# misterk72/MiniVideo

Hardware: NVIDIA B200
Metric: 1080p_idr_frames_per_s_recon_rgb (higher is better)
Workload: dtype int32

## Files before the change

minivideo_b200/csrc/mvg_api.cu:

```cuda
#include "mvgpu.h"

#include <cuda_runtime.h>
#include <nvtx3/nvToolsExt.h>

#include <algorithm>
#include <cstdarg>
#include <cstdio>
#include <cstdlib>
#include <cstring>
#include <new>
#include <thread>
#include <vector>

#include "mvg_internal.h"
#include "mvg_kernels.cuh"
#include "mvg_fused.cuh"


static char g_create_error[512] = "";

struct MvgRange {
    explicit MvgRange(const char *name) { nvtxRangePushA(name); }
    ~MvgRange() { nvtxRangePop(); }
};

#define MVG_PIPE_DEPTH 3
#define MVG_MAX_TICKETS 8

struct MvgTicket {
    cudaEvent_t done = nullptr;
    bool busy = false;
    uint64_t *h_picbase = nullptr;
    int cap = 0;
};
#define MVG_WORK_RING  64
#define MVG_K2_GROUP   1024

struct mvg_ctx {
    int device = -1, sm_count = 0;
    int k1_ctas_per_sm = 1, k2_ctas_per_sm = 1, kf_ctas_per_sm = 1;
    int mode = MVG_PIPELINE_FUSED;
    int stagger_override = -1;
    int max_w = 0, max_h = 0, max_pics = 0;
    int w_mbs = 0, h_mbs = 0;
    bool have_sps = false;
    char err[512] = "";

    cudaStream_t stream = nullptr, s_h2d = nullptr, s_d2h = nullptr;
    cudaEvent_t ev[4] = {nullptr, nullptr, nullptr, nullptr};
    cudaEvent_t ev_mark[2] = {nullptr, nullptr};
    cudaEvent_t ev_h2d[MVG_PIPE_DEPTH] = {}, ev_comp[MVG_PIPE_DEPTH] = {}, ev_d2h[MVG_PIPE_DEPTH] = {};
    bool ran_k3 = false, ran_fused = false;
    bool tiles_valid = false;
    int launches = 0, last_scale = 0;

    uint8_t *d_kind = nullptr, *d_i16 = nullptr, *d_cm = nullptr, *d_cbp = nullptr, *d_modes = nullptr;
    int8_t *d_qp = nullptr;
    int16_t *d_coeff = nullptr;
    uint32_t *d_nzb = nullptr, *d_woff = nullptr;
    uint16_t *d_words = nullptr;
    uint64_t *d_picbase = nullptr;
    MvgTicket tickets[MVG_MAX_TICKETS];
    long long pipe_idx = 0;
    bool region_used[MVG_PIPE_DEPTH] = {};
    int16_t *d_resid = nullptr;
    MvgMbCtl *d_ctl = nullptr;
    uint8_t *d_tiles = nullptr;
    uint8_t *d_yuv = nullptr, *d_rgb = nullptr;
    uint2 *d_halo = nullptr;
    int *d_work = nullptr;
    unsigned long long *d_stats = nullptr;
    int work_next = 0;
    unsigned epoch = 0;
    int pipe_chunk = 0;
    MvgTables *d_tab = nullptr;
    MvgLuts *d_luts = nullptr;
    struct Alloc { void *base; size_t bytes; const char *name; };
    std::vector<Alloc> allocs;
    bool guard = false;

    size_t n_mb_max() const { return (size_t)max_w * max_h; }
    size_t n_mb() const { return (size_t)w_mbs * h_mbs; }
};

static int fail(mvg_ctx *ctx, const char *fmt, ...)
{
    char *dst = ctx ? ctx->err : g_create_error;
    va_list ap;
    va_start(ap, fmt);
    vsnprintf(dst, 512, fmt, ap);
    va_end(ap);
    return MVG_FAILURE;
}

#define CK(ctx, call)                                                                      \
    do {                                                                                   \
        cudaError_t e__ = (call);                                                          \
        if (e__ != cudaSuccess)                                                            \
            return fail(ctx, "%s failed: %s (%s:%d)", #call, cudaGetErrorString(e__), __FILE__, __LINE__); \
    } while (0)


static void zigzag(int n, uint8_t *zz)
{
    int r = 0, c = 0;
    bool up = true;
    for (int k = 0; k < n * n; k++) {
        zz[k] = (uint8_t)(r * n + c);
        if (up) {
            if (c == n - 1) { r++; up = false; }
            else if (r == 0) { c++; up = false; }
            else { r--; c++; }
        } else {
            if (r == n - 1) { c++; up = true; }
            else if (c == 0) { r++; up = true; }
            else { r++; c--; }
        }
    }
}

extern "C" int mvg_build_level_scale(const uint8_t *lists4x4, const uint8_t *list8x8,
                                     int32_t ls4[3 * 6 * 16], int32_t ls8[6 * 64])
{
    static const int v4[6][3] = {{10,16,13},{11,18,14},{13,20,16},{14,23,18},{16,25,20},{18,29,23}};
    static const int v8[6][6] = {{20,18,32,19,25,24},{22,19,35,21,28,26},{26,23,42,24,33,31},
                                 {28,25,45,26,35,33},{32,28,51,30,40,38},{36,32,58,34,46,43}};
    if (!ls4 || !ls8) return MVG_FAILURE;
    uint8_t zz4[16], zz8[64];
    zigzag(4, zz4); zigzag(8, zz8);
    for (int c = 0; c < 3; c++) {
        int m[16];
        for (int k = 0; k < 16; k++) m[zz4[k]] = lists4x4 ? lists4x4[c * 16 + k] : 16;
        for (int q = 0; q < 6; q++)
            for (int i = 0; i < 4; i++)
                for (int j = 0; j < 4; j++) {
                    const int cls = (i % 2 == 0 && j % 2 == 0) ? 0 : (i % 2 == 1 && j % 2 == 1) ? 1 : 2;
                    ls4[(c * 6 + q) * 16 + i * 4 + j] = m[i * 4 + j] * v4[q][cls];
                }
    }
    int m8[64];
    for (int k = 0; k < 64; k++) m8[zz8[k]] = list8x8 ? list8x8[k] : 16;
    for (int q = 0; q < 6; q++)
        for (int i = 0; i < 8; i++)
            for (int j = 0; j < 8; j++) {
                int cls;
                if (i % 4 == 0 && j % 4 == 0) cls = 0;
                else if (i % 2 == 1 && j % 2 == 1) cls = 1;
                else if (i % 4 == 2 && j % 4 == 2) cls = 2;
                else if ((i % 4 == 0 && j % 2 == 1) || (i % 2 == 1 && j % 4 == 0)) cls = 3;
                else if ((i % 4 == 0 && j % 4 == 2) || (i % 4 == 2 && j % 4 == 0)) cls = 4;
                else cls = 5;
                ls8[q * 64 + i * 8 + j] = m8[i * 8 + j] * v8[q][cls];
            }
    return MVG_SUCCESS;
}

struct Ref { bool left; int i; };
static Ref T(int i) { return {false, i}; }
static Ref L(int i) { return i < 0 ? Ref{false, -1} : Ref{true, i}; }

struct Taps { Ref r[4]; int form; };
static Taps tap3(Ref p, Ref q, Ref r) { return {{p, q, q, r}, 3}; }
static Taps tap2(Ref p, Ref q) { return {{p, p, q, q}, 2}; }
static Taps tap1(Ref p) { return {{p, p, p, p}, 1}; }
static Taps tapend(Ref p, Ref q) { return {{p, q, q, q}, 4}; }

static Taps nxn_taps(int n, int mode, int x, int y)
{
    switch (mode) {
    case 0: return tap1(T(x));
    case 1: return tap1(L(y));
    case 3: return (x == n - 1 && y == n - 1) ? tapend(T(2 * n - 2), T(2 * n - 1))
                                              : tap3(T(x + y), T(x + y + 1), T(x + y + 2));
    case 4:
        if (x > y) return tap3(T(x - y - 2), T(x - y - 1), T(x - y));
        if (x < y) return tap3(L(y - x - 2), L(y - x - 1), L(y - x));
        return tap3(T(0), T(-1), L(0));
    case 5: {
        const int z = 2 * x - y, i = x - (y >> 1);
        if (z >= 0 && !(z & 1)) return tap2(T(i - 1), T(i));
        if (z >= 0) return tap3(T(i - 2), T(i - 1), T(i));
        if (z == -1) return tap3(L(0), T(-1), T(0));
        return tap3(L(y - 2 * x - 1), L(y - 2 * x - 2), L(y - 2 * x - 3));
    }
    case 6: {
        const int z = 2 * y - x, i = y - (x >> 1);
        if (z >= 0 && !(z & 1)) return tap2(L(i - 1), L(i));
        if (z >= 0) return tap3(L(i - 2), L(i - 1), L(i));
        if (z == -1) return tap3(L(0), T(-1), T(0));
        return tap3(T(x - 2 * y - 1), T(x - 2 * y - 2), T(x - 2 * y - 3));
    }
    case 7: {
        const int i = x + (y >> 1);
        return (y & 1) ? tap3(T(i), T(i + 1), T(i + 2)) : tap2(T(i), T(i + 1));
    }
    case 8: {
        const int z = x + 2 * y, i = y + (x >> 1), zmax = 2 * n - 3;
        if (z > zmax) return tap1(L(n - 1));
        if (z == zmax) return tapend(L(n - 2), L(n - 1));
        return (z & 1) ? tap3(L(i), L(i + 1), L(i + 2)) : tap2(L(i), L(i + 1));
    }
    default: return tap1(T(0));
    }
}

extern "C" void mvg_build_luts(MvgLuts *out)
{
    memset(out, 0, sizeof *out);
    for (int row = 0; row < 16; row++) {
        const int mode = row == 11 ? 3 : row == 15 ? 7 : row;
        const bool dc = row == 2 || row == 9 || row == 10;
        if ((mode > 8 && !dc)) continue;
        const bool tr = row < 9;
        for (int y = 0; y < 4; y++)
            for (int x = 0; x < 4; x++) {
                Taps t = nxn_taps(4, mode, x, y);
                if (dc) {
                    const bool above = row == 9 || (row == 2 && !(x & 1));
                    for (int k = 0; k < 4; k++) t.r[k] = above ? T(k) : L(k);
                }
                uint32_t word = 0;
                for (int k = 0; k < 4; k++) {
                    int off;
                    if (t.r[k].left) off = t.r[k].i * MVG_LT_STRIDE - 1;
                    else {
                        int i = t.r[k].i;
                        if (!tr && i > 3) i = 3;
                        off = -MVG_LT_STRIDE + i;
                    }
                    word |= (uint32_t)(off + MVG_LUT4_BIAS) << (8 * k);
                }
                out->lut4[row][y * 4 + x] = out->lut4[row][16 + y * 4 + x] = word;
            }
    }
    auto line8 = [](Ref r) { return r.left ? MVG_N8_LEFT(r.i) : MVG_N8_TOP(r.i); };
    for (int mode = 0; mode < 9; mode++)
        for (int lane = 0; lane < 32; lane++) {
            uint32_t word = 0;
            for (int s = 0; s < 2; s++) {
                const int x = ((lane >> 3) & 1) * 4 + (lane & 1) * 2 + s, y = (lane >> 4) * 4 + ((lane >> 1) & 3);
                int idx = MVG_N8_DC, variant = 0;
                if (mode != 2) {
                    const Taps t = nxn_taps(8, mode, x, y);
                    if (t.form == 1) { idx = line8(t.r[0]); variant = 0; }
                    else if (t.form == 2) {
                        const int a = line8(t.r[0]), b = line8(t.r[3]);
                        idx = a < b ? a : b; variant = 1;
                    } else { idx = line8(t.r[1]); variant = 2; }
                }
                word |= (uint32_t)(mode == 2 ? MVG_N8_DC : MVG_N8_IDX(idx, variant)) << (16 * s);
            }
            out->lut8[mode][lane] = word;
        }
}


extern "C" const char *mvg_last_error(const mvg_ctx *ctx) { return ctx ? ctx->err : g_create_error; }

#define MVG_GUARD_BYTES ((size_t)64 << 10)
#define MVG_GUARD_BYTE  0xA5
#define MVG_POISON_BYTE 0x5A

static cudaError_t galloc(mvg_ctx *ctx, void **p, size_t bytes, const char *name)
{
    const size_t g = ctx->guard ? MVG_GUARD_BYTES : 0;
    void *base = nullptr;
    cudaError_t e = cudaMalloc(&base, bytes + 2 * g);
    if (e != cudaSuccess) return e;
    try { ctx->allocs.push_back({base, bytes, name}); } catch (...) { cudaFree(base); return cudaErrorMemoryAllocation; }
    if (ctx->guard) {
        e = cudaMemset(base, MVG_GUARD_BYTE, bytes + 2 * g);
        if (e == cudaSuccess) e = cudaMemset((uint8_t *)base + g, MVG_POISON_BYTE, bytes);
        if (e != cudaSuccess) return e;
    }
    *p = (uint8_t *)base + g;
    return cudaSuccess;
}
template <typename T>
static cudaError_t dalloc(mvg_ctx *ctx, T **p, size_t count, const char *name) { return galloc(ctx, (void **)p, count * sizeof(T), name); }

extern "C" int mvg_create(mvg_ctx **out, int device, int max_w_mbs, int max_h_mbs, int max_pics)
{
    if (!out) return fail(nullptr, "mvg_create: out is NULL");
    *out = nullptr;
    if (max_w_mbs < 1 || max_h_mbs < 1 || max_pics < 1) return fail(nullptr, "mvg_create: bad geometry");
    int n_dev = 0;
    cudaError_t e = cudaGetDeviceCount(&n_dev);
    if (e != cudaSuccess || n_dev == 0)
        return fail(nullptr, "mvg_create: no CUDA device (%s); this library has no CPU fallback",
                    e == cudaSuccess ? "device count 0" : cudaGetErrorString(e));
    if (device < 0 || device >= n_dev) return fail(nullptr, "mvg_create: device %d out of range (0..%d)", device, n_dev - 1);

    mvg_ctx *ctx = new (std::nothrow) mvg_ctx;
    if (!ctx) return fail(nullptr, "mvg_create: out of host memory");
    ctx->device = device; ctx->max_w = max_w_mbs; ctx->max_h = max_h_mbs; ctx->max_pics = max_pics;
    if (const char *gd = getenv("MVG_DEBUG_GUARD")) ctx->guard = gd[0] == '1';

    auto bail = [&](const char *what, cudaError_t err) {
        fail(nullptr, "mvg_create: %s: %s", what, cudaGetErrorString(err));
        mvg_destroy(ctx);
        return MVG_FAILURE;
    };
#define TRY(what, call) do { cudaError_t e2 = (call); if (e2 != cudaSuccess) return bail(what, e2); } while (0)
    TRY("cudaSetDevice", cudaSetDevice(device));
    cudaDeviceProp prop;
    TRY("cudaGetDeviceProperties", cudaGetDeviceProperties(&prop, device));
    ctx->sm_count = prop.multiProcessorCount;
    TRY("k1 shared memory", cudaFuncSetAttribute(k1_dequant_idct, cudaFuncAttributeMaxDynamicSharedMemorySize, (int)(sizeof(K1WarpSmem) * K1_WARPS)));
    TRY("occupancy k1", cudaOccupancyMaxActiveBlocksPerMultiprocessor(&ctx->k1_ctas_per_sm, k1_dequant_idct, K1_WARPS * 32, sizeof(K1WarpSmem) * K1_WARPS));
    TRY("k2 shared memory", cudaFuncSetAttribute(k2_wavefront, cudaFuncAttributeMaxDynamicSharedMemorySize, (int)K2_SMEM_BYTES));
    TRY("occupancy k2", cudaOccupancyMaxActiveBlocksPerMultiprocessor(&ctx->k2_ctas_per_sm, k2_wavefront, K2_WARPS * 32, K2_SMEM_BYTES));
    TRY("kf shared memory", cudaFuncSetAttribute(kf_recon<KF_OUT_TILES>, cudaFuncAttributeMaxDynamicSharedMemorySize, (int)KF_SMEM_BYTES(KF_OUT_TILES)));
    TRY("kf shared memory", cudaFuncSetAttribute(kf_recon<KF_OUT_RGB>, cudaFuncAttributeMaxDynamicSharedMemorySize, (int)KF_SMEM_BYTES(KF_OUT_RGB)));
    TRY("kf shared memory", cudaFuncSetAttribute(kf_recon<KF_OUT_RGBS, 1>, cudaFuncAttributeMaxDynamicSharedMemorySize, (int)KF_SMEM_BYTES(KF_OUT_RGBS)));
    TRY("kf shared memory", cudaFuncSetAttribute(kf_recon<KF_OUT_RGBS, 2>, cudaFuncAttributeMaxDynamicSharedMemorySize, (int)KF_SMEM_BYTES(KF_OUT_RGBS)));
    TRY("kf shared memory", cudaFuncSetAttribute(kf_recon<KF_OUT_RGBS, 3>, cudaFuncAttributeMaxDynamicSharedMemorySize, (int)KF_SMEM_BYTES(KF_OUT_RGBS)));
    TRY("kf shared memory", cudaFuncSetAttribute(kf_recon<KF_OUT_RGBS, 4>, cudaFuncAttributeMaxDynamicSharedMemorySize, (int)KF_SMEM_BYTES(KF_OUT_RGBS)));
    {
        int a = 0, b = 0;
        TRY("occupancy kf", cudaOccupancyMaxActiveBlocksPerMultiprocessor(&a, kf_recon<KF_OUT_RGB>, KF_WARPS_OF(KF_OUT_RGB) * 32, KF_SMEM_BYTES(KF_OUT_RGB)));
        TRY("occupancy kf", cudaOccupancyMaxActiveBlocksPerMultiprocessor(&b, kf_recon<KF_OUT_TILES>, KF_WARPS_OF(KF_OUT_TILES) * 32, KF_SMEM_BYTES(KF_OUT_TILES)));
        ctx->kf_ctas_per_sm = std::min(a, b);
    }
    if (ctx->k1_ctas_per_sm < 1 || ctx->k2_ctas_per_sm < 1 || ctx->kf_ctas_per_sm < 1)
        return bail("kernel does not fit on an SM", cudaErrorLaunchOutOfResources);
    if (const char *m = getenv("MVG_PIPELINE")) ctx->mode = strcmp(m, "split") == 0 ? MVG_PIPELINE_SPLIT : MVG_PIPELINE_FUSED;
    if (const char *e = getenv("MVG_KF_STAGGER")) ctx->stagger_override = std::min(std::max(atoi(e), 0), 64);
    TRY("stream", cudaStreamCreateWithFlags(&ctx->stream, cudaStreamNonBlocking));
    TRY("stream", cudaStreamCreateWithFlags(&ctx->s_h2d, cudaStreamNonBlocking));
    TRY("stream", cudaStreamCreateWithFlags(&ctx->s_d2h, cudaStreamNonBlocking));
    for (auto &ev : ctx->ev) TRY("event", cudaEventCreate(&ev));
    for (auto &ev : ctx->ev_mark) TRY("event", cudaEventCreate(&ev));
    for (int i = 0; i < MVG_PIPE_DEPTH; i++) {
        TRY("event", cudaEventCreateWithFlags(&ctx->ev_h2d[i], cudaEventDisableTiming));
        TRY("event", cudaEventCreateWithFlags(&ctx->ev_comp[i], cudaEventDisableTiming));
        TRY("event", cudaEventCreateWithFlags(&ctx->ev_d2h[i], cudaEventDisableTiming));
    }
    const size_t n = ctx->n_mb_max() * (size_t)max_pics;
    TRY("alloc mb_kind", dalloc(ctx, &ctx->d_kind, n, "mb_kind"));
    TRY("alloc i16_mode", dalloc(ctx, &ctx->d_i16, n, "i16_mode"));
    TRY("alloc chroma_mode", dalloc(ctx, &ctx->d_cm, n, "chroma_mode"));
    TRY("alloc qp", dalloc(ctx, &ctx->d_qp, n, "qp"));
    TRY("alloc cbp", dalloc(ctx, &ctx->d_cbp, n, "cbp"));
    TRY("alloc luma_modes", dalloc(ctx, &ctx->d_modes, n * 16, "luma_modes"));
    TRY("alloc coeff", dalloc(ctx, &ctx->d_coeff, n * 384, "coeff"));
    TRY("alloc tiles", dalloc(ctx, &ctx->d_tiles, n * 384, "tiles"));
    TRY("alloc rgb", dalloc(ctx, &ctx->d_rgb, n * 768, "rgb"));
    TRY("alloc halo", dalloc(ctx, &ctx->d_halo, n * 8, "halo"));
    if (!ctx->guard) TRY("clear halo", cudaMemset(ctx->d_halo, 0, n * 8 * sizeof(uint2)));
    TRY("alloc work", dalloc(ctx, &ctx->d_work, MVG_WORK_RING, "work"));
    TRY("alloc stats", dalloc(ctx, &ctx->d_stats, 16, "stats"));
    TRY("clear stats", cudaMemset(ctx->d_stats, 0, 16 * sizeof(unsigned long long)));
    TRY("alloc tables", dalloc(ctx, &ctx->d_tab, 1, "tables"));
    TRY("alloc luts", dalloc(ctx, &ctx->d_luts, 1, "luts"));
    MvgLuts luts;
    mvg_build_luts(&luts);
    TRY("upload luts", cudaMemcpy(ctx->d_luts, &luts, sizeof luts, cudaMemcpyHostToDevice));
#undef TRY
    *out = ctx;
    return MVG_SUCCESS;
}

extern "C" int mvg_destroy(mvg_ctx *ctx)
{
    if (!ctx) return MVG_FAILURE;
    cudaSetDevice(ctx->device);
    cudaDeviceSynchronize();
    for (auto &a : ctx->allocs) cudaFree(a.base);
    for (auto &t : ctx->tickets) { if (t.h_picbase) cudaFreeHost(t.h_picbase); if (t.done) cudaEventDestroy(t.done); }
    for (auto ev : ctx->ev) if (ev) cudaEventDestroy(ev);
    for (auto ev : ctx->ev_mark) if (ev) cudaEventDestroy(ev);
    for (int i = 0; i < MVG_PIPE_DEPTH; i++) {
        if (ctx->ev_h2d[i]) cudaEventDestroy(ctx->ev_h2d[i]);
        if (ctx->ev_comp[i]) cudaEventDestroy(ctx->ev_comp[i]);
        if (ctx->ev_d2h[i]) cudaEventDestroy(ctx->ev_d2h[i]);
    }
    if (ctx->stream) cudaStreamDestroy(ctx->stream);
    if (ctx->s_h2d) cudaStreamDestroy(ctx->s_h2d);
    if (ctx->s_d2h) cudaStreamDestroy(ctx->s_d2h);
    delete ctx;
    return MVG_SUCCESS;
}

extern "C" int mvg_set_sps(mvg_ctx *ctx, int width_mbs, int height_mbs,
                           const int32_t level_scale4x4[3 * 6 * 16], const int32_t level_scale8x8[6 * 64],
                           int cb_qp_offset, int cr_qp_offset)
{
    MvgRange nvtx_range("mvg_set_sps");
    if (!ctx) return MVG_FAILURE;
    if (!level_scale4x4 || !level_scale8x8) return fail(ctx, "mvg_set_sps: NULL table");
    if (width_mbs < 1 || height_mbs < 1 || width_mbs > ctx->max_w || height_mbs > ctx->max_h)
        return fail(ctx, "mvg_set_sps: %dx%d MBs exceeds the context capacity %dx%d",
                    width_mbs, height_mbs, ctx->max_w, ctx->max_h);
    CK(ctx, cudaSetDevice(ctx->device));
    MvgTables t;
    memset(&t, 0, sizeof t);
    memcpy(t.ls4, level_scale4x4, sizeof t.ls4);
    memcpy(t.ls8, level_scale8x8, sizeof t.ls8);
    for (int c = 0; c < 3; c++)
        for (int qp = 0; qp < 52; qp++)
            for (int k = 0; k < 16; k++) {
                const int32_t v = t.ls4[c][qp % 6][k];
                t.ls4q[c][qp][k] = qp > 23 ? (int32_t)((uint32_t)v << (qp / 6 - 4)) : v;
            }
    uint8_t zz8[64];
    zigzag(8, zz8);
    for (int k = 0; k < 64; k++) t.zz8inv[zz8[k]] = (uint8_t)k;
    t.cb_qp_offset = cb_qp_offset; t.cr_qp_offset = cr_qp_offset;
    CK(ctx, cudaStreamSynchronize(ctx->s_h2d));
    CK(ctx, cudaStreamSynchronize(ctx->stream));
    CK(ctx, cudaStreamSynchronize(ctx->s_d2h));
    CK(ctx, cudaMemcpy(ctx->d_tab, &t, sizeof t, cudaMemcpyHostToDevice));
    ctx->w_mbs = width_mbs; ctx->h_mbs = height_mbs; ctx->have_sps = true;
    return MVG_SUCCESS;
}

extern "C" int mvg_set_pipeline(mvg_ctx *ctx, int chunk_pics)
{
    if (!ctx || chunk_pics < 0) return MVG_FAILURE;
    ctx->pipe_chunk = chunk_pics;
    return MVG_SUCCESS;
}

extern "C" int mvg_dev_k2_stats(mvg_ctx *ctx, unsigned long long out[16])
{
    if (!ctx || !out) return MVG_FAILURE;
    CK(ctx, cudaSetDevice(ctx->device));
    CK(ctx, cudaStreamSynchronize(ctx->stream));
    CK(ctx, cudaMemcpy(out, ctx->d_stats, 16 * sizeof(unsigned long long), cudaMemcpyDeviceToHost));
    CK(ctx, cudaMemset(ctx->d_stats, 0, 16 * sizeof(unsigned long long)));
    return MVG_SUCCESS;
}

extern "C" long long mvg_debug_check(mvg_ctx *ctx, char *report, size_t report_cap)
{
    if (!ctx) return -1;
    if (report && report_cap) report[0] = 0;
    if (!ctx->guard) return 0;
    if (cudaSetDevice(ctx->device) != cudaSuccess || cudaDeviceSynchronize() != cudaSuccess) return -1;
    std::vector<uint8_t> h(MVG_GUARD_BYTES);
    long long bad = 0;
    for (auto &a : ctx->allocs)
        for (int side = 0; side < 2; side++) {
            const uint8_t *src = (const uint8_t *)a.base + (side ? MVG_GUARD_BYTES + a.bytes : 0);
            if (cudaMemcpy(h.data(), src, MVG_GUARD_BYTES, cudaMemcpyDeviceToHost) != cudaSuccess) return -1;
            long long here = 0;
            for (uint8_t b : h) here += b != MVG_GUARD_BYTE;
            if (here && report && report_cap) {
                const size_t o = strlen(report);
                snprintf(report + o, report_cap - o, "%s%s(%s): %lld bytes", o ? ", " : "", a.name, side ? "after" : "before", here);
            }
            bad += here;
        }
    return bad;
}

extern "C" int mvg_debug_check_kernels(mvg_ctx *ctx, unsigned long long out[8])
{
    if (!ctx || !out) return MVG_FAILURE;
    memset(out, 0, 8 * sizeof(unsigned long long));
#ifdef MVG_CHECKED
    CK(ctx, cudaSetDevice(ctx->device));
    CK(ctx, cudaDeviceSynchronize());
    CK(ctx, cudaMemcpyFromSymbol(out, mvg_check_fail, 8 * sizeof(unsigned long long)));
    return MVG_SUCCESS;
#else
    return MVG_UNSUPPORTED;
#endif
}

extern "C" int mvg_device_count(void)
{
    int n = 0;
    return cudaGetDeviceCount(&n) == cudaSuccess ? n : 0;
}

extern "C" int mvg_width(const mvg_ctx *ctx) { return ctx ? 16 * ctx->w_mbs : 0; }
extern "C" int mvg_height(const mvg_ctx *ctx) { return ctx ? 16 * ctx->h_mbs : 0; }
extern "C" int mvg_max_pics(const mvg_ctx *ctx) { return ctx ? ctx->max_pics : 0; }
extern "C" int mvg_sm_count(const mvg_ctx *ctx) { return ctx ? ctx->sm_count : 0; }

extern "C" void *mvg_host_alloc(size_t bytes)
{
    void *p = nullptr;
    if (cudaHostAlloc(&p, bytes, cudaHostAllocDefault) != cudaSuccess) return nullptr;
    return p;
}
extern "C" void mvg_host_free(void *p) { if (p) cudaFreeHost(p); }


static int check_ready(mvg_ctx *ctx, int first_slot, int n_pics, const char *who)
{
    if (!ctx) return MVG_FAILURE;
    if (!ctx->have_sps) return fail(ctx, "%s: mvg_set_sps() has not been called", who);
    if (n_pics < 1 || first_slot < 0 || first_slot + n_pics > ctx->max_pics)
        return fail(ctx, "%s: slots [%d,%d) outside [0,%d)", who, first_slot, first_slot + n_pics, ctx->max_pics);
    return MVG_SUCCESS;
}

static int upload_async(mvg_ctx *ctx, const mvg_batch *b, int src_pic, int first_slot, int n_pics, cudaStream_t st)
{
    const size_t n = ctx->n_mb(), o = (size_t)first_slot * n, s = (size_t)src_pic * n, cnt = (size_t)n_pics * n;
    CK(ctx, cudaMemcpyAsync(ctx->d_kind + o, b->mb_kind + s, cnt, cudaMemcpyHostToDevice, st));
    CK(ctx, cudaMemcpyAsync(ctx->d_i16 + o, b->i16_mode + s, cnt, cudaMemcpyHostToDevice, st));
    CK(ctx, cudaMemcpyAsync(ctx->d_cm + o, b->chroma_mode + s, cnt, cudaMemcpyHostToDevice, st));
    CK(ctx, cudaMemcpyAsync(ctx->d_qp + o, b->qp_y + s, cnt, cudaMemcpyHostToDevice, st));
    if (b->cbp) CK(ctx, cudaMemcpyAsync(ctx->d_cbp + o, b->cbp + s, cnt, cudaMemcpyHostToDevice, st));
    CK(ctx, cudaMemcpyAsync(ctx->d_modes + o * 16, b->luma_modes + s * 16, cnt * 16, cudaMemcpyHostToDevice, st));
    CK(ctx, cudaMemcpyAsync(ctx->d_coeff + o * 384, b->coeff + s * 384, cnt * 768, cudaMemcpyHostToDevice, st));
    return MVG_SUCCESS;
}

static int check_batch(mvg_ctx *ctx, const mvg_batch *b, const char *who)
{
    if (!b) return fail(ctx, "%s: batch is NULL", who);
    if (!b->mb_kind || !b->i16_mode || !b->chroma_mode || !b->qp_y || !b->luma_modes || !b->coeff)
        return fail(ctx, "%s: a required SoA pointer is NULL", who);
    return MVG_SUCCESS;
}

extern "C" int mvg_upload(mvg_ctx *ctx, const mvg_batch *b, int first_slot)
{
    MvgRange nvtx_range("mvg_upload");
    if (!ctx) return MVG_FAILURE;
    if (check_batch(ctx, b, "mvg_upload") != MVG_SUCCESS) return MVG_FAILURE;
    if (check_ready(ctx, first_slot, b->n_pics, "mvg_upload") != MVG_SUCCESS) return MVG_FAILURE;
    CK(ctx, cudaSetDevice(ctx->device));
    if (upload_async(ctx, b, 0, first_slot, b->n_pics, ctx->stream) != MVG_SUCCESS) return MVG_FAILURE;
    CK(ctx, cudaStreamSynchronize(ctx->stream));
    return MVG_SUCCESS;
}

extern "C" int mvg_clone_slot(mvg_ctx *ctx, int src_slot, int dst_slot)
{
    MvgRange nvtx_range("mvg_clone_slot");
    if (check_ready(ctx, src_slot, 1, "mvg_clone_slot") != MVG_SUCCESS) return MVG_FAILURE;
    if (check_ready(ctx, dst_slot, 1, "mvg_clone_slot") != MVG_SUCCESS) return MVG_FAILURE;
    CK(ctx, cudaSetDevice(ctx->device));
    const size_t n = ctx->n_mb(), s = (size_t)src_slot * n, d = (size_t)dst_slot * n;
    cudaStream_t st = ctx->stream;
    CK(ctx, cudaMemcpyAsync(ctx->d_kind + d, ctx->d_kind + s, n, cudaMemcpyDeviceToDevice, st));
    CK(ctx, cudaMemcpyAsync(ctx->d_i16 + d, ctx->d_i16 + s, n, cudaMemcpyDeviceToDevice, st));
    CK(ctx, cudaMemcpyAsync(ctx->d_cm + d, ctx->d_cm + s, n, cudaMemcpyDeviceToDevice, st));
    CK(ctx, cudaMemcpyAsync(ctx->d_qp + d, ctx->d_qp + s, n, cudaMemcpyDeviceToDevice, st));
    CK(ctx, cudaMemcpyAsync(ctx->d_cbp + d, ctx->d_cbp + s, n, cudaMemcpyDeviceToDevice, st));
    CK(ctx, cudaMemcpyAsync(ctx->d_modes + d * 16, ctx->d_modes + s * 16, n * 16, cudaMemcpyDeviceToDevice, st));
    CK(ctx, cudaMemcpyAsync(ctx->d_coeff + d * 384, ctx->d_coeff + s * 384, n * 768, cudaMemcpyDeviceToDevice, st));
    return MVG_SUCCESS;
}


static int ensure_yuv(mvg_ctx *ctx)
{
    if (!ctx->d_yuv) CK(ctx, dalloc(ctx, &ctx->d_yuv, ctx->n_mb_max() * (size_t)ctx->max_pics * 384, "yuv"));
    return MVG_SUCCESS;
}
static int ensure_split(mvg_ctx *ctx)
{
    const size_t n = ctx->n_mb_max() * (size_t)ctx->max_pics;
    if (!ctx->d_resid) CK(ctx, dalloc(ctx, &ctx->d_resid, n * 384, "residual"));
    if (!ctx->d_ctl) CK(ctx, dalloc(ctx, &ctx->d_ctl, n, "ctl"));
    return MVG_SUCCESS;
}

static int launch_planar(mvg_ctx *ctx, int first_slot, int n_pics, cudaStream_t st)
{
    if (ensure_yuv(ctx) != MVG_SUCCESS) return MVG_FAILURE;
    K3Params p;
    p.tiles = ctx->d_tiles; p.yuv = ctx->d_yuv; p.rgb = nullptr; p.width = 16 * ctx->w_mbs; p.height = 16 * ctx->h_mbs;
    p.scale = 1; p.first_slot = first_slot; p.n_pics = n_pics;
    const long long threads = (long long)ctx->n_mb() * 12 * n_pics;
    const int grid = (int)std::min<long long>((threads + 255) / 256, (long long)ctx->sm_count * 32);
    k4_yuv_planar<<<grid, 256, 0, st>>>(p);
    CK(ctx, cudaGetLastError());
    return MVG_SUCCESS;
}

static int launch_k1(mvg_ctx *ctx, int first_slot, int n_pics, cudaStream_t st)
{
    if (ensure_split(ctx) != MVG_SUCCESS) return MVG_FAILURE;
    const size_t n = ctx->n_mb();
    K1Params p;
    const size_t o = (size_t)first_slot * n;
    p.mb_kind = ctx->d_kind + o; p.i16_mode = ctx->d_i16 + o; p.chroma_mode = ctx->d_cm + o;
    p.luma_modes = ctx->d_modes + o * 16; p.qp_y = ctx->d_qp + o; p.coeff = ctx->d_coeff + o * 384;
    p.resid = ctx->d_resid + o * 384; p.ctl = ctx->d_ctl + o; p.tab = ctx->d_tab;
    p.n_mbs = (long long)n * n_pics;
    const long long groups = (p.n_mbs + K1_GROUP - 1) / K1_GROUP;
    const long long want = (groups + K1_WARPS - 1) / K1_WARPS;
    const int grid = (int)std::min<long long>(want, (long long)ctx->sm_count * ctx->k1_ctas_per_sm);
    k1_dequant_idct<<<grid, K1_WARPS * 32, sizeof(K1WarpSmem) * K1_WARPS, st>>>(p);
    CK(ctx, cudaGetLastError());
    return MVG_SUCCESS;
}

static int launch_k3(mvg_ctx *ctx, int first_slot, int n_pics, int rgb_scale, cudaStream_t st)
{
    const size_t n = ctx->n_mb();
    const int width = 16 * ctx->w_mbs, height = 16 * ctx->h_mbs;
    K3Params p;
    p.tiles = ctx->d_tiles; p.yuv = nullptr; p.rgb = ctx->d_rgb; p.width = width; p.height = height; p.scale = rgb_scale;
    p.first_slot = first_slot; p.n_pics = n_pics;
    const long long threads = rgb_scale == 1 ? (long long)n * 8 * n_pics
                                             : (long long)(width / rgb_scale) * (height / rgb_scale) * n_pics;
    const int grid = (int)std::min<long long>((threads + 255) / 256, (long long)ctx->sm_count * 32);
    const bool pow2 = rgb_scale == 2 || rgb_scale == 4 || rgb_scale == 8 || rgb_scale == 16;
    if (rgb_scale == 1) k3_rgb_full<<<grid, 256, 0, st>>>(p);
    else if (pow2) k3_rgb_scaled<<<(int)std::min<long long>(((long long)n * n_pics + 31) / 32, (long long)ctx->sm_count * 16), 256, 0, st>>>(p);
    else k3_rgb_scaled_generic<<<grid, 256, 0, st>>>(p);
    CK(ctx, cudaGetLastError());
    return MVG_SUCCESS;
}

static int launch_stages(mvg_ctx *ctx, int first_slot, int n_pics, int rgb_scale, bool want_tiles, cudaStream_t st, bool timed)
{
    const int W = ctx->w_mbs, H = ctx->h_mbs;
    const size_t n = ctx->n_mb();
    const int width = 16 * W, height = 16 * H;
    if (rgb_scale < 0 || (rgb_scale > 0 && (width % rgb_scale || height % rgb_scale)))
        return fail(ctx, "rgb_scale %d does not divide %dx%d", rgb_scale, width, height);

    int *work = ctx->d_work + ctx->work_next;
    ctx->work_next = (ctx->work_next + 1) % MVG_WORK_RING;
    CK(ctx, cudaMemsetAsync(work, 0, sizeof(int), st));
    if (++ctx->epoch == 0) ctx->epoch = 1;

    const bool fused = ctx->mode == MVG_PIPELINE_FUSED;
    const bool thumbs = rgb_scale == 2 || rgb_scale == 4 || rgb_scale == 8 || rgb_scale == 16;
    const bool rgb_direct = fused && !want_tiles && (rgb_scale == 1 || thumbs);
    int launches = 0;
    if (timed) CK(ctx, cudaEventRecord(ctx->ev[0], st));
    if (!fused) {
        if (launch_k1(ctx, first_slot, n_pics, st) != MVG_SUCCESS) return MVG_FAILURE;
        launches++;
    }
    if (timed) CK(ctx, cudaEventRecord(ctx->ev[1], st));
    const long long items = (long long)n_pics * H;
    if (fused) {
        KFParams p;
        p.mb_kind = ctx->d_kind; p.i16_mode = ctx->d_i16; p.chroma_mode = ctx->d_cm; p.luma_modes = ctx->d_modes;
        p.qp_y = ctx->d_qp; p.coeff = ctx->d_coeff; p.tiles = ctx->d_tiles; p.rgb = ctx->d_rgb; p.halo = ctx->d_halo;
        p.work = work; p.tab = ctx->d_tab; p.luts = ctx->d_luts; p.epoch = ctx->epoch;
        p.w_mbs = W; p.h_mbs = H; p.first_slot = first_slot; p.n_pics = n_pics; p.group = MVG_K2_GROUP;
        p.sel[0] = 1u; p.sel[1] = 1u << 8; p.sel[2] = 1u << 16; p.sel[3] = 1u << 24;
        p.stats = ctx->d_stats;
        p.stagger = items < 2LL * ctx->sm_count * KF_WARPS ? KF_GROUP + 1 : KF_STAGGER;
        if (ctx->stagger_override >= 0) p.stagger = ctx->stagger_override;
        const int grid = (int)std::min<long long>(items, (long long)ctx->sm_count * ctx->kf_ctas_per_sm);
        if (rgb_direct && thumbs) {
            const unsigned bt = KF_WARPS_OF(KF_OUT_RGBS) * 32;
            const size_t sm = KF_SMEM_BYTES(KF_OUT_RGBS);
            if (rgb_scale == 2)      kf_recon<KF_OUT_RGBS, 1><<<grid, bt, sm, st>>>(p);
            else if (rgb_scale == 4) kf_recon<KF_OUT_RGBS, 2><<<grid, bt, sm, st>>>(p);
            else if (rgb_scale == 8) kf_recon<KF_OUT_RGBS, 3><<<grid, bt, sm, st>>>(p);
            else                     kf_recon<KF_OUT_RGBS, 4><<<grid, bt, sm, st>>>(p);
        } else if (rgb_direct) kf_recon<KF_OUT_RGB><<<grid, KF_WARPS_OF(KF_OUT_RGB) * 32, KF_SMEM_BYTES(KF_OUT_RGB), st>>>(p);
        else kf_recon<KF_OUT_TILES><<<grid, KF_WARPS_OF(KF_OUT_TILES) * 32, KF_SMEM_BYTES(KF_OUT_TILES), st>>>(p);
        launches++;
    } else {
        K2Params p;
        p.resid = ctx->d_resid; p.ctl = ctx->d_ctl; p.tiles = ctx->d_tiles; p.halo = ctx->d_halo;
        p.epoch = ctx->epoch; p.group = MVG_K2_GROUP; p.stats = ctx->d_stats;
        p.sel[0] = 1u; p.sel[1] = 1u << 8; p.sel[2] = 1u << 16; p.sel[3] = 1u << 24;
        p.work = work; p.luts = ctx->d_luts; p.w_mbs = W; p.h_mbs = H; p.first_slot = first_slot; p.n_pics = n_pics;
        const int grid = (int)std::min<long long>((items + K2_WARPS - 1) / K2_WARPS, (long long)ctx->sm_count * ctx->k2_ctas_per_sm);
        k2_wavefront<<<grid, K2_WARPS * 32, K2_SMEM_BYTES, st>>>(p);
        launches++;
    }
    CK(ctx, cudaGetLastError());
    if (timed) CK(ctx, cudaEventRecord(ctx->ev[2], st));
    const bool run_k3 = rgb_scale >= 1 && !rgb_direct;
    if (run_k3) {
        if (launch_k3(ctx, first_slot, n_pics, rgb_scale, st) != MVG_SUCCESS) return MVG_FAILURE;
        launches++;
    }
    if (timed) {
        CK(ctx, cudaEventRecord(ctx->ev[3], st));
        ctx->ran_k3 = run_k3;
        ctx->ran_fused = fused;
        ctx->launches = launches;
    }
    ctx->last_scale = rgb_scale;
    ctx->tiles_valid = !rgb_direct;
    return MVG_SUCCESS;
}

extern "C" int mvg_run(mvg_ctx *ctx, int first_slot, int n_pics, int rgb_scale)
{
    MvgRange nvtx_range("mvg_run");
    if (check_ready(ctx, first_slot, n_pics, "mvg_run") != MVG_SUCCESS) return MVG_FAILURE;
    CK(ctx, cudaSetDevice(ctx->device));
    return launch_stages(ctx, first_slot, n_pics, rgb_scale, true, ctx->stream, true);
}

extern "C" int mvg_run_thumbs(mvg_ctx *ctx, int first_slot, int n_pics, int rgb_scale)
{
    MvgRange nvtx_range("mvg_run_thumbs");
    if (check_ready(ctx, first_slot, n_pics, "mvg_run_thumbs") != MVG_SUCCESS) return MVG_FAILURE;
    if (rgb_scale < 1) return fail(ctx, "mvg_run_thumbs: rgb_scale %d", rgb_scale);
    CK(ctx, cudaSetDevice(ctx->device));
    return launch_stages(ctx, first_slot, n_pics, rgb_scale, false, ctx->stream, true);
}

extern "C" int mvg_run_rgb(mvg_ctx *ctx, int first_slot, int n_pics)
{
    MvgRange nvtx_range("mvg_run_rgb");
    if (check_ready(ctx, first_slot, n_pics, "mvg_run_rgb") != MVG_SUCCESS) return MVG_FAILURE;
    CK(ctx, cudaSetDevice(ctx->device));
    return launch_stages(ctx, first_slot, n_pics, 1, false, ctx->stream, true);
}

extern "C" int mvg_set_pipeline_mode(mvg_ctx *ctx, int mode)
{
    if (!ctx || (mode != MVG_PIPELINE_FUSED && mode != MVG_PIPELINE_SPLIT)) return MVG_FAILURE;
    ctx->mode = mode;
    return MVG_SUCCESS;
}

extern "C" int mvg_sync(mvg_ctx *ctx)
{
    if (!ctx) return MVG_FAILURE;
    CK(ctx, cudaSetDevice(ctx->device));
    CK(ctx, cudaStreamSynchronize(ctx->stream));
    CK(ctx, cudaStreamSynchronize(ctx->s_h2d));
    CK(ctx, cudaStreamSynchronize(ctx->s_d2h));
    return MVG_SUCCESS;
}

extern "C" int mvg_get_timing(mvg_ctx *ctx, mvg_timing *out)
{
    if (!ctx || !out) return MVG_FAILURE;
    CK(ctx, cudaSetDevice(ctx->device));
    CK(ctx, cudaEventSynchronize(ctx->ev[3]));
    out->k1_dequant_idct_ms = out->k2_wavefront_ms = out->fused_ms = 0.f;
    if (ctx->ran_fused) CK(ctx, cudaEventElapsedTime(&out->fused_ms, ctx->ev[1], ctx->ev[2]));
    else {
        CK(ctx, cudaEventElapsedTime(&out->k1_dequant_idct_ms, ctx->ev[0], ctx->ev[1]));
        CK(ctx, cudaEventElapsedTime(&out->k2_wavefront_ms, ctx->ev[1], ctx->ev[2]));
    }
    out->k3_rgb_ms = 0.f;
    if (ctx->ran_k3) CK(ctx, cudaEventElapsedTime(&out->k3_rgb_ms, ctx->ev[2], ctx->ev[3]));
    CK(ctx, cudaEventElapsedTime(&out->total_ms, ctx->ev[0], ctx->ev[3]));
    out->launches = ctx->launches;
    return MVG_SUCCESS;
}

extern "C" int mvg_mark(mvg_ctx *ctx, int which)
{
    if (!ctx || which < 0 || which > 1) return MVG_FAILURE;
    CK(ctx, cudaSetDevice(ctx->device));
    CK(ctx, cudaEventRecord(ctx->ev_mark[which], ctx->stream));
    return MVG_SUCCESS;
}

extern "C" int mvg_mark_elapsed(mvg_ctx *ctx, float *ms)
{
    if (!ctx || !ms) return MVG_FAILURE;
    CK(ctx, cudaSetDevice(ctx->device));
    CK(ctx, cudaEventSynchronize(ctx->ev_mark[1]));
    CK(ctx, cudaEventElapsedTime(ms, ctx->ev_mark[0], ctx->ev_mark[1]));
    return MVG_SUCCESS;
}


static size_t rgb_bytes(const mvg_ctx *ctx, int scale)
{
    return (size_t)(16 * ctx->w_mbs / scale) * (16 * ctx->h_mbs / scale) * 3;
}

extern "C" int mvg_download_yuv420(mvg_ctx *ctx, int slot, uint8_t *y, uint8_t *cb, uint8_t *cr)
{
    MvgRange nvtx_range("mvg_download_yuv420");
    if (check_ready(ctx, slot, 1, "mvg_download_yuv420") != MVG_SUCCESS) return MVG_FAILURE;
    if (!ctx->tiles_valid) return fail(ctx, "mvg_download_yuv420: the last run produced RGB24 only (mvg_run_rgb, mvg_run_thumbs); use mvg_run()");
    CK(ctx, cudaSetDevice(ctx->device));
    const size_t n = ctx->n_mb();
    if (launch_planar(ctx, slot, 1, ctx->stream) != MVG_SUCCESS) return MVG_FAILURE;
    const uint8_t *src = ctx->d_yuv + (size_t)slot * n * 384;
    CK(ctx, cudaStreamSynchronize(ctx->stream));
    if (y) CK(ctx, cudaMemcpy(y, src, n * 256, cudaMemcpyDeviceToHost));
    if (cb) CK(ctx, cudaMemcpy(cb, src + n * 256, n * 64, cudaMemcpyDeviceToHost));
    if (cr) CK(ctx, cudaMemcpy(cr, src + n * 320, n * 64, cudaMemcpyDeviceToHost));
    return MVG_SUCCESS;
}

extern "C" int mvg_download_rgb(mvg_ctx *ctx, int slot, uint8_t *rgb)
{
    MvgRange nvtx_range("mvg_download_rgb");
    if (check_ready(ctx, slot, 1, "mvg_download_rgb") != MVG_SUCCESS) return MVG_FAILURE;
    if (!rgb || ctx->last_scale < 1) return fail(ctx, "mvg_download_rgb: no RGB output (last run had rgb_scale 0)");
    CK(ctx, cudaSetDevice(ctx->device));
    const size_t sz = rgb_bytes(ctx, ctx->last_scale);
    CK(ctx, cudaStreamSynchronize(ctx->stream));
    CK(ctx, cudaMemcpy(rgb, ctx->d_rgb + (size_t)slot * sz, sz, cudaMemcpyDeviceToHost));
    return MVG_SUCCESS;
}

extern "C" int mvg_download_residual(mvg_ctx *ctx, int slot, int16_t *residual)
{
    MvgRange nvtx_range("mvg_download_residual");
    if (check_ready(ctx, slot, 1, "mvg_download_residual") != MVG_SUCCESS) return MVG_FAILURE;
    if (!residual) return fail(ctx, "mvg_download_residual: NULL");
    CK(ctx, cudaSetDevice(ctx->device));
    const size_t n = ctx->n_mb();
    if (launch_k1(ctx, slot, 1, ctx->stream) != MVG_SUCCESS) return MVG_FAILURE;
    CK(ctx, cudaStreamSynchronize(ctx->stream));
    int16_t *tmp = new (std::nothrow) int16_t[n * 384];
    if (!tmp) return fail(ctx, "mvg_download_residual: out of host memory");
    cudaError_t e = cudaMemcpy(tmp, ctx->d_resid + (size_t)slot * n * 384, n * 768, cudaMemcpyDeviceToHost);
    if (e != cudaSuccess) { delete[] tmp; return fail(ctx, "cudaMemcpy failed: %s", cudaGetErrorString(e)); }
    for (size_t mb = 0; mb < n; mb++) {
        const int16_t *src = tmp + mb * 384;
        int16_t *dst = residual + mb * 384;
        for (int b = 0; b < 16; b++) {
            const int bx = (b & 1) | (((b >> 2) & 1) << 1), by = ((b >> 1) & 1) | ((b >> 3) << 1);
            for (int i = 0; i < 4; i++)
                for (int j = 0; j < 4; j++) dst[(by * 4 + i) * 16 + bx * 4 + j] = src[b * 16 + i * 4 + j];
        }
        for (int p = 0; p < 2; p++)
            for (int b = 0; b < 4; b++)
                for (int i = 0; i < 4; i++)
                    for (int j = 0; j < 4; j++)
                        dst[256 + p * 64 + ((b >> 1) * 4 + i) * 8 + (b & 1) * 4 + j] = src[256 + p * 64 + b * 16 + i * 4 + j];
    }
    delete[] tmp;
    return MVG_SUCCESS;
}


static int take_ticket(mvg_ctx *ctx, mvg_ticket *out)
{
    for (int i = 0; i < MVG_MAX_TICKETS; i++)
        if (!ctx->tickets[i].busy) {
            if (!ctx->tickets[i].done) CK(ctx, cudaEventCreateWithFlags(&ctx->tickets[i].done, cudaEventDisableTiming | cudaEventBlockingSync));
            *out = i;
            return MVG_SUCCESS;
        }
    return fail(ctx, "too many submissions in flight (%d): mvg_wait() for one first", MVG_MAX_TICKETS);
}

template <typename Upload, typename Expand>
static int decode_pipeline(mvg_ctx *ctx, int n_pics, uint8_t *yuv_out, uint8_t *rgb_out, int rgb_scale, cudaEvent_t done_ev,
                           Upload upload, Expand expand)
{
    const int scale = rgb_out ? rgb_scale : 0;
    const size_t n = ctx->n_mb();
    const size_t yuv_sz = n * 384, rgb_sz = scale ? rgb_bytes(ctx, scale) : 0;
    if (yuv_out && ensure_yuv(ctx) != MVG_SUCCESS) return MVG_FAILURE;
    int depth = MVG_PIPE_DEPTH;
    if (ctx->max_pics < depth) depth = 1;
    const int region = std::max(1, ctx->max_pics / depth);
    int chunk = std::min(region, std::max(1, (n_pics + 7) / 8));
    if (scale > 1 && !yuv_out) chunk = std::min(region, std::max(chunk, std::min(n_pics, 128)));
    if (ctx->pipe_chunk > 0) chunk = std::min(ctx->pipe_chunk, region);
    for (int done = 0; done < n_pics; done += chunk, ctx->pipe_idx++) {
        const int cnt = std::min(chunk, n_pics - done);
        const int r = (int)(ctx->pipe_idx % depth), slot0 = r * region;
        const bool used = ctx->region_used[r];
        ctx->region_used[r] = true;
        if (used) CK(ctx, cudaStreamWaitEvent(ctx->s_h2d, ctx->ev_comp[r], 0));
        if (upload(done, slot0, cnt) != MVG_SUCCESS) return MVG_FAILURE;
        CK(ctx, cudaEventRecord(ctx->ev_h2d[r], ctx->s_h2d));
        CK(ctx, cudaStreamWaitEvent(ctx->stream, ctx->ev_h2d[r], 0));
        if (used) CK(ctx, cudaStreamWaitEvent(ctx->stream, ctx->ev_d2h[r], 0));
        if (expand(slot0, cnt) != MVG_SUCCESS) return MVG_FAILURE;
        if (launch_stages(ctx, slot0, cnt, scale, yuv_out != nullptr, ctx->stream, false) != MVG_SUCCESS) return MVG_FAILURE;
        if (yuv_out && launch_planar(ctx, slot0, cnt, ctx->stream) != MVG_SUCCESS) return MVG_FAILURE;
        CK(ctx, cudaEventRecord(ctx->ev_comp[r], ctx->stream));
        CK(ctx, cudaStreamWaitEvent(ctx->s_d2h, ctx->ev_comp[r], 0));
        if (yuv_out)
            CK(ctx, cudaMemcpyAsync(yuv_out + (size_t)done * yuv_sz, ctx->d_yuv + (size_t)slot0 * yuv_sz,
                                    (size_t)cnt * yuv_sz, cudaMemcpyDeviceToHost, ctx->s_d2h));
        if (rgb_out)
            CK(ctx, cudaMemcpyAsync(rgb_out + (size_t)done * rgb_sz, ctx->d_rgb + (size_t)slot0 * rgb_sz,
                                    (size_t)cnt * rgb_sz, cudaMemcpyDeviceToHost, ctx->s_d2h));
        CK(ctx, cudaEventRecord(ctx->ev_d2h[r], ctx->s_d2h));
    }
    CK(ctx, cudaEventRecord(done_ev, ctx->s_d2h));
    return MVG_SUCCESS;
}

extern "C" int mvg_wait(mvg_ctx *ctx, mvg_ticket ticket)
{
    MvgRange nvtx_range("mvg_wait");
    if (!ctx) return MVG_FAILURE;
    if (ticket < 0 || ticket >= MVG_MAX_TICKETS || !ctx->tickets[ticket].busy) return fail(ctx, "mvg_wait: ticket %d is not in flight", (int)ticket);
    CK(ctx, cudaSetDevice(ctx->device));
    ctx->tickets[ticket].busy = false;
    CK(ctx, cudaEventSynchronize(ctx->tickets[ticket].done));
    return MVG_SUCCESS;
}

extern "C" int mvg_poll(mvg_ctx *ctx, mvg_ticket ticket, int *done)
{
    if (!ctx || !done) return MVG_FAILURE;
    if (ticket < 0 || ticket >= MVG_MAX_TICKETS || !ctx->tickets[ticket].busy) return fail(ctx, "mvg_poll: ticket %d is not in flight", (int)ticket);
    const cudaError_t e = cudaEventQuery(ctx->tickets[ticket].done);
    if (e != cudaSuccess && e != cudaErrorNotReady) return fail(ctx, "mvg_poll: %s", cudaGetErrorString(e));
    *done = e == cudaSuccess;
    return MVG_SUCCESS;
}

extern "C" int mvg_submit(mvg_ctx *ctx, const mvg_batch *b, uint8_t *yuv_out, uint8_t *rgb_out, int rgb_scale, mvg_ticket *ticket)
{
    MvgRange nvtx_range("mvg_submit");
    if (!ctx) return MVG_FAILURE;
    if (!ticket) return fail(ctx, "mvg_submit: ticket is NULL");
    if (check_batch(ctx, b, "mvg_submit") != MVG_SUCCESS) return MVG_FAILURE;
    if (!ctx->have_sps) return fail(ctx, "mvg_submit: mvg_set_sps() has not been called");
    if (b->n_pics < 1) return fail(ctx, "mvg_submit: empty batch");
    if (rgb_out && rgb_scale < 1) return fail(ctx, "mvg_submit: rgb_out given but rgb_scale < 1");
    CK(ctx, cudaSetDevice(ctx->device));
    if (take_ticket(ctx, ticket) != MVG_SUCCESS) return MVG_FAILURE;
    MvgTicket &t = ctx->tickets[*ticket];
    const mvg_batch batch = *b;
    if (decode_pipeline(ctx, batch.n_pics, yuv_out, rgb_out, rgb_scale, t.done,
                        [&](int done, int slot0, int cnt) { return upload_async(ctx, &batch, done, slot0, cnt, ctx->s_h2d); },
                        [&](int, int) { return (int)MVG_SUCCESS; }) != MVG_SUCCESS) return MVG_FAILURE;
    t.busy = true;
    return MVG_SUCCESS;
}

extern "C" int mvg_decode_host(mvg_ctx *ctx, const mvg_batch *b, uint8_t *yuv_out, uint8_t *rgb_out, int rgb_scale)
{
    mvg_ticket t;
    if (mvg_submit(ctx, b, yuv_out, rgb_out, rgb_scale, &t) != MVG_SUCCESS) return MVG_FAILURE;
    return mvg_wait(ctx, t);
}


extern "C" int mvg_pack_batch(const int16_t *coeff, int n_pics, int n_mbs, uint32_t *nz_blocks, uint32_t *word_off,
                              uint64_t *pic_off, uint16_t *words, size_t words_capacity, int n_threads)
{
    MvgRange nvtx_range("mvg_pack_batch");
    if (!coeff || !nz_blocks || !word_off || !pic_off || !words || n_pics < 1 || n_mbs < 1) return MVG_FAILURE;
    try {
    std::vector<uint64_t> pic_words((size_t)n_pics);
    auto pass1 = [&](int p) {
        uint64_t off = 0;
        for (int m = 0; m < n_mbs; m++) {
            const size_t mb = (size_t)p * n_mbs + m;
            const int16_t *c = coeff + mb * 384;
            uint32_t nzb = 0;
            unsigned words_here = 0;
            for (int b = 0; b < 24; b++) {
                unsigned cnt = 0;
                for (int k = 0; k < 16; k++) cnt += c[b * 16 + k] != 0;
                if (cnt) { nzb |= 1u << b; words_here += 1 + cnt; }
            }
            nz_blocks[mb] = nzb;
            word_off[mb] = (uint32_t)off;
            off += words_here;
        }
        pic_words[(size_t)p] = off;
    };
    auto pass2 = [&](int p) {
        for (int m = 0; m < n_mbs; m++) {
            const size_t mb = (size_t)p * n_mbs + m;
            const int16_t *c = coeff + mb * 384;
            const uint32_t nzb = nz_blocks[mb];
            uint16_t *w = words + pic_off[p] + word_off[mb];
            uint16_t *lv = w + __builtin_popcount(nzb);
            for (int b = 0; b < 24; b++) {
                if (!((nzb >> b) & 1u)) continue;
                unsigned mask = 0;
                for (int k = 0; k < 16; k++)
                    if (c[b * 16 + k]) { mask |= 1u << k; *lv++ = (uint16_t)c[b * 16 + k]; }
                *w++ = (uint16_t)mask;
            }
        }
    };
    int nt = n_threads > 0 ? n_threads : (int)std::thread::hardware_concurrency();
    nt = std::max(1, std::min(nt, n_pics));
    auto run = [&](auto &fn) {
        std::vector<std::thread> th;
        for (int t = 0; t < nt; t++)
            th.emplace_back([&, t] { for (int p = t; p < n_pics; p += nt) fn(p); });
        for (auto &x : th) x.join();
    };
    run(pass1);
    pic_off[0] = 0;
    for (int p = 0; p < n_pics; p++) pic_off[p + 1] = pic_off[p] + pic_words[(size_t)p];
    if (pic_off[n_pics] > words_capacity) return MVG_FAILURE;
    run(pass2);
    } catch (...) {
        return MVG_FAILURE;
    }
    return MVG_SUCCESS;
}

extern "C" int mvg_submit_packed(mvg_ctx *ctx, const mvg_packed_batch *b, uint8_t *yuv_out, uint8_t *rgb_out, int rgb_scale, mvg_ticket *ticket)
{
    MvgRange nvtx_range("mvg_submit_packed");
    if (!ctx) return MVG_FAILURE;
    if (!ticket) return fail(ctx, "mvg_submit_packed: ticket is NULL");
    if (!b) return fail(ctx, "mvg_decode_host_packed: batch is NULL");
    if (!b->mb_kind || !b->i16_mode || !b->chroma_mode || !b->qp_y || !b->luma_modes || !b->nz_blocks || !b->word_off ||
        !b->pic_off || !b->words)
        return fail(ctx, "mvg_decode_host_packed: a required pointer is NULL");
    if (!ctx->have_sps) return fail(ctx, "mvg_decode_host_packed: mvg_set_sps() has not been called");
    if (b->n_pics < 1) return fail(ctx, "mvg_decode_host_packed: empty batch");
    if (rgb_out && rgb_scale < 1) return fail(ctx, "mvg_decode_host_packed: rgb_out given but rgb_scale < 1");
    CK(ctx, cudaSetDevice(ctx->device));
    const size_t n = ctx->n_mb();
    if (!ctx->d_words) {
        const size_t cap = ctx->n_mb_max() * (size_t)ctx->max_pics;
        CK(ctx, dalloc(ctx, &ctx->d_nzb, cap, "nz_blocks"));
        CK(ctx, dalloc(ctx, &ctx->d_woff, cap, "word_off"));
        CK(ctx, dalloc(ctx, &ctx->d_words, cap * MVG_PACKED_WORDS_PER_MB, "words"));
        CK(ctx, dalloc(ctx, &ctx->d_picbase, (size_t)ctx->max_pics * 2 + 2, "pic_base"));
    }
    if (take_ticket(ctx, ticket) != MVG_SUCCESS) return MVG_FAILURE;
    MvgTicket &tk = ctx->tickets[*ticket];
    if (b->n_pics > tk.cap) {
        if (tk.h_picbase) cudaFreeHost(tk.h_picbase);
        tk.h_picbase = nullptr; tk.cap = 0;
        CK(ctx, cudaHostAlloc((void **)&tk.h_picbase, ((size_t)b->n_pics * 2 + 2) * sizeof(uint64_t), cudaHostAllocDefault));
        tk.cap = b->n_pics;
    }
    for (int p = 0; p < b->n_pics; p++)
        if (b->pic_off[p + 1] < b->pic_off[p] || b->pic_off[p + 1] - b->pic_off[p] > (uint64_t)n * MVG_PACKED_WORDS_PER_MB)
            return fail(ctx, "mvg_decode_host_packed: picture %d has an impossible word count", p);
    auto upload = [&](int done, int slot0, int cnt) -> int {
        const size_t o = (size_t)slot0 * n, s = (size_t)done * n, c = (size_t)cnt * n;
        cudaStream_t st = ctx->s_h2d;
        CK(ctx, cudaMemcpyAsync(ctx->d_kind + o, b->mb_kind + s, c, cudaMemcpyHostToDevice, st));
        CK(ctx, cudaMemcpyAsync(ctx->d_i16 + o, b->i16_mode + s, c, cudaMemcpyHostToDevice, st));
        CK(ctx, cudaMemcpyAsync(ctx->d_cm + o, b->chroma_mode + s, c, cudaMemcpyHostToDevice, st));
        CK(ctx, cudaMemcpyAsync(ctx->d_qp + o, b->qp_y + s, c, cudaMemcpyHostToDevice, st));
        CK(ctx, cudaMemcpyAsync(ctx->d_modes + o * 16, b->luma_modes + s * 16, c * 16, cudaMemcpyHostToDevice, st));
        CK(ctx, cudaMemcpyAsync(ctx->d_nzb + o, b->nz_blocks + s, c * sizeof(uint32_t), cudaMemcpyHostToDevice, st));
        CK(ctx, cudaMemcpyAsync(ctx->d_woff + o, b->word_off + s, c * sizeof(uint32_t), cudaMemcpyHostToDevice, st));
        const uint64_t w0 = b->pic_off[done], w1 = b->pic_off[done + cnt], base = (uint64_t)o * MVG_PACKED_WORDS_PER_MB;
        if (w1 > w0)
            CK(ctx, cudaMemcpyAsync(ctx->d_words + base, b->words + w0, (size_t)(w1 - w0) * sizeof(uint16_t), cudaMemcpyHostToDevice, st));
        uint64_t *hb = tk.h_picbase + 2 * (size_t)done;
        for (int i = 0; i <= cnt; i++) hb[i] = base + (b->pic_off[done + i] - w0);
        CK(ctx, cudaMemcpyAsync(ctx->d_picbase + 2 * (size_t)slot0, hb, (size_t)(cnt + 1) * sizeof(uint64_t), cudaMemcpyHostToDevice, st));
        return MVG_SUCCESS;
    };
    auto expand = [&](int slot0, int cnt) -> int {
        K0Params p;
        const size_t o = (size_t)slot0 * n;
        p.nz_blocks = ctx->d_nzb + o; p.word_off = ctx->d_woff + o; p.pic_base = ctx->d_picbase + 2 * (size_t)slot0;
        p.words = ctx->d_words; p.coeff = ctx->d_coeff + o * 384; p.n_mbs = (long long)cnt * (long long)n; p.mbs_per_pic = (int)n;
        const long long warps = p.n_mbs;
        const int grid = (int)std::min<long long>((warps + 7) / 8, (long long)ctx->sm_count * 16);
        k0_expand_levels<<<grid, 256, 0, ctx->stream>>>(p);
        CK(ctx, cudaGetLastError());
        return MVG_SUCCESS;
    };
    if (decode_pipeline(ctx, b->n_pics, yuv_out, rgb_out, rgb_scale, tk.done, upload, expand) != MVG_SUCCESS) return MVG_FAILURE;
    tk.busy = true;
    return MVG_SUCCESS;
}

extern "C" int mvg_decode_host_packed(mvg_ctx *ctx, const mvg_packed_batch *b, uint8_t *yuv_out, uint8_t *rgb_out, int rgb_scale)
{
    mvg_ticket t;
    if (mvg_submit_packed(ctx, b, yuv_out, rgb_out, rgb_scale, &t) != MVG_SUCCESS) return MVG_FAILURE;
    return mvg_wait(ctx, t);
}
```

minivideo_b200/csrc/mvg_fused.cuh:

```cuda
#pragma once

#include <cstddef>

#include "mvg_kernels.cuh"

#ifndef KF_GROUP
#define KF_GROUP 4
#endif
#ifndef KF_WARPS
#define KF_WARPS 25
#endif
#ifndef KF_WARPS_TILES
#define KF_WARPS_TILES 28
#endif
#ifndef KF_WARPS_RGBS
#define KF_WARPS_RGBS 28
#endif
#define KF_WARPS_OF(out) ((out) == 1 ? KF_WARPS : (out) == 2 ? KF_WARPS_RGBS : KF_WARPS_TILES)
#ifndef KF_COMPACT8
#define KF_COMPACT8 false
#endif
#ifndef KF_POLL_NS
#define KF_POLL_NS 1000
#endif
#ifndef KF_STAGGER
#define KF_STAGGER 12
#endif
#ifndef KF_MBS
#define KF_MBS 392
#endif
#define KF_OUT_TILES 0
#define KF_OUT_RGB   1
#define KF_OUT_RGBS  2
#define KF_RGBS_PITCH 96
#define KF_RGB_STRIDE 112
#ifndef KF_WO_GROUP
#define KF_WO_GROUP (KF_GROUP == 4)
#endif
#define KF_RGB_GSTRIDE 208
#ifndef KF_HALO_GROUP
#define KF_HALO_GROUP (KF_GROUP == 4)
#endif

struct KFParams {
    const uint8_t *mb_kind, *i16_mode, *chroma_mode, *luma_modes;
    const int8_t  *qp_y;
    const int16_t *coeff;
    uint8_t       *tiles;
    uint8_t       *rgb;
    uint2         *halo;
    int           *work;
    const MvgTables *tab;
    const MvgLuts   *luts;
    unsigned        epoch;
    int w_mbs, h_mbs, first_slot, n_pics, group;
    int stagger;
    unsigned        sel[4];
    unsigned long long *stats;
};

#ifdef KF_STATS
#define KF_STAT(...) __VA_ARGS__
#else
#define KF_STAT(...)
#endif

template <int OUT>
struct KFWarpSmemT {
    union {
        MvgXfScratch<KF_GROUP> x;
        uint8_t rgb[OUT == 0 ? 16 : OUT == 2 ? 8 * KF_RGBS_PITCH : KF_WO_GROUP ? 16 * KF_RGB_GSTRIDE : 16 * KF_RGB_STRIDE];
    } u;
    MVG_CANARY(c0)
    __align__(128) int16_t tile[KF_GROUP * KF_MBS];
    __align__(8) uint64_t mbar;
    __align__(16) uint32_t hrow[36];
    MVG_CANARY(c1)
    __align__(16) uint8_t lt[MVG_LT_ROWS * MVG_LT_STRIDE];
    uint8_t ct_pad[4];
    alignas(OUT == 0 ? 16 : 4) uint8_t ct[2][MVG_CT_PLANE];
    MVG_CANARY(c2)
    __align__(16) uint8_t n8[MVG_N8_BYTES];
    MVG_CANARY(c3)
#ifdef KF_REC_PAD
    uint8_t pad[KF_REC_PAD];
#endif
};

#define KF_LUT_BYTES  ((sizeof(MvgLuts) + 127) / 128 * 128)
#define KF_TAB_BYTES  ((sizeof(MvgXfTables) + 127) / 128 * 128)
#define KF_SMEM_BYTES(out) (sizeof(KFWarpSmemT<out>) * KF_WARPS_OF(out) + 2048 + KF_LUT_BYTES + KF_TAB_BYTES)

#ifdef KF_MAXREG
#define KF_BOUNDS __maxnreg__(KF_MAXREG)
#else
#define KF_BOUNDS __launch_bounds__(KF_WARPS_OF(OUT) * 32, 1)
#endif
template <int OUT, int SL = 2>
__global__ void KF_BOUNDS
kf_recon(KFParams p)
{
    extern __shared__ __align__(128) uint8_t kf_smem[];
    typedef KFWarpSmemT<OUT> KFWarpSmem;
    const int lane = mvg_lane();
    const unsigned wid = __shfl_sync(MVG_FULL, threadIdx.x >> 5, 0);
    const unsigned base = mvg_smem_u32(kf_smem);
    const unsigned lut_addr = __shfl_sync(MVG_FULL, mvg_keep((base + 2047u) & ~2047u), 0);
    const unsigned n_before = (lut_addr - base) / (unsigned)sizeof(KFWarpSmem);
    MvgLuts *luts = reinterpret_cast<MvgLuts *>(__cvta_shared_to_generic(lut_addr));
    MvgXfTables &T = *reinterpret_cast<MvgXfTables *>(__cvta_shared_to_generic(lut_addr + (unsigned)KF_LUT_BYTES));
    unsigned rec_addr = base + (wid < n_before ? wid * (unsigned)sizeof(KFWarpSmem)
                                               : (lut_addr - base) + (unsigned)(KF_LUT_BYTES + KF_TAB_BYTES) + (wid - n_before) * (unsigned)sizeof(KFWarpSmem));
    rec_addr = __shfl_sync(MVG_FULL, mvg_keep(rec_addr), 0);
    KFWarpSmem &s = *reinterpret_cast<KFWarpSmem *>(__cvta_shared_to_generic(rec_addr));
    for (int i = threadIdx.x; i < (int)(KF_LUT_BYTES / 16); i += blockDim.x)
        reinterpret_cast<uint4 *>(luts)[i] = __ldg(reinterpret_cast<const uint4 *>(p.luts) + i);
    mvg_xf_load_tables(T, p.tab);
    if (lane == 0) mvg_mbar_init(&s.mbar, 1);
    asm volatile("fence.mbarrier_init.release.cluster;" ::: "memory");
    asm volatile("fence.proxy.async.shared::cta;" ::: "memory");
    __syncthreads();

    const int W = p.w_mbs, H = p.h_mbs, n_mb = W * H;
    const int total = p.n_pics * H;
    const unsigned epoch = p.epoch;
    const int n_groups = (W + KF_GROUP - 1) / KF_GROUP;

    K2Ctx c;
#ifdef MVG_CHECKED
    c.rec_lo = reinterpret_cast<const uint8_t *>(&s); c.rec_hi = c.rec_lo + sizeof(KFWarpSmem);
    if (lane < 4) s.c0[lane] = s.c1[lane] = s.c2[lane] = s.c3[lane] = MVG_CANARY_WORD;
    __syncwarp();
#endif
    c.lt = s.lt; c.ct = &s.ct[0][0]; c.n8 = s.n8; c.lut8 = reinterpret_cast<const uint8_t *>(&luts->lut8[0][lane]);
    c.lane = lane;
    c.sel = p.sel;
    c.resid = reinterpret_cast<const uint8_t *>(s.tile);
    {
        const int half = lane >> 4, pix = lane & 15, px = pix & 3, py = pix >> 2;
        c.lut4 = lut_addr + (unsigned)lane * 4u;
        c.h4 = half ? 0u : (unsigned)(4 * MVG_LT_STRIDE - 8);
        c.s4 = py * MVG_LT_STRIDE + px + (int)c.h4;
        c.r4odd = pix * 2 + (half ? 64 : 0);
        c.r4even = pix * 2 + (half ? -64 : 0);
        c.m4c = half ? 0x10100010u : 0x10001000u;
        c.m4b = half ? 0x00000100u : 0x00000011u;
        c.m4cc = half ? 0x00001000u : 0u;
        const int n = lane < 25 ? lane : 24;
        if (n < 8)       c.n8tr = (7 - n) * MVG_LT_STRIDE - 1;
        else if (n == 8) c.n8tr = -MVG_LT_STRIDE - 1;
        else             c.n8tr = -MVG_LT_STRIDE + (n - 9);
        c.n8notr = n > 16 ? -MVG_LT_STRIDE + 7 : c.n8tr;
        const int x8 = ((lane >> 3) & 1) * 4 + (lane & 1) * 2, y8 = (lane >> 4) * 4 + ((lane >> 1) & 3);
        c.s8 = y8 * MVG_LT_STRIDE + x8;
        c.fixA = lane == 7 ? 0x10u : lane == 8 ? 0x22u : lane == 9 ? 0x20u : 0u;
        c.fixB = lane == 7 ? 0x04u : lane == 8 ? 0x05u : lane == 9 ? 0x08u : 0u;
        c.fixD = lane == 7 ? 0x01u : lane == 9 ? 0x02u : 0u;
        c.lut4 = mvg_keep(c.lut4); c.h4 = mvg_keep(c.h4); c.s4 = mvg_keep(c.s4); c.r4odd = mvg_keep(c.r4odd); c.r4even = mvg_keep(c.r4even);
    }
    uint8_t *const halo_top = lane < 4 ? s.lt + K2_TO(lane * 4, -1)
                            : lane < 8 ? s.ct[(lane >> 1) & 1] + K2_CO((lane & 1) * 4, -1)
                                       : s.lt + K2_TO(16 + (lane & 1) * 4, -1);
    const uint8_t *const halo_bot = lane < 4 ? halo_top + 16 * MVG_LT_STRIDE : halo_top + 8 * MVG_CT_STRIDE;
    const uint8_t *const cn_src = (lane == 3 || lane == 5 || lane == 7) ? halo_top + 3 : s.lt;
    uint8_t *const cn_dst = lane == 3 ? s.lt + K2_TO(-1, -1) : lane == 5 ? s.ct[0] + K2_CO(-1, -1)
                          : lane == 7 ? s.ct[1] + K2_CO(-1, -1) : s.lt;
    const uint8_t *wo_src, *wo_csrc = nullptr;
    uint8_t *lc_dst, *lc_cdst = nullptr, *rgb_dst = nullptr;
    const uint8_t *lc_src = nullptr;
    int wo_off = 0;
    if (OUT == KF_OUT_TILES) {
        wo_src = lane < 16 ? s.lt + K2_TO(0, lane) : s.ct[(lane >> 3) & 1] + K2_CO(0, lane & 7);
        wo_off = lane < 16 ? lane * 16 : 256 + (lane - 16) * 8;
        lc_dst = lane < 16 ? s.lt + K2_TO(-1, lane) : s.ct[(lane >> 3) & 1] + K2_CO(-1, lane & 7);
    } else {
        const int q = lane >> 2, h = lane & 3;
        wo_src = s.lt + K2_TO(4 * h, 2 * q);
        wo_csrc = s.ct[0] + K2_CO(2 * h, q);
        lc_dst = s.lt + K2_TO(-1, 2 * q);
        lc_cdst = s.ct[0] + K2_CO(-1, q);
        lc_dst = lane < 16 ? s.lt + K2_TO(-1, lane) : s.ct[(lane >> 3) & 1] + K2_CO(-1, lane & 7);
        lc_src = lc_dst + (lane < 16 ? 16 : 8);
        rgb_dst = KF_WO_GROUP ? s.u.rgb + q * KF_RGB_GSTRIDE + 12 * h : s.u.rgb + 2 * q * KF_RGB_STRIDE + 12 * h;
    }
    const unsigned lc_sel = lane < 16 ? 7u : 3u;
    const int pitch = 48 * W;

    MvgSideInfo side;
    side.init(lane, p.mb_kind, p.i16_mode, p.chroma_mode, p.luma_modes, p.qp_y);
    unsigned parity = 0;
    KF_STAT(unsigned long long st[8] = {0, 0, 0, 0, 0, 0, 0, 0};)

    for (;;) {
        int item = 0;
        if (lane == 0) item = atomicAdd(p.work, 1);
        item = __shfl_sync(MVG_FULL, item, 0);
        if (item >= total) break;
        const int g0 = item / (p.group * H);
        const int gsize = min(p.group, p.n_pics - g0 * p.group);
        const int within = item - g0 * p.group * H;
        const int row = within / gsize;
        const int slot = p.first_slot + g0 * p.group + (within - row * gsize);
        const size_t mb0 = (size_t)slot * n_mb + (size_t)row * W;
        const int16_t *lv_row = p.coeff + mb0 * 384;

        if (lane == 0) {
            const int n0 = min(KF_GROUP, W);
            asm volatile("fence.proxy.async.shared::cta;" ::: "memory");
            mvg_mbar_expect_tx(&s.mbar, (unsigned)n0 * 768u);
            if (KF_MBS == 384) mvg_bulk_load(s.tile, lv_row, (unsigned)n0 * 768u, &s.mbar);
            else for (int j = 0; j < n0; j++) mvg_bulk_load(s.tile + j * KF_MBS, lv_row + j * 384, 768u, &s.mbar);
        }
        unsigned nmeta = side.load(lane, (long long)mb0, min(KF_GROUP, W));

        constexpr int sl = SL, per = 16 >> sl;
        const int opitch = W * per * 3;
        uint8_t *wo_run = OUT == KF_OUT_TILES ? p.tiles + mb0 * 384 + wo_off
                        : OUT == KF_OUT_RGB   ? p.rgb + (size_t)slot * ((size_t)n_mb * 768) + (size_t)row * 16 * pitch
                                              : p.rgb + ((size_t)slot * H + row) * ((size_t)per * opitch);
        uint2 *hm_run = p.halo + mb0 * 8 + lane;
        const bool availB = row > 0, publish = row < H - 1;
        const int hwords = W * 8;
#if KF_HALO_GROUP
        const uint4 *ha_run = reinterpret_cast<const uint4 *>(p.halo + (mb0 - W) * 8) + lane;
        uint4 hq = make_uint4(0, epoch, 0, epoch);
#else
        const uint2 *ha_run = p.halo + (mb0 - W) * 8 + lane;
        uint2 qa = make_uint2(0, epoch), qb = make_uint2(0, epoch);
#endif
        if (availB) {
            if (p.stagger > 0) {
                const uint2 *probe = p.halo + (mb0 - W + min(p.stagger, W - 1)) * 8 + 7;
                KF_STAT(const long long ts = clock64();)
                while (mvg_ld_relaxed_u64(probe).y != epoch) { __nanosleep(2000); KF_STAT(st[0]++;) }
                KF_STAT(st[1] += clock64() - ts;)
            }
#if KF_HALO_GROUP
            if (lane < 17 && 2 * lane < hwords) hq = mvg_ld_relaxed_2u64(ha_run);
#else
            if (lane < hwords) qb = mvg_ld_relaxed_u64(ha_run);
#endif
        }
#if !KF_HALO_GROUP
        unsigned okA = 0;
#endif

        KF_STAT(st[5]++; const long long trow = clock64();)
        for (int g = 0; g < n_groups; g++) {
            const unsigned meta = nmeta;
            const int nmb = min(KF_GROUP, W - g * KF_GROUP);
            const int n_next = min(KF_GROUP, W - (g + 1) * KF_GROUP);
            if (n_next > 0) nmeta = side.load(lane, (long long)mb0 + (g + 1) * KF_GROUP, n_next);
            int16_t *tile = s.tile;
            mvg_mbar_wait(&s.mbar, parity);
            parity ^= 1u;
            if (n_next > 0 && lane == 0) mvg_mbar_expect_tx(&s.mbar, (unsigned)n_next * 768u);

            mvg_xf_group<KF_GROUP, KF_MBS>(tile, s.u.x, T, meta, nmb, lane);
            const uint4 rec = mvg_ctl_from_meta(meta);

#if KF_HALO_GROUP
            if (availB) {
                for (;;) {
                    if (__all_sync(MVG_FULL, hq.y == epoch && hq.w == epoch)) break;
                    const uint2 *probe = p.halo + (mb0 - W + min(g * KF_GROUP + max(p.stagger, KF_GROUP + 1), W - 1)) * 8 + 7;
                    KF_STAT(const long long ts = clock64(); st[2]++;)
                    while (mvg_ld_relaxed_u64(probe).y != epoch) { __nanosleep(KF_POLL_NS); KF_STAT(st[3]++;) }
                    KF_STAT(st[4] += clock64() - ts;)
                    if (lane < 17 && g * 32 + 2 * lane < hwords) hq = mvg_ld_relaxed_2u64(ha_run);
                }
                if (lane < 17) *reinterpret_cast<uint2 *>(s.hrow + 2 * lane) = make_uint2(hq.x, hq.z);
                ha_run += 16;
                hq = make_uint4(0, epoch, 0, epoch);
                if (n_next > 0 && lane < 17 && (g + 1) * 32 + 2 * lane < hwords) hq = mvg_ld_relaxed_2u64(ha_run);
                __syncwarp();
            }
#endif

            for (int j = 0; j < nmb; j++) {
                const int mx = g * KF_GROUP + j;
#if !KF_HALO_GROUP
                const int hj = mx & 3;
#endif
                const bool availA = mx > 0, availC = availB && mx < W - 1, availD = availA && availB;

#if KF_HALO_GROUP
                if (availB && lane < 10) *reinterpret_cast<unsigned *>(halo_top) = s.hrow[8 * j + lane];
                __syncwarp();
#else
                if (availB) {
                    if (hj == 0) {
                        qa = qb;
                        okA = __ballot_sync(MVG_FULL, qa.y == epoch);
                    }
                    bool all_ok = okA == MVG_FULL;
                    if (hj == 3 && availC) all_ok = all_ok && (__ballot_sync(MVG_FULL, qb.y == epoch) & 3u) == 3u;
                    if (!all_ok) {
                      const unsigned need = availC ? 0x3FFu : 0xFFu;
                      unsigned have = __funnelshift_r(okA, hj == 3 ? __ballot_sync(MVG_FULL, qb.y == epoch) : 0u, 8 * hj);
                      if ((have & need) != need) {
                        const uint2 *probe = p.halo + (mb0 - W + min(mx + max(p.stagger, 2), W - 1)) * 8 + 7;
                        KF_STAT(const long long ts = clock64(); st[2]++;)
                        while (mvg_ld_relaxed_u64(probe).y != epoch) { __nanosleep(KF_POLL_NS); KF_STAT(st[3]++;) }
                        KF_STAT(st[4] += clock64() - ts;)
                        do {
                            if ((mx & ~3) * 8 + lane < hwords) qa = mvg_ld_relaxed_u64(ha_run);
                            if ((mx & ~3) * 8 + 32 + lane < hwords) qb = mvg_ld_relaxed_u64(ha_run + 32);
                            okA = __ballot_sync(MVG_FULL, qa.y == epoch);
                            have = __funnelshift_r(okA, __ballot_sync(MVG_FULL, qb.y == epoch), 8 * hj);
                        } while ((have & need) != need);
                      }
                    }
                    const unsigned src = (hj == 3 && lane < 2) ? qb.x : qa.x;
                    const unsigned v = __shfl_sync(MVG_FULL, src, (8 * hj + lane) & 31);
                    if (lane < 10) *reinterpret_cast<unsigned *>(halo_top) = v;
                    if (hj == 3) ha_run += 32;
                }
                __syncwarp();
                if (availB && hj == 0) {
                    qb = make_uint2(0, epoch);
                    if (mx * 8 + 32 + lane < hwords) qb = mvg_ld_relaxed_u64(ha_run + 32);
                }
#endif
                c.resid = reinterpret_cast<const uint8_t *>(tile + j * KF_MBS);
                const unsigned cx = __shfl_sync(MVG_FULL, rec.x, 8 * j), cy = __shfl_sync(MVG_FULL, rec.y, 8 * j);
                const unsigned cz = __shfl_sync(MVG_FULL, rec.z, 8 * j);

                const int kind = cx & 255, i16 = (cx >> 8) & 255, cmode = (cx >> 16) & 255;
                if (kind == MVG_MB_I16x16)    k2_luma16(c, i16, availA, availB);
                else if (kind == MVG_MB_I4x4) k2_luma4(c, cy, cz, availA, availB, availC);
                else                          k2_luma8<KF_COMPACT8>(c, cy, availA, availB, availC, availD);
                k2_chroma(c, cmode, availA, availB);
                __syncwarp();

                if (publish && lane < 8)
                    mvg_st_relaxed_u64(hm_run, *reinterpret_cast<const unsigned *>(halo_bot), epoch);
                hm_run += 8;
                if (OUT == KF_OUT_TILES) {
                    const uint2 wa = *reinterpret_cast<const uint2 *>(wo_src);
                    uint2 wb = make_uint2(0u, 0u);
                    if (lane < 16) {
                        wb = *reinterpret_cast<const uint2 *>(wo_src + 8);
                        *reinterpret_cast<uint4 *>(wo_run) = make_uint4(wa.x, wa.y, wb.x, wb.y);
                    } else *reinterpret_cast<uint2 *>(wo_run) = wa;
                    wo_run += 384;
                    *lc_dst = (uint8_t)__byte_perm(wa.y, wb.y, lc_sel);
                } else {
                    const unsigned y0 = *reinterpret_cast<const unsigned *>(wo_src);
                    const unsigned y1 = *reinterpret_cast<const unsigned *>(wo_src + MVG_LT_STRIDE);
                    const unsigned cb2 = mvg_pair_lo(*reinterpret_cast<const uint16_t *>(wo_csrc));
                    const unsigned cr2 = mvg_pair_lo(*reinterpret_cast<const uint16_t *>(wo_csrc + MVG_CT_PLANE));
                    *lc_dst = *lc_src;
                    const unsigned rC = __vsub2(((cr2 * 204u) >> 7) & 0x01ff01ffu, 0x00de00deu);
                    const unsigned bC = __vsub2(((cb2 * 129u) >> 6) & 0x03ff03ffu, 0x01140114u);
                    const unsigned gC = __vsub2(__vsub2(0x00870087u, ((cb2 * 25u) >> 6) & 0x00ff00ffu),
                                                ((cr2 * 13u) >> 4) & 0x00ff00ffu);
                    if (OUT == KF_OUT_RGBS) {
                        unsigned aR = 0, aG = 0, aB = 0;
#pragma unroll
                        for (int r = 0; r < 2; r++) {
                            const unsigned w = r ? y1 : y0;
                            const unsigned te = ((mvg_pair_even(w) * 149u) >> 7) & 0x01ff01ffu;
                            const unsigned to = ((mvg_pair_odd(w) * 149u) >> 7) & 0x01ff01ffu;
                            aR += mvg_add_clip8x2(te, rC) + mvg_add_clip8x2(to, rC);
                            aG += mvg_add_clip8x2(te, gC) + mvg_add_clip8x2(to, gC);
                            aB += mvg_add_clip8x2(te, bC) + mvg_add_clip8x2(to, bC);
                        }
                        const int q = lane >> 2, h = lane & 3;
                        if constexpr (sl == 1) {
                            uint16_t *d = reinterpret_cast<uint16_t *>(s.u.rgb + q * KF_RGBS_PITCH + j * 24 + h * 6);
                            const unsigned R0 = ((aR & 0xffffu) + 2) >> 2, R1 = ((aR >> 16) + 2) >> 2;
                            const unsigned G0 = ((aG & 0xffffu) + 2) >> 2, G1 = ((aG >> 16) + 2) >> 2;
                            const unsigned B0 = ((aB & 0xffffu) + 2) >> 2, B1 = ((aB >> 16) + 2) >> 2;
                            d[0] = (uint16_t)(R0 | (G0 << 8)); d[1] = (uint16_t)(B0 | (R1 << 8)); d[2] = (uint16_t)(G1 | (B1 << 8));
                        } else {
                            unsigned R = (aR & 0xffffu) + (aR >> 16), G = (aG & 0xffffu) + (aG >> 16), B = (aB & 0xffffu) + (aB >> 16);
                            R += __shfl_xor_sync(MVG_FULL, R, 4); G += __shfl_xor_sync(MVG_FULL, G, 4); B += __shfl_xor_sync(MVG_FULL, B, 4);
                            if constexpr (sl >= 3) {
                                R += __shfl_xor_sync(MVG_FULL, R, 8); G += __shfl_xor_sync(MVG_FULL, G, 8); B += __shfl_xor_sync(MVG_FULL, B, 8);
                                R += __shfl_xor_sync(MVG_FULL, R, 1); G += __shfl_xor_sync(MVG_FULL, G, 1); B += __shfl_xor_sync(MVG_FULL, B, 1);
                            }
                            if constexpr (sl == 4) {
                                R += __shfl_xor_sync(MVG_FULL, R, 16); G += __shfl_xor_sync(MVG_FULL, G, 16); B += __shfl_xor_sync(MVG_FULL, B, 16);
                                R += __shfl_xor_sync(MVG_FULL, R, 2); G += __shfl_xor_sync(MVG_FULL, G, 2); B += __shfl_xor_sync(MVG_FULL, B, 2);
                            }
                            const bool writer = sl == 2 ? !(q & 1) : sl == 3 ? !(q & 3) && !(h & 1) : lane == 0;
                            if (writer) {
                                constexpr unsigned rnd = 1u << (2 * sl - 1);
                                constexpr int qs = sl > 1 ? sl - 1 : 0, hs = sl > 2 ? sl - 2 : 0;
                                uint8_t *d = s.u.rgb + (q >> qs) * KF_RGBS_PITCH + (j * per + (h >> hs)) * 3;
                                d[0] = (uint8_t)((R + rnd) >> (2 * sl)); d[1] = (uint8_t)((G + rnd) >> (2 * sl)); d[2] = (uint8_t)((B + rnd) >> (2 * sl));
                            }
                        }
                    } else
#pragma unroll
                    for (int r = 0; r < 2; r++) {
                        const unsigned w = r ? y1 : y0;
                        const unsigned te = ((mvg_pair_even(w) * 149u) >> 7) & 0x01ff01ffu;
                        const unsigned to = ((mvg_pair_odd(w) * 149u) >> 7) & 0x01ff01ffu;
                        const unsigned Re = mvg_add_clip8x2(te, rC), Ro = mvg_add_clip8x2(to, rC);
                        const unsigned Ge = mvg_add_clip8x2(te, gC), Go = mvg_add_clip8x2(to, gC);
                        const unsigned Be = mvg_add_clip8x2(te, bC), Bo = mvg_add_clip8x2(to, bC);
                        const unsigned X = __byte_perm(Re, Ge, 0x6240);
                        const unsigned Y = __byte_perm(Be, Ro, 0x6240);
                        const unsigned Z = __byte_perm(Go, Bo, 0x6240);
                        unsigned *d = KF_WO_GROUP ? reinterpret_cast<unsigned *>(rgb_dst + r * 8 * KF_RGB_GSTRIDE + 48 * j)
                                                  : reinterpret_cast<unsigned *>(rgb_dst + r * KF_RGB_STRIDE + 48 * (j & 1));
                        d[0] = __byte_perm(X, Y, 0x5410);
                        d[1] = __byte_perm(Z, X, 0x7610);
                        d[2] = __byte_perm(Y, Z, 0x7632);
                    }
                }
                *cn_dst = *cn_src;
                __syncwarp();
                if (j < n_next && lane == 0) {
                    asm volatile("fence.proxy.async.shared::cta;" ::: "memory");
                    mvg_bulk_load(tile + j * KF_MBS, lv_row + (size_t)(mx + KF_GROUP) * 384, 768u, &s.mbar);
                }
                if (OUT == KF_OUT_RGBS && j == nmb - 1) {
                    constexpr int unit = sl <= 2 ? 4 : 1, ppr = KF_GROUP * per * 3 / unit, total = per * ppr;
#pragma unroll 1
                    for (int idx = lane; idx < total; idx += 32) {
                        const int r = idx / ppr, c = idx - r * ppr;
                        if (c * unit < nmb * per * 3) {
                            if (unit == 4) *reinterpret_cast<unsigned *>(wo_run + (size_t)r * opitch + 4 * c) = *reinterpret_cast<const unsigned *>(s.u.rgb + r * KF_RGBS_PITCH + 4 * c);
                            else wo_run[(size_t)r * opitch + c] = s.u.rgb[r * KF_RGBS_PITCH + c];
                        }
                    }
                    wo_run += KF_GROUP * per * 3;
                    __syncwarp();
                }
#if KF_WO_GROUP
                if (OUT == KF_OUT_RGB && j == nmb - 1) {
                    const int wc = lane & 3, ws = (lane >> 3) + 4 * ((lane >> 2) & 1);
                    const uint8_t *rd = s.u.rgb + ws * KF_RGB_GSTRIDE + wc * 16;
                    uint8_t *gd = wo_run + (size_t)(2 * ws) * pitch + wc * 16;
#pragma unroll
                    for (int hb = 0; hb < 2; hb++)
#pragma unroll
                        for (int m = 0; m < 3; m++)
                            if (4 * m + wc < 3 * nmb)
                                *reinterpret_cast<uint4 *>(gd + (size_t)hb * pitch + 64 * m) =
                                    *reinterpret_cast<const uint4 *>(rd + hb * 8 * KF_RGB_GSTRIDE + 64 * m);
                    wo_run += 192;
                    __syncwarp();
                }
#else
                if (OUT == KF_OUT_RGB && ((j & 1) || j == nmb - 1)) {
                    const int n_here = (j & 1) + 1;
#pragma unroll
                    for (int k = 0; k < 3; k++) {
                        const int ch = lane + 32 * k, r = ch / 6, col = ch - r * 6;
                        if (col < 3 * n_here) {
                            const uint4 v = *reinterpret_cast<const uint4 *>(s.u.rgb + r * KF_RGB_STRIDE + col * 16);
#ifdef KF_RGB_LINEAR
                            *reinterpret_cast<uint4 *>(p.rgb + (size_t)slot * ((size_t)n_mb * 768) + ((size_t)row * W + mx - (j & 1)) * 768 + ch * 16) = v;
#else
                            *reinterpret_cast<uint4 *>(wo_run + (size_t)r * pitch + col * 16) = v;
#endif
                        }
                    }
                    wo_run += 96;
                    __syncwarp();
                }
#endif
            }
        }
        KF_STAT(st[6] += clock64() - trow;)
    }
    KF_STAT(if (lane == 0 && p.stats) for (int i = 0; i < 8; i++) atomicAdd(p.stats + i, st[i]);)
#ifdef MVG_CHECKED
    __syncwarp();
    if (lane < 4) MVG_ASSERT(s.c0[lane] == MVG_CANARY_WORD && s.c1[lane] == MVG_CANARY_WORD && s.c2[lane] == MVG_CANARY_WORD && s.c3[lane] == MVG_CANARY_WORD, 2);
#endif
}
```

minivideo_b200/csrc/mvg_kernels.cuh:

```cuda
#pragma once

#include <cuda_runtime.h>
#include <stddef.h>
#include <stdint.h>

#include "mvg_internal.h"

#define MVG_FULL 0xffffffffu

#ifdef MVG_CHECKED
__device__ unsigned long long mvg_check_fail[8];
#define MVG_ASSERT(cond, slot) do { if (!(cond)) atomicAdd(&mvg_check_fail[slot], 1ull); } while (0)
#define MVG_CANARY(name) uint32_t name[4];
#define MVG_CANARY_WORD 0xC0DEC0DEu
#else
#define MVG_ASSERT(cond, slot) do { } while (0)
#define MVG_CANARY(name)
#endif


struct MvgTables {
    int32_t ls4[3][6][16];
    int32_t ls4q[3][52][16];
    int32_t ls8[6][64];
    uint8_t zz8inv[64];
    int32_t cb_qp_offset, cr_qp_offset;
};

__device__ __forceinline__ int mvg_clip8(int v) { return min(max(v, 0), 255); }

__device__ __forceinline__ int mvg_lane()
{
    int l;
    asm volatile("mov.u32 %0, %%laneid;" : "=r"(l));
    return l;
}

__device__ __forceinline__ int mvg_keep(int v) { asm volatile("" : "+r"(v)); return v; }
__device__ __forceinline__ unsigned mvg_keep(unsigned v) { asm volatile("" : "+r"(v)); return v; }

__constant__ unsigned char mvg_qpc_tab[22] = {29,30,31,32,32,33,34,34,35,35,36,36,37,37,37,38,38,38,39,39,39,39};

__device__ __forceinline__ int mvg_chroma_qp(int qp_y, int offset)
{
    const int qpi = min(max(qp_y + offset, 0), 51);
    return qpi < 30 ? qpi : (int)mvg_qpc_tab[qpi - 30];
}


struct K0Params {
    const uint32_t *nz_blocks, *word_off;
    const uint64_t *pic_base;
    const uint16_t *words;
    int16_t        *coeff;
    long long       n_mbs;
    int             mbs_per_pic;
};

__global__ void __launch_bounds__(256)
k0_expand_levels(K0Params p)
{
    const int lane = threadIdx.x & 31;
    const long long warp0 = ((long long)blockIdx.x * blockDim.x + threadIdx.x) >> 5;
    const long long n_warps = ((long long)gridDim.x * blockDim.x) >> 5;
    for (long long mb = warp0; mb < p.n_mbs; mb += n_warps) {
        const unsigned nzb = __ldg(p.nz_blocks + mb) & 0x00FFFFFFu;
        const long long pic = mb / p.mbs_per_pic;
        const uint16_t *w = p.words + __ldg(p.pic_base + pic) + __ldg(p.word_off + mb);
        const uint16_t *end = p.words + __ldg(p.pic_base + pic + 1);
        const bool coded = (nzb >> lane) & 1u;
        const uint16_t *mp = w + __popc(nzb & ((1u << lane) - 1u));
        const unsigned mask = (coded && mp < end) ? (unsigned)__ldg(mp) : 0u;
        int pre = __popc(mask);
#pragma unroll
        for (int o = 1; o < 32; o <<= 1) {
            const int t = __shfl_up_sync(MVG_FULL, pre, o);
            if (lane >= o) pre += t;
        }
        const uint16_t *lv = w + __popc(nzb) + pre - __popc(mask);
        unsigned out[8] = {0, 0, 0, 0, 0, 0, 0, 0};
        unsigned m = mask;
        while (m) {
            const int k = __ffs(m) - 1;
            m &= m - 1;
            const unsigned v = lv < end ? (unsigned)__ldg(lv) : 0u;
            lv++;
#pragma unroll
            for (int q = 0; q < 8; q++)
                if ((k >> 1) == q) out[q] |= v << (16 * (k & 1));
        }
        if (lane < 24) {
            uint4 *dst = reinterpret_cast<uint4 *>(p.coeff + mb * 384 + lane * 16);
            dst[0] = make_uint4(out[0], out[1], out[2], out[3]);
            dst[1] = make_uint4(out[4], out[5], out[6], out[7]);
        }
    }
}


struct K1Params {
    const uint8_t *mb_kind, *i16_mode, *chroma_mode, *luma_modes;
    const int8_t  *qp_y;
    const int16_t *coeff;
    int16_t       *resid;
    MvgMbCtl      *ctl;
    const MvgTables *tab;
    long long      n_mbs;
};

__device__ __forceinline__ void mvg_bfly4(int a, int b, int c, int d, int &o0, int &o1, int &o2, int &o3)
{
    int e0 = a + c, e1 = a - c, e2 = (b >> 1) - d, e3 = b + (d >> 1);
    o0 = e0 + e3; o1 = e1 + e2; o2 = e1 - e2; o3 = e0 - e3;
}

__device__ __forceinline__ void mvg_idct8_1d(int (&v)[8])
{
    int a0 = v[0] + v[4];
    int a1 = -v[3] + v[5] - v[7] - (v[7] >> 1);
    int a2 = v[0] - v[4];
    int a3 = v[1] + v[7] - v[3] - (v[3] >> 1);
    int a4 = (v[2] >> 1) - v[6];
    int a5 = -v[1] + v[7] + v[5] + (v[5] >> 1);
    int a6 = v[2] + (v[6] >> 1);
    int a7 = v[3] + v[5] + v[1] + (v[1] >> 1);
    int b0 = a0 + a6, b1 = a1 + (a7 >> 2), b2 = a2 + a4, b3 = a3 + (a5 >> 2);
    int b4 = a2 - a4, b5 = (a3 >> 2) - a5, b6 = a0 - a6, b7 = a7 - (a1 >> 2);
    v[0] = b0 + b7; v[1] = b2 + b5; v[2] = b4 + b3; v[3] = b6 + b1;
    v[4] = b6 - b1; v[5] = b4 - b3; v[6] = b2 - b5; v[7] = b0 - b7;
}

__device__ __forceinline__ unsigned mvg_pack_sat16(int hi, int lo)
{
    unsigned d;
    asm("cvt.pack.sat.s16.s32 %0, %1, %2;" : "=r"(d) : "r"(hi), "r"(lo));
    return d;
}
__device__ __forceinline__ unsigned mvg_pack_shr6(int hi, int lo)
{
    const unsigned t = ((mvg_pack_sat16(hi, lo) >> 6) & 0x03ff03ffu) ^ 0x02000200u;
    return __vsub2(t, 0x02000200u);
}

#define K1_WARPS 12
#define K1_GROUP 4
#define K1_TILE  (K1_GROUP * 384)

__device__ __forceinline__ uint32_t mvg_smem_u32(const void *p) { return (uint32_t)__cvta_generic_to_shared(p); }
__device__ __forceinline__ void mvg_mbar_init(uint64_t *bar, unsigned count)
{
    asm volatile("mbarrier.init.shared::cta.b64 [%0], %1;" :: "r"(mvg_smem_u32(bar)), "r"(count) : "memory");
}
__device__ __forceinline__ void mvg_mbar_expect_tx(uint64_t *bar, unsigned bytes)
{
    asm volatile("mbarrier.arrive.expect_tx.shared::cta.b64 _, [%0], %1;" :: "r"(mvg_smem_u32(bar)), "r"(bytes) : "memory");
}
__device__ __forceinline__ void mvg_mbar_wait(uint64_t *bar, unsigned parity)
{
    unsigned ok;
    do {
        asm volatile("{\n .reg .pred p;\n mbarrier.try_wait.parity.shared::cta.b64 p, [%1], %2;\n selp.u32 %0, 1, 0, p;\n}"
                     : "=r"(ok) : "r"(mvg_smem_u32(bar)), "r"(parity) : "memory");
    } while (!ok);
}
__device__ __forceinline__ void mvg_bulk_load(void *dst_smem, const void *src, unsigned bytes, uint64_t *bar)
{
    asm volatile("cp.async.bulk.shared::cluster.global.mbarrier::complete_tx::bytes [%0], [%1], %2, [%3];"
                 :: "r"(mvg_smem_u32(dst_smem)), "l"(src), "r"(bytes), "r"(mvg_smem_u32(bar)) : "memory");
}
__device__ __forceinline__ void mvg_bulk_store(void *dst, const void *src_smem, unsigned bytes)
{
    asm volatile("fence.proxy.async.shared::cta;" ::: "memory");
    asm volatile("cp.async.bulk.global.shared::cta.bulk_group [%0], [%1], %2;"
                 :: "l"(dst), "r"(mvg_smem_u32(src_smem)), "r"(bytes) : "memory");
    asm volatile("cp.async.bulk.commit_group;" ::: "memory");
}
__device__ __forceinline__ void mvg_bulk_wait_read() { asm volatile("cp.async.bulk.wait_group.read 0;" ::: "memory"); }

template <int G>
struct MvgXfScratch {
    int32_t  dc[G][24];
    int32_t  f1[G][16];
    int32_t  tr[4][8][9];
    uint32_t meta[G];
    int32_t  ls0[G];
    uint8_t  list4[G * 24 + 8];
    uint8_t  list8[G * 4 + 4];
};

struct MvgXfTables {
    int32_t  ls4[3 * 6 * 16];
    int32_t  ls4q[3 * 52 * 16];
    int32_t  ls8[6 * 64];
    __align__(8) uint8_t zz8inv[64];
    uint8_t  dcsh[52];
    uint16_t qpc[2][52];
};

struct K1WarpSmem {
    __align__(128) int16_t tile[2][K1_TILE];
    MvgXfScratch<K1_GROUP> x;
    __align__(8) uint64_t mbar[2];
};

__device__ __forceinline__ int mvg_blk_of(int bx, int by) { return (bx & 1) | ((by & 1) << 1) | ((bx >> 1) << 2) | ((by >> 1) << 3); }

__device__ __forceinline__ void mvg_xf_load_tables(MvgXfTables &t, const MvgTables *tab)
{
    const int tid = threadIdx.x, nt = blockDim.x;
    for (int i = tid; i < 3 * 6 * 16; i += nt) t.ls4[i] = (&tab->ls4[0][0][0])[i];
    for (int i = tid; i < 3 * 52 * 16; i += nt) t.ls4q[i] = (&tab->ls4q[0][0][0])[i];
    for (int i = tid; i < 6 * 64; i += nt) t.ls8[i] = (&tab->ls8[0][0])[i];
    for (int i = tid; i < 64; i += nt) t.zz8inv[i] = tab->zz8inv[i];
    for (int i = tid; i < 52; i += nt) t.dcsh[i] = (uint8_t)(i > 23 ? 0 : 4 - i / 6);
    for (int i = tid; i < 104; i += nt) {
        const int pl = i >= 52, qpc = mvg_chroma_qp(i - 52 * pl, pl ? tab->cr_qp_offset : tab->cb_qp_offset);
        t.qpc[pl][i - 52 * pl] = (uint16_t)(qpc | ((qpc / 6) << 8));
    }
}

struct MvgSideInfo {
    const uint8_t *src;
    int stride;
    __device__ __forceinline__ void init(int lane, const uint8_t *mb_kind, const uint8_t *i16_mode, const uint8_t *chroma_mode,
                                         const uint8_t *luma_modes, const int8_t *qp_y)
    {
        const int mt = lane & 7;
        src = mt < 4 ? luma_modes + 4 * mt : mt == 4 ? mb_kind : mt == 5 ? reinterpret_cast<const uint8_t *>(qp_y)
                     : mt == 6 ? i16_mode : chroma_mode;
        stride = mt < 4 ? 16 : 1;
    }
    __device__ __forceinline__ unsigned load(int lane, long long first, int n) const
    {
        unsigned v = 0u;
        if ((lane >> 3) < n) {
            const uint8_t *q = src + (first + (lane >> 3)) * stride;
            if ((lane & 7) < 4) v = __ldg(reinterpret_cast<const unsigned *>(q));
            else v = (unsigned)__ldg(q);
        }
        return v;
    }
};

template <int G, int MBS = 384>
__device__ __forceinline__ void mvg_xf_group(int16_t *tile, MvgXfScratch<G> &s, const MvgXfTables &T, unsigned meta, int nmb, int lane)
{
    const int mj = lane >> 3, mt = lane & 7;
    const int kind_j = (int)__shfl_sync(MVG_FULL, meta, (lane & ~7) + 4);
    const int qp_j = min(max((int)(signed char)__shfl_sync(MVG_FULL, meta, (lane & ~7) + 5), 0), 51);
    if (mt == 0 && mj < G) {
        const unsigned sh = T.dcsh[qp_j];
        s.meta[mj] = (unsigned)kind_j | ((unsigned)(qp_j & 255) << 8) | (sh << 16) | (((1u << sh) >> 1) << 24);
        s.ls0[mj] = T.ls4q[qp_j * 16];
    }

    if (mj < nmb) {
        const int16_t *cf = tile + mj * MBS;
        if (kind_j == MVG_MB_I16x16 && mt < 4) {
            const int a = cf[mvg_blk_of(0, mt) * 16], b = cf[mvg_blk_of(1, mt) * 16];
            const int c = cf[mvg_blk_of(2, mt) * 16], d = cf[mvg_blk_of(3, mt) * 16];
            int32_t *f1 = s.f1[mj] + mt * 4;
            f1[0] = a + b + c + d; f1[1] = a + b - c - d; f1[2] = a - b - c + d; f1[3] = a - b + c - d;
        } else if (mt == 4 || mt == 5) {
            const int pl = mt - 4;
            const int16_t *cc = cf + 256 + pl * 64;
            const int c00 = cc[0], c01 = cc[16], c10 = cc[32], c11 = cc[48];
            const int qe = T.qpc[pl][qp_j], qpc = qe & 255, qd = qe >> 8;
            const int ls00 = T.ls4[((pl + 1) * 6 + (qpc - 6 * qd)) * 16];
            const int f[4] = {c00 + c01 + c10 + c11, c00 - c01 + c10 - c11, c00 + c01 - c10 - c11, c00 - c01 - c10 + c11};
#pragma unroll
            for (int k = 0; k < 4; k++) s.dc[mj][16 + pl * 4 + k] = (int)((unsigned)(f[k] * ls00) << qd) >> 5;
        }
    }
    __syncwarp();
    if (mj < nmb && kind_j == MVG_MB_I16x16 && mt < 4) {
        const int32_t *f1 = s.f1[mj];
        const int a = f1[mt], b = f1[4 + mt], c = f1[8 + mt], d = f1[12 + mt];
        const int f[4] = {a + b + c + d, a + b - c - d, a - b - c + d, a - b + c - d};
        const int qd = qp_j / 6, ls00 = T.ls4[(qp_j - 6 * qd) * 16];
#pragma unroll
        for (int i = 0; i < 4; i++) {
            const int t = f[i] * ls00;
            s.dc[mj][mvg_blk_of(mt, i)] = (qp_j >= 36) ? (int)((unsigned)t << (qd - 6)) : ((t + (1 << (5 - qd))) >> (6 - qd));
        }
    }
    __syncwarp();

    int n4 = 0, n8 = 0;
#pragma unroll 1
    for (int r = 0; r < (G * 24 + 31) / 32; r++) {
        const int u = lane + 32 * r, j0 = G <= 4 ? r + (lane >= 24 - 8 * r) : u / 24, b = u - 24 * j0;
        const bool live = j0 < nmb;
        const int j = live ? j0 : 0;
        const unsigned mw = s.meta[j];
        const int kind = mw & 255;
        const bool is8 = kind == MVG_MB_I8x8 && b < 16;
        uint4 *blk = reinterpret_cast<uint4 *>(tile + j * MBS + b * 16);
        const int o = (lane >> 2) & 1;
        const uint4 wa = blk[o], wb = blk[o ^ 1];
        const unsigned x0 = o ? wb.x : wa.x, x4 = o ? wa.x : wb.x;
        const unsigned rest = (x0 & 0xffff0000u) | x4 | wa.y | wa.z | wa.w | wb.y | wb.z | wb.w;
        const int dcraw = (short)(x0 & 0xffff);
        const bool nz8q = live && is8 && (rest | (x0 & 0xffffu)) != 0;
        const bool general = live && !is8 && rest != 0;
        {
            const bool has_dc = b >= 16 || kind == MVG_MB_I16x16;
            const int sh = (mw >> 16) & 255;
            const int plain = (dcraw * s.ls0[j] + (int)(mw >> 24)) >> sh;
            const int d = has_dc ? s.dc[j][b] : plain;
            const int rv = min(max((d + 32) >> 6, -512), 511);
            if (live && !is8 && rest == 0 && (rv != 0 || dcraw != 0)) {
                const unsigned pk = (unsigned)(rv & 0xffff) * 0x10001u;
                blk[o] = make_uint4(pk, pk, pk, pk); blk[o ^ 1] = make_uint4(pk, pk, pk, pk);
            }
        }
        const unsigned gb = __ballot_sync(MVG_FULL, general);
        if (general) s.list4[n4 + __popc(gb & ((1u << lane) - 1))] = (uint8_t)u;
        n4 += __popc(gb);
        const unsigned qb = __ballot_sync(MVG_FULL, nz8q);
        const bool any8 = live && is8 && ((qb >> (lane & ~3)) & 0xFu) != 0;
        const bool lead8 = any8 && (lane & 3) == 0;
        const unsigned lb = __ballot_sync(MVG_FULL, lead8);
        if (lead8) s.list8[n8 + __popc(lb & ((1u << lane) - 1))] = (uint8_t)(j * 4 + (b >> 2));
        n8 += __popc(lb);
    }
    __syncwarp();

    for (int base = 0; base < n4; base += 32) {
        if (base + lane < n4) {
            const int u = s.list4[base + lane], j = u / 24, b = u - 24 * j;
            MVG_ASSERT(base + lane < G * 24 + 8 && j < nmb, 1);
            const unsigned mw = s.meta[j];
            const int kind = mw & 255, qp = (signed char)(mw >> 8);
            const int comp = b < 16 ? 0 : (b < 20 ? 1 : 2);
            const int qpb = comp ? (T.qpc[comp - 1][qp] & 255) : qp;
            uint4 *blk = reinterpret_cast<uint4 *>(tile + j * MBS + b * 16);
            const uint4 a = blk[0], bb = blk[1];
            int c[16];
            c[0] = (short)(a.x & 0xffff); c[1] = (int)a.x >> 16; c[4] = (short)(a.y & 0xffff); c[8] = (int)a.y >> 16;
            c[5] = (short)(a.z & 0xffff); c[2] = (int)a.z >> 16; c[3] = (short)(a.w & 0xffff); c[6] = (int)a.w >> 16;
            c[9] = (short)(bb.x & 0xffff); c[12] = (int)bb.x >> 16; c[13] = (short)(bb.y & 0xffff); c[10] = (int)bb.y >> 16;
            c[7] = (short)(bb.z & 0xffff); c[11] = (int)bb.z >> 16; c[14] = (short)(bb.w & 0xffff); c[15] = (int)bb.w >> 16;
            const bool keep_dc = comp != 0 || kind == MVG_MB_I16x16;
            const int dc_in = keep_dc ? s.dc[j][b] : 0;
            const int4 *lq = reinterpret_cast<const int4 *>(T.ls4q + (comp * 52 + qpb) * 16);
            const int4 l0 = lq[0], l1 = lq[1], l2 = lq[2], l3 = lq[3];
            const int ls[16] = {l0.x, l0.y, l0.z, l0.w, l1.x, l1.y, l1.z, l1.w, l2.x, l2.y, l2.z, l2.w, l3.x, l3.y, l3.z, l3.w};
            {
                const int sh = T.dcsh[qpb], rnd = (1 << sh) >> 1;
#pragma unroll
                for (int k = 0; k < 16; k++) c[k] = (c[k] * ls[k] + rnd) >> sh;
            }
            if (keep_dc) c[0] = dc_in;
            c[0] += 32;
#pragma unroll
            for (int i = 0; i < 4; i++)
                mvg_bfly4(c[4 * i], c[4 * i + 1], c[4 * i + 2], c[4 * i + 3], c[4 * i], c[4 * i + 1], c[4 * i + 2], c[4 * i + 3]);
#pragma unroll
            for (int q = 0; q < 4; q++)
                mvg_bfly4(c[q], c[4 + q], c[8 + q], c[12 + q], c[q], c[4 + q], c[8 + q], c[12 + q]);
            uint4 o0, o1;
            o0.x = mvg_pack_shr6(c[1], c[0]);   o0.y = mvg_pack_shr6(c[3], c[2]);
            o0.z = mvg_pack_shr6(c[5], c[4]);   o0.w = mvg_pack_shr6(c[7], c[6]);
            o1.x = mvg_pack_shr6(c[9], c[8]);   o1.y = mvg_pack_shr6(c[11], c[10]);
            o1.z = mvg_pack_shr6(c[13], c[12]); o1.w = mvg_pack_shr6(c[15], c[14]);
            blk[0] = o0; blk[1] = o1;
        }
    }

    for (int base = 0; base < n8; base += 4) {
        const int slot = base + (lane >> 3), row = lane & 7;
        const bool act = slot < n8;
        int v[8];
        int16_t *o8 = tile;
        if (act) {
            const int id = s.list8[slot], j = id >> 2, b8 = id & 3;
            MVG_ASSERT(slot < G * 4 + 4 && j < nmb, 1);
            const int qp = (signed char)(s.meta[j] >> 8);
            const int qd8 = qp / 6;
            const int32_t *l8 = T.ls8 + (qp - 6 * qd8) * 64 + row * 8;
            const int16_t *in = tile + j * MBS + b8 * 64;
            const uint2 zz = *reinterpret_cast<const uint2 *>(T.zz8inv + row * 8);
#pragma unroll
            for (int q = 0; q < 8; q++) {
                const unsigned k = ((q < 4 ? zz.x : zz.y) >> (8 * (q & 3))) & 255u;
                v[q] = (int)in[k] * l8[q];
            }
            {
                const int up = max(qd8 - 6, 0), down = max(6 - qd8, 0), rnd = (1 << down) >> 1, mul = 1 << up;
#pragma unroll
                for (int q = 0; q < 8; q++) v[q] = (v[q] * mul + rnd) >> down;
            }
            if (row == 0) v[0] += 32;
            mvg_idct8_1d(v);
#pragma unroll
            for (int q = 0; q < 8; q++) s.tr[lane >> 3][row][q] = v[q];
            o8 = tile + j * MBS + (b8 * 4 + (row >> 2)) * 16 + (row & 3);
        }
        __syncwarp();
        if (act) {
#pragma unroll
            for (int i = 0; i < 8; i++) v[i] = s.tr[lane >> 3][i][row];
            mvg_idct8_1d(v);
#pragma unroll
            for (int i = 0; i < 8; i++) o8[(i >> 2) * 32 + (i & 3) * 4] = (int16_t)min(max(v[i] >> 6, -512), 511);
        }
        __syncwarp();
    }
    __syncwarp();
}

__device__ __forceinline__ uint4 mvg_ctl_from_meta(unsigned meta)
{
    const unsigned nib = (meta & 0xF) | ((meta >> 4) & 0xF0) | ((meta >> 8) & 0xF00) | ((meta >> 12) & 0xF000);
    const unsigned n1 = __shfl_down_sync(MVG_FULL, nib, 1), n2 = __shfl_down_sync(MVG_FULL, nib, 2);
    const unsigned n3 = __shfl_down_sync(MVG_FULL, nib, 3);
    const unsigned k4 = __shfl_down_sync(MVG_FULL, meta, 4), k6 = __shfl_down_sync(MVG_FULL, meta, 6);
    const unsigned k7 = __shfl_down_sync(MVG_FULL, meta, 7);
    return make_uint4((k4 & 255) | ((k6 & 255) << 8) | ((k7 & 255) << 16), nib | (n2 << 16),
                      __funnelshift_l(n1 | (n3 << 16), n1 | (n3 << 16), 8), 0u);
}

__global__ void __launch_bounds__(K1_WARPS * 32, 2)
k1_dequant_idct(K1Params p)
{
    __shared__ MvgXfTables s_tab;
    extern __shared__ __align__(128) uint8_t k1_smem[];
    K1WarpSmem *s_warp = reinterpret_cast<K1WarpSmem *>(k1_smem);
    mvg_xf_load_tables(s_tab, p.tab);

    const int lane = mvg_lane();
    K1WarpSmem &s = s_warp[threadIdx.x >> 5];
    if (lane == 0) { mvg_mbar_init(&s.mbar[0], 1); mvg_mbar_init(&s.mbar[1], 1); }
    asm volatile("fence.mbarrier_init.release.cluster;" ::: "memory");
    asm volatile("fence.proxy.async.shared::cta;" ::: "memory");
    __syncthreads();

    const long long n_groups = (p.n_mbs + K1_GROUP - 1) / K1_GROUP;
    const long long stride = (long long)gridDim.x * K1_WARPS;
    long long g = (long long)blockIdx.x * K1_WARPS + (threadIdx.x >> 5);

    MvgSideInfo side;
    side.init(lane, p.mb_kind, p.i16_mode, p.chroma_mode, p.luma_modes, p.qp_y);
    auto issue_load = [&](int buf, long long grp) {
        const long long mb0 = grp * K1_GROUP;
        const unsigned bytes = (unsigned)min((long long)K1_GROUP, p.n_mbs - mb0) * 768u;
        mvg_mbar_expect_tx(&s.mbar[buf], bytes);
        mvg_bulk_load(s.tile[buf], p.coeff + mb0 * 384, bytes, &s.mbar[buf]);
    };

    unsigned nmeta = 0;
    if (g < n_groups) {
        if (lane == 0) issue_load(0, g);
        nmeta = side.load(lane, g * K1_GROUP, (int)min((long long)K1_GROUP, p.n_mbs - g * K1_GROUP));
    }
    unsigned parity = 0;

    for (int it = 0; g < n_groups; g += stride, it++) {
        const int buf = it & 1;
        const unsigned meta = nmeta;
        {
            const long long gn = g + stride;
            if (gn < n_groups) {
                if (lane == 0) { mvg_bulk_wait_read(); issue_load(buf ^ 1, gn); }
                nmeta = side.load(lane, gn * K1_GROUP, (int)min((long long)K1_GROUP, p.n_mbs - gn * K1_GROUP));
            }
        }
        const long long mb0 = g * K1_GROUP;
        const int nmb = (int)min((long long)K1_GROUP, p.n_mbs - mb0);
        int16_t *tile = s.tile[buf];

        mvg_mbar_wait(&s.mbar[buf], (parity >> buf) & 1u);
        parity ^= 1u << buf;

        mvg_xf_group<K1_GROUP>(tile, s.x, s_tab, meta, nmb, lane);

        if (lane == 0) mvg_bulk_store(p.resid + mb0 * 384, tile, (unsigned)nmb * 768u);
        {
            const uint4 rec = mvg_ctl_from_meta(meta);
            if ((lane & 7) == 0 && (lane >> 3) < nmb) *reinterpret_cast<uint4 *>(p.ctl + mb0 + (lane >> 3)) = rec;
        }
        __syncwarp();
    }
    if (lane == 0) mvg_bulk_wait_read();
}


struct K2Params {
    const int16_t  *resid;
    const MvgMbCtl *ctl;
    uint8_t        *tiles;
    uint2          *halo;
    int            *work;
    const MvgLuts  *luts;
    unsigned        epoch;
    int w_mbs, h_mbs, first_slot, n_pics, group;
    unsigned long long *stats;
    unsigned        sel[4];
};

#ifdef MVG_K2_PROFILE
#define K2_PROF(...) __VA_ARGS__
#else
#define K2_PROF(...)
#endif
#ifndef K2_POLL_NS
#define K2_POLL_NS   100
#endif
#ifndef K2_WARPS
#define K2_WARPS     16
#endif
#define K2_CTL_CHUNK 32
#define K2_RING      4
#define K2_TO(x, y)  (((y) + 1) * MVG_LT_STRIDE + MVG_LT_XOFF + (x))
#define K2_CO(x, y)  (((y) + 1) * MVG_CT_STRIDE + MVG_CT_XOFF + (x))

struct K2WarpSmem {
    __align__(16) MvgMbCtl ctl[2 * K2_CTL_CHUNK];
    MVG_CANARY(c0)
    __align__(16) int16_t  resid[K2_RING][384];
    MVG_CANARY(c1)
    __align__(16) uint8_t  lt[MVG_LT_ROWS * MVG_LT_STRIDE];
    __align__(16) uint8_t  ct[2][MVG_CT_PLANE];
    MVG_CANARY(c2)
    __align__(16) uint8_t  n8[MVG_N8_BYTES];
    MVG_CANARY(c3)
};

#define K2_LUT_BYTES  ((sizeof(MvgLuts) + 127) / 128 * 128)
#define K2_SMEM_BYTES (sizeof(K2WarpSmem) * K2_WARPS + 2048 + K2_LUT_BYTES)

__device__ __forceinline__ void mvg_cp_async16(void *dst_smem, const void *src)
{
    asm volatile("cp.async.cg.shared.global [%0], [%1], 16;" :: "r"(mvg_smem_u32(dst_smem)), "l"(src) : "memory");
}
__device__ __forceinline__ void mvg_cp_async_commit() { asm volatile("cp.async.commit_group;" ::: "memory"); }
template <int N>
__device__ __forceinline__ void mvg_cp_async_wait() { asm volatile("cp.async.wait_group %0;" :: "n"(N) : "memory"); }

__device__ __forceinline__ uint2 mvg_ld_relaxed_u64(const uint2 *p)
{
    unsigned long long v;
    asm volatile("ld.relaxed.gpu.global.u64 %0, [%1];" : "=l"(v) : "l"(p) : "memory");
    return make_uint2((unsigned)v, (unsigned)(v >> 32));
}
__device__ __forceinline__ uint4 mvg_ld_relaxed_2u64(const uint4 *p)
{
    unsigned long long a, b;
    asm volatile("ld.relaxed.gpu.global.v2.u64 {%0, %1}, [%2];" : "=l"(a), "=l"(b) : "l"(p) : "memory");
    return make_uint4((unsigned)a, (unsigned)(a >> 32), (unsigned)b, (unsigned)(b >> 32));
}
__device__ __forceinline__ void mvg_st_relaxed_u64(uint2 *p, unsigned lo, unsigned hi)
{
    const unsigned long long v = (unsigned long long)lo | ((unsigned long long)hi << 32);
    asm volatile("st.relaxed.gpu.global.u64 [%0], %1;" :: "l"(p), "l"(v) : "memory");
}

__device__ __forceinline__ int mvg_sum4(unsigned w) { return (int)__dp4a(w, 0x01010101u, 0u); }
__device__ __forceinline__ int mvg_add_clip8(int pred, int r) { return __viaddmin_s32_relu(pred, r, 255); }
__device__ __forceinline__ unsigned mvg_add_clip8x2(unsigned pred2, unsigned r2) { return __viaddmin_s16x2_relu(pred2, r2, 0x00ff00ffu); }
__device__ __forceinline__ unsigned mvg_pair_lo(unsigned w) { return __byte_perm(w, 0, 0x4140); }
__device__ __forceinline__ unsigned mvg_pair_hi(unsigned w) { return __byte_perm(w, 0, 0x4342); }
__device__ __forceinline__ unsigned mvg_pairs_to_bytes(unsigned a, unsigned b) { return __byte_perm(a, b, 0x6420); }

struct K2Ctx {
#ifdef MVG_CHECKED
    const uint8_t *rec_lo, *rec_hi;
#endif
    uint8_t *lt, *ct;
    uint8_t *n8;
    const uint8_t *resid;
    const uint8_t *lut8;
    int lane;
    unsigned lut4;
    int s4;
    int r4odd, r4even;
    unsigned h4;
    unsigned m4c, m4b, m4cc;
    const unsigned *sel;
    int n8tr, n8notr;
    int s8;
    unsigned fixA, fixB, fixD;
};

__device__ __forceinline__ void k2_luma16(const K2Ctx &c, int mode, bool left, bool up)
{
    uint8_t *lt = c.lt;
    const int lane = c.lane, p = lane >> 2;
    const int x0 = (p & 2) * 4, y = ((p & 1) + (p >> 2) * 2) * 4 + (lane & 3);
    unsigned pp[4];
    if (mode == 0) {
        const uint2 t = *reinterpret_cast<const uint2 *>(lt + K2_TO(0, -1) + x0);
        pp[0] = mvg_pair_lo(t.x); pp[1] = mvg_pair_hi(t.x); pp[2] = mvg_pair_lo(t.y); pp[3] = mvg_pair_hi(t.y);
    } else if (mode == 1) {
        pp[0] = pp[1] = pp[2] = pp[3] = (unsigned)lt[K2_TO(-1, 0) + y * MVG_LT_STRIDE] * 0x10001u;
    } else if (mode == 2) {
        int v = 0;
        if (lane < 16) { if (left) v = lt[K2_TO(-1, 0) + lane * MVG_LT_STRIDE]; }
        else if (lane < 20) { if (up) v = mvg_sum4(*reinterpret_cast<const unsigned *>(lt + K2_TO(0, -1) + (lane - 16) * 4)); }
#pragma unroll
        for (int o = 16; o > 0; o >>= 1) v += __shfl_xor_sync(MVG_FULL, v, o);
        v = (left && up) ? (v + 16) >> 5 : (left || up) ? (v + 8) >> 4 : 128;
        pp[0] = pp[1] = pp[2] = pp[3] = (unsigned)v * 0x10001u;
    } else {
        int term = 0;
        const int i = lane & 7;
        if (lane < 8)       term = (i + 1) * ((int)lt[K2_TO(8 + i, -1)] - (int)lt[K2_TO(6 - i, -1)]);
        else if (lane < 16) term = (i + 1) * ((int)lt[K2_TO(-1, 8 + i)] - (int)lt[K2_TO(-1, 6 - i)]);
#pragma unroll
        for (int o = 4; o > 0; o >>= 1) term += __shfl_xor_sync(MVG_FULL, term, o);
        const int H = __shfl_sync(MVG_FULL, term, 0), V = __shfl_sync(MVG_FULL, term, 8);
        const int a = 16 * ((int)lt[K2_TO(-1, 15)] + (int)lt[K2_TO(15, -1)]);
        const int b = (5 * H + 32) >> 6, cc = (5 * V + 32) >> 6;
        const int v0 = a + cc * (y - 7) + 16 + b * (x0 - 7);
        unsigned pair = __vadd2((unsigned)(v0 & 0xffff) * 0x10001u, (unsigned)b << 16);
        const unsigned step = (unsigned)((2 * b) & 0xffff) * 0x10001u;
#pragma unroll
        for (int k = 0; k < 4; k++) {
            pp[k] = (__vimin_s16x2_relu(pair, 0x1fff1fffu) >> 5) & 0x00ff00ffu;
            pair = __vadd2(pair, step);
        }
    }
    const uint8_t *r = c.resid + (lane >> 2) * 64 + (lane & 3) * 8;
    const uint2 ra = *reinterpret_cast<const uint2 *>(r);
    const uint2 rb = *reinterpret_cast<const uint2 *>(r + 32);
    const unsigned lo = mvg_pairs_to_bytes(mvg_add_clip8x2(pp[0], ra.x), mvg_add_clip8x2(pp[1], ra.y));
    const unsigned hi = mvg_pairs_to_bytes(mvg_add_clip8x2(pp[2], rb.x), mvg_add_clip8x2(pp[3], rb.y));
    *reinterpret_cast<uint2 *>(lt + K2_TO(0, 0) + y * MVG_LT_STRIDE + x0) = make_uint2(lo, hi);
}

template <int T>
__device__ __forceinline__ void k2_luma4_step(const K2Ctx &c, unsigned seq, unsigned dcsteps)
{
    constexpr int bx0 = T & 1, by0 = T >> 1;
    constexpr bool v0 = T <= 7, v1 = T >= 2;
    constexpr int org1 = K2_TO(bx0 * 4 + 8, by0 * 4 - 4);
    constexpr int blk0 = (bx0 & 1) | ((by0 & 1) << 1) | ((bx0 >> 1) << 2) | ((by0 >> 1) << 3);
    constexpr int sh = 4 * (T & 7);
    const unsigned m = (sh >= 7 ? (seq >> (sh >= 7 ? sh - 7 : 0)) : (seq << (sh >= 7 ? 0 : 7 - sh))) & 0x780u;
    unsigned e;
    asm("ld.shared.u32 %0, [%1];" : "=r"(e) : "r"(m | c.lut4));
    const uint8_t *nb = c.lt + (org1 - MVG_LUT4_BIAS);
#ifdef MVG_CHECKED
#pragma unroll
    for (int k = 0; k < 4; k++) {
        const uint8_t *a = nb + __dp4a(e, c.sel[k], c.h4);
        MVG_ASSERT(a >= c.rec_lo && a < c.rec_hi, 0);
    }
#endif
    int sum = (int)nb[__dp4a(e, c.sel[0], c.h4)] + (int)nb[__dp4a(e, c.sel[1], c.h4)] +
              (int)nb[__dp4a(e, c.sel[2], c.h4)] + (int)nb[__dp4a(e, c.sel[3], c.h4)] + 2;
#ifdef MVG_CHECKED
    {
        const uint8_t *a = c.resid + blk0 * 32 + ((by0 & 1) ? c.r4odd : c.r4even);
        MVG_ASSERT(a >= c.rec_lo && a + 2 <= c.rec_hi, 0);
    }
#endif
    int shift = 2;
    if (dcsteps & (1u << T)) {
        const int other = __shfl_xor_sync(MVG_FULL, sum, 1);
        if (m == 0x100u) { sum += other; shift = 3; }
    }
    const int r = *reinterpret_cast<const int16_t *>(c.resid + blk0 * 32 + ((by0 & 1) ? c.r4odd : c.r4even));
    const int v = mvg_add_clip8(sum >> shift, r);
    if ((v0 && v1) || (c.lane >= 16 ? v1 : v0)) c.lt[org1 + c.s4] = (uint8_t)v;
    __syncwarp();
}

__device__ __forceinline__ unsigned k2_dc_nibbles(unsigned seq)
{
    return (seq >> 1) & ~seq & ~(seq >> 2) & ~(seq >> 3) & 0x11111111u;
}

__device__ __forceinline__ void k2_luma4(const K2Ctx &c, unsigned w1, unsigned w2, bool availA, bool availB, bool availC)
{
    const bool half = c.lane >= 16;
    unsigned seq = half ? w2 : w1;
    const unsigned notr = c.m4c | (availB ? 0u : c.m4b) | (availC ? 0u : c.m4cc);
    seq |= (seq & (seq >> 1) & notr) << 3;
    if (!availA || !availB) {
        const unsigned d = k2_dc_nibbles(seq);
        unsigned top = 0, left = 0;
        if (!availB) top = half ? 0x00001100u : (availA ? 0x00000011u : 0x00000010u);
        if (!availA && !half) left = availB ? 0x01010101u : 0x01010100u;
        seq |= (d & top) << 3;
        seq ^= (d & left) * 0xBu;
        if (!availA && !availB) {
            if (c.lane < 4) c.lt[K2_TO(-1, 0) + c.lane * MVG_LT_STRIDE] = 128;
            if (c.lane == 4) *reinterpret_cast<unsigned *>(c.lt + K2_TO(0, -1)) = 0x80808080u;
            __syncwarp();
        }
    }
    unsigned dcsteps;
    {
        const unsigned d = k2_dc_nibbles(seq);
        unsigned bits = (((d | (d >> 3)) & 0x03030303u) * 0x01041040u) >> 24;
        if (half) bits = (bits & 0xfcu) | ((bits & 3u) << 8);
        dcsteps = __reduce_or_sync(MVG_FULL, bits);
    }
    k2_luma4_step<0>(c, seq, dcsteps);
    k2_luma4_step<1>(c, seq, dcsteps);
    k2_luma4_step<2>(c, seq, dcsteps);
    k2_luma4_step<3>(c, seq, dcsteps);
    k2_luma4_step<4>(c, seq, dcsteps);
    k2_luma4_step<5>(c, seq, dcsteps);
    k2_luma4_step<6>(c, seq, dcsteps);
    k2_luma4_step<7>(c, seq, dcsteps);
    k2_luma4_step<8>(c, seq, dcsteps);
    k2_luma4_step<9>(c, seq, dcsteps);
}

template <int B8>
__device__ __forceinline__ void k2_luma8_block(const K2Ctx &c, unsigned modes, unsigned fix, bool availA, bool availB, bool availC)
{
    uint8_t *lt = c.lt;
    const int lane = c.lane;
    constexpr int xo = (B8 & 1) * 8, yo = (B8 >> 1) * 8;
    constexpr int org = K2_TO(xo, yo);
    const unsigned mode = (modes >> (4 * B8)) & 15u;
    const bool left = (B8 & 1) ? true : availA, up = (B8 & 2) ? true : availB;
    const bool tr = B8 == 0 ? availB : (B8 == 1 ? availC : (B8 == 2));

    const int raw = lt[org + (tr ? c.n8tr : c.n8notr)];
    int prev = __shfl_up_sync(MVG_FULL, raw, 1), next = __shfl_down_sync(MVG_FULL, raw, 1);
    if (B8 != 3) {
        if (fix & (1u << (2 * B8))) next = raw;
        if (fix & (2u << (2 * B8))) prev = raw;
    }
    const int filt = (prev + 2 * raw + next + 2) >> 2;
    const int fp = __shfl_up_sync(MVG_FULL, filt, 1);
    int fn = __shfl_down_sync(MVG_FULL, filt, 1);
    if (lane == 24) fn = filt;
    const int f2 = (filt + fn + 1) >> 1, f3 = (fp + 2 * filt + fn + 2) >> 2;
    reinterpret_cast<unsigned *>(c.n8)[lane] = (unsigned)filt | ((unsigned)f2 << 8) | ((unsigned)f3 << 16);
    if (mode == 2) {
        int v = 0;
        if (lane < 8 && left) v = filt;
        if (lane >= 9 && lane < 17 && up) v = filt;
#pragma unroll
        for (int o = 16; o > 0; o >>= 1) v += __shfl_xor_sync(MVG_FULL, v, o);
        v = (left && up) ? (v + 8) >> 4 : (left || up) ? (v + 4) >> 3 : 128;
        if (lane == 0) c.n8[MVG_N8_DC] = (uint8_t)v;
    }
    __syncwarp();
    const unsigned e = *reinterpret_cast<const unsigned *>(c.lut8 + mode * 128);
    MVG_ASSERT(mode < 16 && (e & 0xffffu) < MVG_N8_BYTES && (e >> 16) < MVG_N8_BYTES, 3);
    const unsigned pp = (unsigned)c.n8[e & 0xffffu] | ((unsigned)c.n8[e >> 16] << 16);
    const unsigned r2 = *reinterpret_cast<const unsigned *>(c.resid + B8 * 128 + lane * 4);
    *reinterpret_cast<uint16_t *>(lt + org + c.s8) = (uint16_t)__byte_perm(mvg_add_clip8x2(pp, r2), 0, 0x4420);
    __syncwarp();
}

__device__ __forceinline__ void k2_luma8_block_rt(const K2Ctx &c, int b8, unsigned modes, unsigned fix, bool availA, bool availB, bool availC)
{
    uint8_t *lt = c.lt;
    const int lane = c.lane;
    const int org = K2_TO(0, 0) + (b8 & 1) * 8 + (b8 >> 1) * 8 * MVG_LT_STRIDE;
    const unsigned mode = (modes >> (4 * b8)) & 15u;
    const bool left = (b8 & 1) ? true : availA, up = (b8 & 2) ? true : availB;
    const bool tr = b8 == 0 ? availB : (b8 == 1 ? availC : (b8 == 2));

    const int raw = lt[org + (tr ? c.n8tr : c.n8notr)];
    int prev = __shfl_up_sync(MVG_FULL, raw, 1), next = __shfl_down_sync(MVG_FULL, raw, 1);
    {
        const unsigned f2 = b8 == 3 ? 0u : fix >> (2 * b8);
        if (f2 & 1u) next = raw;
        if (f2 & 2u) prev = raw;
    }
    const int filt = (prev + 2 * raw + next + 2) >> 2;
    const int fp = __shfl_up_sync(MVG_FULL, filt, 1);
    int fn = __shfl_down_sync(MVG_FULL, filt, 1);
    if (lane == 24) fn = filt;
    const int f2 = (filt + fn + 1) >> 1, f3 = (fp + 2 * filt + fn + 2) >> 2;
    reinterpret_cast<unsigned *>(c.n8)[lane] = (unsigned)filt | ((unsigned)f2 << 8) | ((unsigned)f3 << 16);
    if (mode == 2) {
        int v = 0;
        if (lane < 8 && left) v = filt;
        if (lane >= 9 && lane < 17 && up) v = filt;
#pragma unroll
        for (int o = 16; o > 0; o >>= 1) v += __shfl_xor_sync(MVG_FULL, v, o);
        v = (left && up) ? (v + 8) >> 4 : (left || up) ? (v + 4) >> 3 : 128;
        if (lane == 0) c.n8[MVG_N8_DC] = (uint8_t)v;
    }
    __syncwarp();
    const unsigned e = *reinterpret_cast<const unsigned *>(c.lut8 + mode * 128);
    const unsigned pp = (unsigned)c.n8[e & 0xffffu] | ((unsigned)c.n8[e >> 16] << 16);
    const unsigned r2 = *reinterpret_cast<const unsigned *>(c.resid + b8 * 128 + lane * 4);
    *reinterpret_cast<uint16_t *>(lt + org + c.s8) = (uint16_t)__byte_perm(mvg_add_clip8x2(pp, r2), 0, 0x4420);
    __syncwarp();
}

template <bool COMPACT = false>
__device__ __forceinline__ void k2_luma8(const K2Ctx &c, unsigned modes, bool availA, bool availB, bool availC, bool availD)
{
    const unsigned fix = (availA ? 0u : c.fixA) | (availB ? 0u : c.fixB) | (availD ? 0u : c.fixD);
    if (COMPACT) {
#pragma unroll 1
        for (int b8 = 0; b8 < 4; b8++) k2_luma8_block_rt(c, b8, modes, fix, availA, availB, availC);
        return;
    }
    k2_luma8_block<0>(c, modes, fix, availA, availB, availC);
    k2_luma8_block<1>(c, modes, fix, availA, availB, availC);
    k2_luma8_block<2>(c, modes, fix, availA, availB, availC);
    k2_luma8_block<3>(c, modes, fix, availA, availB, availC);
}

__device__ __forceinline__ void k2_chroma(const K2Ctx &c, int mode, bool left, bool up)
{
    const int lane = c.lane, pl = lane >> 4;
    const int x0 = (lane & 4), yo = (lane & 8) >> 1, y = yo + (lane & 3);
    uint8_t *ct = c.ct + pl * MVG_CT_PLANE;
    unsigned p0, p1;
    if (mode == 0) {
        int st = 0, sl = 0;
        if (up) st = mvg_sum4(*reinterpret_cast<const unsigned *>(ct + K2_CO(0, -1) + x0));
        if (left) sl = (int)ct[K2_CO(-1, 0) + yo * MVG_CT_STRIDE] + (int)ct[K2_CO(-1, 1) + yo * MVG_CT_STRIDE] +
                       (int)ct[K2_CO(-1, 2) + yo * MVG_CT_STRIDE] + (int)ct[K2_CO(-1, 3) + yo * MVG_CT_STRIDE];
        int v;
        if (!left && !up) v = 128;
        else if ((x0 == 0) == (yo == 0))
            v = (left && up) ? (st + sl + 4) >> 3 : left ? (sl + 2) >> 2 : (st + 2) >> 2;
        else if (x0 > 0) v = up ? (st + 2) >> 2 : (sl + 2) >> 2;
        else v = left ? (sl + 2) >> 2 : (st + 2) >> 2;
        p0 = p1 = (unsigned)v * 0x10001u;
    } else if (mode == 1) {
        p0 = p1 = (unsigned)ct[K2_CO(-1, 0) + y * MVG_CT_STRIDE] * 0x10001u;
    } else if (mode == 2) {
        const unsigned t = *reinterpret_cast<const unsigned *>(ct + K2_CO(0, -1) + x0);
        p0 = mvg_pair_lo(t); p1 = mvg_pair_hi(t);
    } else {
        const int i = lane & 3, g = (lane >> 2) & 3;
        const int step = g == 0 ? 1 : MVG_CT_STRIDE;
        const int mid = g == 0 ? K2_CO(3, -1) : K2_CO(-1, 3);
        const int term = (g < 2 ? i + 1 : 0) * ((int)ct[mid + (i + 1) * step] - (int)ct[mid - (i + 1) * step]);
        int sum = term + __shfl_xor_sync(MVG_FULL, term, 1);
        sum += __shfl_xor_sync(MVG_FULL, sum, 2);
        const int H = __shfl_sync(MVG_FULL, sum, lane & 16), V = __shfl_sync(MVG_FULL, sum, (lane & 16) + 4);
        const int a = 16 * ((int)ct[K2_CO(-1, 7)] + (int)ct[K2_CO(7, -1)]);
        const int b = (34 * H + 32) >> 6, cc = (34 * V + 32) >> 6;
        const int v0 = a + cc * (y - 3) + 16 + b * (x0 - 3);
        const unsigned pair = __vadd2((unsigned)(v0 & 0xffff) * 0x10001u, (unsigned)b << 16);
        p0 = (__vimin_s16x2_relu(pair, 0x1fff1fffu) >> 5) & 0x00ff00ffu;
        p1 = (__vimin_s16x2_relu(__vadd2(pair, (unsigned)((2 * b) & 0xffff) * 0x10001u), 0x1fff1fffu) >> 5) & 0x00ff00ffu;
    }
    const uint2 r = *reinterpret_cast<const uint2 *>(c.resid + 512 + lane * 8);
    *reinterpret_cast<unsigned *>(ct + K2_CO(0, 0) + y * MVG_CT_STRIDE + x0) =
        mvg_pairs_to_bytes(mvg_add_clip8x2(p0, r.x), mvg_add_clip8x2(p1, r.y));
}

__global__ void __launch_bounds__(K2_WARPS * 32, 2)
k2_wavefront(K2Params p)
{
    extern __shared__ __align__(128) uint8_t k2_smem[];
    const int lane = mvg_lane();
    const unsigned wid = __shfl_sync(MVG_FULL, threadIdx.x >> 5, 0);
    const unsigned base = mvg_smem_u32(k2_smem);
    const unsigned lut_addr = (base + 2047u) & ~2047u;
    const unsigned n_before = (lut_addr - base) / (unsigned)sizeof(K2WarpSmem);
    MvgLuts *luts = reinterpret_cast<MvgLuts *>(k2_smem + (lut_addr - base));
    K2WarpSmem &s = *reinterpret_cast<K2WarpSmem *>(
        wid < n_before ? k2_smem + wid * sizeof(K2WarpSmem)
                       : k2_smem + (lut_addr - base) + K2_LUT_BYTES + (wid - n_before) * sizeof(K2WarpSmem));
    for (int i = threadIdx.x; i < (int)(K2_LUT_BYTES / 16); i += blockDim.x)
        reinterpret_cast<uint4 *>(luts)[i] = __ldg(reinterpret_cast<const uint4 *>(p.luts) + i);
    __syncthreads();

    const int W = p.w_mbs, H = p.h_mbs, n_mb = W * H;
    const int total = p.n_pics * H;
    const unsigned epoch = p.epoch;

    K2Ctx c;
#ifdef MVG_CHECKED
    c.rec_lo = reinterpret_cast<const uint8_t *>(&s); c.rec_hi = c.rec_lo + sizeof(K2WarpSmem);
    if (lane < 4) s.c0[lane] = s.c1[lane] = s.c2[lane] = s.c3[lane] = MVG_CANARY_WORD;
    __syncwarp();
#endif
    c.lt = s.lt; c.ct = &s.ct[0][0]; c.n8 = s.n8; c.lut8 = reinterpret_cast<const uint8_t *>(&luts->lut8[0][lane]);
    c.lane = lane;
    c.sel = p.sel;
    c.resid = reinterpret_cast<const uint8_t *>(s.resid[0]);
    {
        const int half = lane >> 4, pix = lane & 15, px = pix & 3, py = pix >> 2;
        c.lut4 = lut_addr + (unsigned)lane * 4u;
        c.h4 = half ? 0u : (unsigned)(4 * MVG_LT_STRIDE - 8);
        c.s4 = py * MVG_LT_STRIDE + px + (int)c.h4;
        c.r4odd = pix * 2 + (half ? 64 : 0);
        c.r4even = pix * 2 + (half ? -64 : 0);
        c.m4c = half ? 0x10100010u : 0x10001000u;
        c.m4b = half ? 0x00000100u : 0x00000011u;
        c.m4cc = half ? 0x00001000u : 0u;
        const int n = lane < 25 ? lane : 24;
        if (n < 8)       c.n8tr = (7 - n) * MVG_LT_STRIDE - 1;
        else if (n == 8) c.n8tr = -MVG_LT_STRIDE - 1;
        else             c.n8tr = -MVG_LT_STRIDE + (n - 9);
        c.n8notr = n > 16 ? -MVG_LT_STRIDE + 7 : c.n8tr;
        const int x8 = ((lane >> 3) & 1) * 4 + (lane & 1) * 2, y8 = (lane >> 4) * 4 + ((lane >> 1) & 3);
        c.s8 = y8 * MVG_LT_STRIDE + x8;
        c.fixA = lane == 7 ? 0x10u : lane == 8 ? 0x22u : lane == 9 ? 0x20u : 0u;
        c.fixB = lane == 7 ? 0x04u : lane == 8 ? 0x05u : lane == 9 ? 0x08u : 0u;
        c.fixD = lane == 7 ? 0x01u : lane == 9 ? 0x02u : 0u;
    }
    uint8_t *const halo_top = lane < 4 ? s.lt + K2_TO(lane * 4, -1)
                            : lane < 8 ? s.ct[(lane >> 1) & 1] + K2_CO((lane & 1) * 4, -1)
                                       : s.lt + K2_TO(16 + (lane & 1) * 4, -1);
    const uint8_t *const halo_bot = lane < 4 ? halo_top + 16 * MVG_LT_STRIDE : halo_top + 8 * MVG_CT_STRIDE;
    const uint8_t *const wo_src = lane < 16 ? s.lt + K2_TO(0, lane)
                                            : s.ct[(lane >> 3) & 1] + K2_CO(0, lane & 7);
    const int wo_off = lane < 16 ? lane * 16 : 256 + (lane - 16) * 8;
    uint8_t *const lc_dst = lane < 16 ? s.lt + K2_TO(-1, lane) : s.ct[(lane >> 3) & 1] + K2_CO(-1, lane & 7);
    const unsigned lc_sel = lane < 16 ? 7u : 3u;
    const uint8_t *const cn_src = (lane == 3 || lane == 5 || lane == 7) ? halo_top + 3 : s.lt;
    uint8_t *const cn_dst = lane == 3 ? s.lt + K2_TO(-1, -1) : lane == 5 ? s.ct[0] + K2_CO(-1, -1)
                          : lane == 7 ? s.ct[1] + K2_CO(-1, -1) : s.lt;
    uint8_t *const st_dst = reinterpret_cast<uint8_t *>(s.resid[0]) + lane * 16;

    K2_PROF(long long pc[8] = {0, 0, 0, 0, 0, 0, 0, 0}; long long pt0 = clock64();)

    for (;;) {
        K2_PROF(const long long tr0 = clock64();)
        int item = 0;
        if (lane == 0) item = atomicAdd(p.work, 1);
        item = __shfl_sync(MVG_FULL, item, 0);
        if (item >= total) break;
        const int g = item / (p.group * H);
        const int gsize = min(p.group, p.n_pics - g * p.group);
        const int within = item - g * p.group * H;
        const int row = within / gsize;
        const int slot = p.first_slot + g * p.group + (within - row * gsize);
        const size_t mb0 = (size_t)slot * n_mb + (size_t)row * W;

        const uint8_t *st_src = reinterpret_cast<const uint8_t *>(p.resid + mb0 * 384) + lane * 16;
        const MvgMbCtl *ctl = p.ctl + mb0;
        if (lane < W) mvg_cp_async16(&s.ctl[lane], ctl + lane);
        mvg_cp_async16(st_dst, st_src);
        if (W > 1) { mvg_cp_async16(st_dst + 512, st_src + 512); mvg_cp_async16(st_dst + 1024, st_src + 1024); }
        else if (lane < 16) mvg_cp_async16(st_dst + 512, st_src + 512);
        mvg_cp_async_commit();

        const uint8_t *st_run = st_src + 2 * 768;
        uint8_t *wo_run = p.tiles + mb0 * 384 + wo_off;
        uint2 *hm_run = p.halo + mb0 * 8 + lane;
        const uint2 *ha_run = p.halo + (mb0 - W) * 8 + lane;
        const bool availB = row > 0, publish = row < H - 1;
        const int hwords = W * 8;
        uint2 qa = make_uint2(0, epoch), qb = make_uint2(0, epoch);
        if (availB) {
            if (lane < hwords) qb = mvg_ld_relaxed_u64(ha_run);
        }
        unsigned okA = 0;

        K2_PROF(pc[0] += clock64() - tr0;)
        for (int c0 = 0; c0 < W; c0 += K2_CTL_CHUNK) {
            if (c0 + K2_CTL_CHUNK + lane < W)
                mvg_cp_async16(&s.ctl[(c0 + K2_CTL_CHUNK + lane) & (2 * K2_CTL_CHUNK - 1)], ctl + c0 + K2_CTL_CHUNK + lane);
            const int cend = min(c0 + K2_CTL_CHUNK, W);
            for (int mx = c0; mx < cend; mx++) {
                K2_PROF(const long long t0 = clock64();)
                const int j = mx & 3;
                if ((mx & 1) == 0) {
                    const int left = W - (mx + 2);
                    uint8_t *d = st_dst + ((mx + 2) & (K2_RING - 1)) * 768;
                    if (left >= 2) {
                        mvg_cp_async16(d, st_run); mvg_cp_async16(d + 512, st_run + 512); mvg_cp_async16(d + 1024, st_run + 1024);
                    } else if (left == 1) {
                        mvg_cp_async16(d, st_run);
                        if (lane < 16) mvg_cp_async16(d + 512, st_run + 512);
                    }
                    st_run += 2 * 768;
                    mvg_cp_async_commit();
                }
                const bool availA = mx > 0, availC = availB && mx < W - 1, availD = availA && availB;

                if (availB) {
                    if (j == 0) {
                        qa = qb;
                        okA = __ballot_sync(MVG_FULL, qa.y == epoch);
                    }
                    const unsigned need = availC ? 0x3FFu : 0xFFu;
                    unsigned have = __funnelshift_r(okA, j == 3 ? __ballot_sync(MVG_FULL, qb.y == epoch) : 0u, 8 * j);
                    K2_PROF(const long long th = clock64();)
                    if ((have & need) != need) {
                        K2_PROF(pc[5]++;)
                        unsigned ns = K2_POLL_NS;
                        do {
                            K2_PROF(pc[6]++;)
                            __nanosleep(ns);
                            if (ns < 8 * K2_POLL_NS) ns *= 2;
                            if ((mx & ~3) * 8 + lane < hwords) qa = mvg_ld_relaxed_u64(ha_run);
                            if ((mx & ~3) * 8 + 32 + lane < hwords) qb = mvg_ld_relaxed_u64(ha_run + 32);
                            okA = __ballot_sync(MVG_FULL, qa.y == epoch);
                            have = __funnelshift_r(okA, __ballot_sync(MVG_FULL, qb.y == epoch), 8 * j);
                        } while ((have & need) != need);
                    }
                    K2_PROF(pc[7] += clock64() - th;)
                    const unsigned src = (j == 3 && lane < 2) ? qb.x : qa.x;
                    const unsigned v = __shfl_sync(MVG_FULL, src, (8 * j + lane) & 31);
                    if (lane < 10) *reinterpret_cast<unsigned *>(halo_top) = v;
                    if (j == 3) ha_run += 32;
                }
                K2_PROF(const long long t1 = clock64();)
                mvg_cp_async_wait<1>();
                __syncwarp();
                if (availB && j == 0) {
                    qb = make_uint2(0, epoch);
                    if (mx * 8 + 32 + lane < hwords) qb = mvg_ld_relaxed_u64(ha_run + 32);
                }
                K2_PROF(const long long t2 = clock64();)
                c.resid = reinterpret_cast<const uint8_t *>(s.resid[mx & (K2_RING - 1)]);
                const uint4 ctlw = *reinterpret_cast<const uint4 *>(&s.ctl[mx & (2 * K2_CTL_CHUNK - 1)]);

                const int kind = ctlw.x & 255, i16 = (ctlw.x >> 8) & 255, cmode = (ctlw.x >> 16) & 255;
                if (kind == MVG_MB_I16x16)    k2_luma16(c, i16, availA, availB);
                else if (kind == MVG_MB_I4x4) k2_luma4(c, ctlw.y, ctlw.z, availA, availB, availC);
                else                          k2_luma8(c, ctlw.y, availA, availB, availC, availD);
                k2_chroma(c, cmode, availA, availB);
                __syncwarp();
                K2_PROF(const long long t3 = clock64();)

                const uint2 wa = *reinterpret_cast<const uint2 *>(wo_src);
                uint2 wb = make_uint2(0u, 0u);
                if (lane < 16) {
                    wb = *reinterpret_cast<const uint2 *>(wo_src + 8);
                    *reinterpret_cast<uint4 *>(wo_run) = make_uint4(wa.x, wa.y, wb.x, wb.y);
                } else *reinterpret_cast<uint2 *>(wo_run) = wa;
                wo_run += 384;
                if (publish && lane < 8)
                    mvg_st_relaxed_u64(hm_run, *reinterpret_cast<const unsigned *>(halo_bot), epoch);
                hm_run += 8;
                *lc_dst = (uint8_t)__byte_perm(wa.y, wb.y, lc_sel);
                *cn_dst = *cn_src;
                __syncwarp();
                K2_PROF(const long long t4 = clock64(); pc[1] += t1 - t0; pc[2] += t2 - t1; pc[3] += t3 - t2; pc[4] += t4 - t3;)
            }
        }
        mvg_cp_async_wait<0>();
    }
    K2_PROF(if (lane == 0 && p.stats) { for (int i = 0; i < 8; i++) atomicAdd(p.stats + i, (unsigned long long)pc[i]); atomicAdd(p.stats + 8, (unsigned long long)(clock64() - pt0)); })
#ifdef MVG_CHECKED
    __syncwarp();
    if (lane < 4) MVG_ASSERT(s.c0[lane] == MVG_CANARY_WORD && s.c1[lane] == MVG_CANARY_WORD && s.c2[lane] == MVG_CANARY_WORD && s.c3[lane] == MVG_CANARY_WORD, 2);
#endif
}


struct K3Params {
    const uint8_t *tiles;
    uint8_t       *rgb;
    uint8_t       *yuv;
    int width, height, scale, first_slot, n_pics;
};

__device__ __forceinline__ void mvg_ycc_to_rgb(int Y, int Cb, int Cr, int &R, int &G, int &B)
{
    const int t = (298 * Y) >> 8;
    R = mvg_clip8(t + ((408 * Cr) >> 8) - 222);
    G = mvg_clip8(t - ((100 * Cb) >> 8) - ((208 * Cr) >> 8) + 135);
    B = mvg_clip8(t + ((516 * Cb) >> 8) - 276);
}

__device__ __forceinline__ unsigned mvg_pair_even(unsigned w) { return __byte_perm(w, 0, 0x4240); }
__device__ __forceinline__ unsigned mvg_pair_odd(unsigned w)  { return __byte_perm(w, 0, 0x4341); }

#define K3_MBS   32
#define K3_TILE  400
__global__ void __launch_bounds__(256)
k3_rgb_full(K3Params p)
{
    __shared__ __align__(16) uint8_t s_tiles[K3_MBS * K3_TILE];
    const int w_mbs = p.width >> 4, h_mbs = p.height >> 4, n_mb = w_mbs * h_mbs;
    const long long total_mbs = (long long)n_mb * p.n_pics;
    const long long n_groups = (total_mbs + K3_MBS - 1) / K3_MBS;
    const int lane = threadIdx.x & 31, q = threadIdx.x >> 5;
    const size_t ysz = (size_t)p.width * p.height;
    const uint8_t *tiles = p.tiles + (size_t)p.first_slot * n_mb * 384;
    uint8_t *rgb = p.rgb + (size_t)p.first_slot * ysz * 3;
    long long mb = (long long)blockIdx.x * K3_MBS + lane;
    int pic = (int)(mb / n_mb), my = (int)((mb - (long long)pic * n_mb) / w_mbs), mx = (int)(mb - (long long)pic * n_mb - (long long)my * w_mbs);
    const long long stride = (long long)gridDim.x * K3_MBS;
    const int dpic = (int)(stride / n_mb), dmy = (int)((stride - (long long)dpic * n_mb) / w_mbs),
              dmx = (int)(stride - (long long)dpic * n_mb - (long long)dmy * w_mbs);
    for (long long g = blockIdx.x; g < n_groups; g += gridDim.x, mb += stride) {
        {
            const long long first = g * K3_MBS;
            const int n_chunks = (int)min((long long)K3_MBS, total_mbs - first) * 24;
            const uint4 *src = reinterpret_cast<const uint4 *>(tiles + (size_t)first * 384);
#pragma unroll
            for (int k = 0; k < 3; k++) {
                const int ch = threadIdx.x + 256 * k;
                if (ch < n_chunks) {
                    const int t = ch / 24;
                    *reinterpret_cast<uint4 *>(s_tiles + t * K3_TILE + (ch - t * 24) * 16) = __ldg(src + ch);
                }
            }
        }
        __syncthreads();
        if (mb < total_mbs) {
            const uint8_t *tile = s_tiles + lane * K3_TILE;
            const uint4 y0 = *reinterpret_cast<const uint4 *>(tile + q * 32);
            const uint4 y1 = *reinterpret_cast<const uint4 *>(tile + q * 32 + 16);
            const uint2 cb = *reinterpret_cast<const uint2 *>(tile + 256 + q * 8);
            const uint2 cr = *reinterpret_cast<const uint2 *>(tile + 320 + q * 8);
            const unsigned yw[2][4] = {{y0.x, y0.y, y0.z, y0.w}, {y1.x, y1.y, y1.z, y1.w}};
            const unsigned cbw[2] = {cb.x, cb.y}, crw[2] = {cr.x, cr.y};
            unsigned out[2][12];
#pragma unroll
            for (int k = 0; k < 4; k++) {
                const unsigned cb2 = (k & 1) ? mvg_pair_hi(cbw[k >> 1]) : mvg_pair_lo(cbw[k >> 1]);
                const unsigned cr2 = (k & 1) ? mvg_pair_hi(crw[k >> 1]) : mvg_pair_lo(crw[k >> 1]);
                const unsigned rC = __vsub2(((cr2 * 204u) >> 7) & 0x01ff01ffu, 0x00de00deu);
                const unsigned bC = __vsub2(((cb2 * 129u) >> 6) & 0x03ff03ffu, 0x01140114u);
                const unsigned gC = __vsub2(__vsub2(0x00870087u, ((cb2 * 25u) >> 6) & 0x00ff00ffu),
                                            ((cr2 * 13u) >> 4) & 0x00ff00ffu);
#pragma unroll
                for (int r = 0; r < 2; r++) {
                    const unsigned w = yw[r][k];
                    const unsigned te = ((mvg_pair_even(w) * 149u) >> 7) & 0x01ff01ffu;
                    const unsigned to = ((mvg_pair_odd(w) * 149u) >> 7) & 0x01ff01ffu;
                    const unsigned Re = mvg_add_clip8x2(te, rC), Ro = mvg_add_clip8x2(to, rC);
                    const unsigned Ge = mvg_add_clip8x2(te, gC), Go = mvg_add_clip8x2(to, gC);
                    const unsigned Be = mvg_add_clip8x2(te, bC), Bo = mvg_add_clip8x2(to, bC);
                    const unsigned X = __byte_perm(Re, Ge, 0x6240);
                    const unsigned Y = __byte_perm(Be, Ro, 0x6240);
                    const unsigned Z = __byte_perm(Go, Bo, 0x6240);
                    out[r][3 * k]     = __byte_perm(X, Y, 0x5410);
                    out[r][3 * k + 1] = __byte_perm(Z, X, 0x7610);
                    out[r][3 * k + 2] = __byte_perm(Y, Z, 0x7632);
                }
            }
#pragma unroll
            for (int r = 0; r < 2; r++) {
                uint4 *dst = reinterpret_cast<uint4 *>(rgb + (size_t)pic * ysz * 3 +
                                                       ((size_t)(my * 16 + 2 * q + r) * p.width + mx * 16) * 3);
                dst[0] = make_uint4(out[r][0], out[r][1], out[r][2], out[r][3]);
                dst[1] = make_uint4(out[r][4], out[r][5], out[r][6], out[r][7]);
                dst[2] = make_uint4(out[r][8], out[r][9], out[r][10], out[r][11]);
            }
        }
        mx += dmx; my += dmy; pic += dpic;
        if (mx >= w_mbs) { mx -= w_mbs; my++; }
        if (my >= h_mbs) { my -= h_mbs; pic++; }
        __syncthreads();
    }
}

__global__ void __launch_bounds__(256)
k3_rgb_scaled_generic(K3Params p)
{
    const int s = p.scale, ow = p.width / s, oh = p.height / s;
    const long long per_pic = (long long)ow * oh, total = per_pic * p.n_pics;
    const size_t ysz = (size_t)p.width * p.height;
    const int area = s * s, w_mbs = p.width >> 4;
    for (long long g = (long long)blockIdx.x * blockDim.x + threadIdx.x; g < total; g += (long long)gridDim.x * blockDim.x) {
        const int pic = (int)(g / per_pic);
        const long long rem = g - (long long)pic * per_pic;
        const int oy = (int)(rem / ow), ox = (int)(rem - (long long)oy * ow);
        const size_t slot = (size_t)(p.first_slot + pic);
        const uint8_t *tiles = p.tiles + slot * (ysz * 3 / 2);
        int aR = 0, aG = 0, aB = 0;
        for (int dy = 0; dy < s; dy++) {
            const int py = oy * s + dy;
            for (int dx = 0; dx < s; dx++) {
                const int px = ox * s + dx;
                const uint8_t *tile = tiles + ((size_t)(py >> 4) * w_mbs + (px >> 4)) * 384;
                const int co = ((py & 15) >> 1) * 8 + ((px & 15) >> 1);
                int R, G, B;
                mvg_ycc_to_rgb(__ldg(tile + (py & 15) * 16 + (px & 15)), __ldg(tile + 256 + co), __ldg(tile + 320 + co), R, G, B);
                aR += R; aG += G; aB += B;
            }
        }
        uint8_t *o = p.rgb + slot * ((size_t)ow * oh * 3) + ((size_t)oy * ow + ox) * 3;
        o[0] = (uint8_t)((aR + area / 2) / area);
        o[1] = (uint8_t)((aG + area / 2) / area);
        o[2] = (uint8_t)((aB + area / 2) / area);
    }
}

__global__ void __launch_bounds__(256)
k3_rgb_scaled(K3Params p)
{
    __shared__ __align__(16) uint8_t s_tiles[K3_MBS * K3_TILE];
    const int w_mbs = p.width >> 4, h_mbs = p.height >> 4, n_mb = w_mbs * h_mbs;
    const long long total_mbs = (long long)n_mb * p.n_pics;
    const long long n_groups = (total_mbs + K3_MBS - 1) / K3_MBS;
    const int sc = p.scale, ow = p.width / sc, oh = p.height / sc;
    const int sh = sc == 2 ? 2 : sc == 4 ? 4 : sc == 8 ? 6 : 8;
    const size_t out_pic = (size_t)ow * oh * 3;
    const uint8_t *tiles = p.tiles + (size_t)p.first_slot * n_mb * 384;
    uint8_t *rgb = p.rgb + (size_t)p.first_slot * out_pic;
    for (long long g = blockIdx.x; g < n_groups; g += gridDim.x) {
        const long long first = g * K3_MBS;
        const int n_here = (int)min((long long)K3_MBS, total_mbs - first);
        {
            const uint4 *src = reinterpret_cast<const uint4 *>(tiles + (size_t)first * 384);
#pragma unroll
            for (int k = 0; k < 3; k++) {
                const int ch = threadIdx.x + 256 * k;
                if (ch < n_here * 24) {
                    const int t = ch / 24;
                    *reinterpret_cast<uint4 *>(s_tiles + t * K3_TILE + (ch - t * 24) * 16) = __ldg(src + ch);
                }
            }
        }
        __syncthreads();
#pragma unroll
        for (int half = 0; half < 2; half++) {
            const int cell = threadIdx.x + 256 * half;
            const int mbl = cell >> 4, cz = cell & 15;
            const int cx = (cz & 1) | ((cz >> 1) & 2), cy = ((cz >> 1) & 1) | ((cz >> 2) & 2);
            const bool live = mbl < n_here;
            unsigned sumR = 0, sumG = 0, sumB = 0;
            unsigned q2[2][2][3];
            if (live) {
                const uint8_t *tile = s_tiles + mbl * K3_TILE;
                const unsigned cbp = *reinterpret_cast<const uint16_t *>(tile + 256 + (cy * 2) * 8 + cx * 2) |
                                     (unsigned)*reinterpret_cast<const uint16_t *>(tile + 256 + (cy * 2 + 1) * 8 + cx * 2) << 16;
                const unsigned crp = *reinterpret_cast<const uint16_t *>(tile + 320 + (cy * 2) * 8 + cx * 2) |
                                     (unsigned)*reinterpret_cast<const uint16_t *>(tile + 320 + (cy * 2 + 1) * 8 + cx * 2) << 16;
#pragma unroll
                for (int qy = 0; qy < 2; qy++) {
                    const unsigned cb2 = qy ? mvg_pair_hi(cbp) : mvg_pair_lo(cbp);
                    const unsigned cr2 = qy ? mvg_pair_hi(crp) : mvg_pair_lo(crp);
                    const unsigned rC = __vsub2(((cr2 * 204u) >> 7) & 0x01ff01ffu, 0x00de00deu);
                    const unsigned bC = __vsub2(((cb2 * 129u) >> 6) & 0x03ff03ffu, 0x01140114u);
                    const unsigned gC = __vsub2(__vsub2(0x00870087u, ((cb2 * 25u) >> 6) & 0x00ff00ffu), ((cr2 * 13u) >> 4) & 0x00ff00ffu);
                    unsigned aR = 0, aG = 0, aB = 0;
#pragma unroll
                    for (int r = 0; r < 2; r++) {
                        const unsigned w = *reinterpret_cast<const unsigned *>(tile + (cy * 4 + qy * 2 + r) * 16 + cx * 4);
                        const unsigned te = ((mvg_pair_even(w) * 149u) >> 7) & 0x01ff01ffu;
                        const unsigned to = ((mvg_pair_odd(w) * 149u) >> 7) & 0x01ff01ffu;
                        aR += mvg_add_clip8x2(te, rC) + mvg_add_clip8x2(to, rC);
                        aG += mvg_add_clip8x2(te, gC) + mvg_add_clip8x2(to, gC);
                        aB += mvg_add_clip8x2(te, bC) + mvg_add_clip8x2(to, bC);
                    }
                    q2[qy][0][0] = aR & 0xffffu; q2[qy][1][0] = aR >> 16;
                    q2[qy][0][1] = aG & 0xffffu; q2[qy][1][1] = aG >> 16;
                    q2[qy][0][2] = aB & 0xffffu; q2[qy][1][2] = aB >> 16;
                    sumR += aR; sumG += aG; sumB += aB;
                }
            }
            const long long mb = first + mbl;
            const int pic = (int)(mb / n_mb), rem = (int)(mb - (long long)pic * n_mb), my = rem / w_mbs, mx = rem - my * w_mbs;
            uint8_t *out = rgb + (size_t)pic * out_pic;
            if (sc == 2) {
                if (live) {
#pragma unroll
                    for (int qy = 0; qy < 2; qy++)
#pragma unroll
                        for (int qx = 0; qx < 2; qx++) {
                            uint8_t *o = out + ((size_t)(my * 8 + cy * 2 + qy) * ow + mx * 8 + cx * 2 + qx) * 3;
                            o[0] = (uint8_t)((q2[qy][qx][0] + 2) >> 2);
                            o[1] = (uint8_t)((q2[qy][qx][1] + 2) >> 2);
                            o[2] = (uint8_t)((q2[qy][qx][2] + 2) >> 2);
                        }
                }
            } else {
                unsigned R = (sumR & 0xffffu) + (sumR >> 16), G = (sumG & 0xffffu) + (sumG >> 16), B = (sumB & 0xffffu) + (sumB >> 16);
                const int span = sc == 4 ? 1 : sc == 8 ? 4 : 16;
                for (int o = 1; o < span; o <<= 1) {
                    R += __shfl_xor_sync(MVG_FULL, R, o); G += __shfl_xor_sync(MVG_FULL, G, o); B += __shfl_xor_sync(MVG_FULL, B, o);
                }
                if (live && (cz & (span - 1)) == 0) {
                    const int per = 16 / sc;
                    const int ox = sc == 4 ? cx : sc == 8 ? cx >> 1 : 0, oy = sc == 4 ? cy : sc == 8 ? cy >> 1 : 0;
                    uint8_t *o = out + ((size_t)(my * per + oy) * ow + mx * per + ox) * 3;
                    const unsigned rnd = 1u << (sh - 1);
                    o[0] = (uint8_t)((R + rnd) >> sh);
                    o[1] = (uint8_t)((G + rnd) >> sh);
                    o[2] = (uint8_t)((B + rnd) >> sh);
                }
            }
        }
        __syncthreads();
    }
}

__global__ void __launch_bounds__(256)
k4_yuv_planar(K3Params p)
{
    const int w_mbs = p.width >> 4, h_mbs = p.height >> 4;
    const long long per_pic = (long long)w_mbs * h_mbs * 12;
    const long long total = per_pic * p.n_pics;
    const size_t ysz = (size_t)p.width * p.height;
    for (long long g = (long long)blockIdx.x * blockDim.x + threadIdx.x; g < total; g += (long long)gridDim.x * blockDim.x) {
        const int pic = (int)(g / per_pic);
        const int rem = (int)(g - (long long)pic * per_pic);
        const int line = rem / w_mbs, mx = rem - line * w_mbs;
        const int my = line / 12, piece = line - my * 12;
        const size_t slot = (size_t)(p.first_slot + pic);
        const uint8_t *tile = p.tiles + slot * (ysz * 3 / 2) + ((size_t)my * w_mbs + mx) * 384;
        uint8_t *Y = p.yuv + slot * (ysz * 3 / 2);
        if (piece < 8) {
            const uint4 a = __ldg(reinterpret_cast<const uint4 *>(tile + piece * 32));
            const uint4 b = __ldg(reinterpret_cast<const uint4 *>(tile + piece * 32 + 16));
            uint8_t *d = Y + (size_t)(my * 16 + piece * 2) * p.width + mx * 16;
            *reinterpret_cast<uint4 *>(d) = a;
            *reinterpret_cast<uint4 *>(d + p.width) = b;
        } else {
            const int q = piece - 8;
            const uint4 cb = __ldg(reinterpret_cast<const uint4 *>(tile + 256 + q * 16));
            const uint4 cr = __ldg(reinterpret_cast<const uint4 *>(tile + 320 + q * 16));
            const int cw = p.width >> 1;
            uint8_t *d = Y + ysz + (size_t)(my * 8 + q * 2) * cw + mx * 8;
            *reinterpret_cast<uint2 *>(d) = make_uint2(cb.x, cb.y);
            *reinterpret_cast<uint2 *>(d + cw) = make_uint2(cb.z, cb.w);
            d += ysz / 4;
            *reinterpret_cast<uint2 *>(d) = make_uint2(cr.x, cr.y);
            *reinterpret_cast<uint2 *>(d + cw) = make_uint2(cr.z, cr.w);
        }
    }
}
```

Measured before the change: 174,500.

## Use coded-block-pattern to skip loading and reconstructing empty residual blocks

Derives a per-macroblock CBP byte in the level-expansion kernel (or memset to all-present when absent) and feeds it into the fused reconstruction kernel's metadata. Bulk loads of coefficient tiles are split into per-8x8/chroma pieces and only issued for coded pieces, with explicit expect_tx and a final arrive. The transform stage skips loading zero blocks and returns per-block presence masks, which the prediction stages use to skip residual shared-memory reads. This trades fewer memory transfers and smem loads for extra mask bookkeeping, ballots and more complex mbarrier accounting.

Measured after the change: 130,300 (median of 6 runs). 25.3% lower.

```diff
diff --git a/minivideo_b200/csrc/mvg_api.cu b/minivideo_b200/csrc/mvg_api.cu
--- a/minivideo_b200/csrc/mvg_api.cu
+++ b/minivideo_b200/csrc/mvg_api.cu
@@ -506,6 +506,7 @@
     CK(ctx, cudaMemcpyAsync(ctx->d_cm + o, b->chroma_mode + s, cnt, cudaMemcpyHostToDevice, st));
     CK(ctx, cudaMemcpyAsync(ctx->d_qp + o, b->qp_y + s, cnt, cudaMemcpyHostToDevice, st));
     if (b->cbp) CK(ctx, cudaMemcpyAsync(ctx->d_cbp + o, b->cbp + s, cnt, cudaMemcpyHostToDevice, st));
+    else CK(ctx, cudaMemsetAsync(ctx->d_cbp + o, 0x2F, cnt, st));
     CK(ctx, cudaMemcpyAsync(ctx->d_modes + o * 16, b->luma_modes + s * 16, cnt * 16, cudaMemcpyHostToDevice, st));
     CK(ctx, cudaMemcpyAsync(ctx->d_coeff + o * 384, b->coeff + s * 384, cnt * 768, cudaMemcpyHostToDevice, st));
     return MVG_SUCCESS;
@@ -639,7 +640,7 @@
     if (fused) {
         KFParams p;
         p.mb_kind = ctx->d_kind; p.i16_mode = ctx->d_i16; p.chroma_mode = ctx->d_cm; p.luma_modes = ctx->d_modes;
-        p.qp_y = ctx->d_qp; p.coeff = ctx->d_coeff; p.tiles = ctx->d_tiles; p.rgb = ctx->d_rgb; p.halo = ctx->d_halo;
+        p.qp_y = ctx->d_qp; p.cbp = ctx->d_cbp; p.coeff = ctx->d_coeff; p.tiles = ctx->d_tiles; p.rgb = ctx->d_rgb; p.halo = ctx->d_halo;
         p.work = work; p.tab = ctx->d_tab; p.luts = ctx->d_luts; p.epoch = ctx->epoch;
         p.w_mbs = W; p.h_mbs = H; p.first_slot = first_slot; p.n_pics = n_pics; p.group = MVG_K2_GROUP;
         p.sel[0] = 1u; p.sel[1] = 1u << 8; p.sel[2] = 1u << 16; p.sel[3] = 1u << 24;
@@ -1043,7 +1044,7 @@
         K0Params p;
         const size_t o = (size_t)slot0 * n;
         p.nz_blocks = ctx->d_nzb + o; p.word_off = ctx->d_woff + o; p.pic_base = ctx->d_picbase + 2 * (size_t)slot0;
-        p.words = ctx->d_words; p.coeff = ctx->d_coeff + o * 384; p.n_mbs = (long long)cnt * (long long)n; p.mbs_per_pic = (int)n;
+        p.words = ctx->d_words; p.coeff = ctx->d_coeff + o * 384; p.cbp = ctx->d_cbp + o; p.n_mbs = (long long)cnt * (long long)n; p.mbs_per_pic = (int)n;
         const long long warps = p.n_mbs;
         const int grid = (int)std::min<long long>((warps + 7) / 8, (long long)ctx->sm_count * 16);
         k0_expand_levels<<<grid, 256, 0, ctx->stream>>>(p);
diff --git a/minivideo_b200/csrc/mvg_fused.cuh b/minivideo_b200/csrc/mvg_fused.cuh
--- a/minivideo_b200/csrc/mvg_fused.cuh
+++ b/minivideo_b200/csrc/mvg_fused.cuh
@@ -45,6 +45,7 @@
 struct KFParams {
     const uint8_t *mb_kind, *i16_mode, *chroma_mode, *luma_modes;
     const int8_t  *qp_y;
+    const uint8_t *cbp;
     const int16_t *coeff;
     uint8_t       *tiles;
     uint8_t       *rgb;
@@ -86,6 +87,20 @@
     uint8_t pad[KF_REC_PAD];
 #endif
 };
+
+__device__ __forceinline__ void kf_copy_piece(int16_t *slot, const int16_t *src, int k, unsigned w, uint64_t *bar)
+{
+    const bool need = k < 4 ? (((w >> (8 + k)) & 1u) != 0 || (w & 255u) == MVG_MB_I16x16) : ((w >> 12) & 15u) != 0;
+    if (need) {
+        const unsigned bytes = k < 4 ? 128u : 256u;
+        asm volatile("fence.proxy.async.shared::cta;" ::: "memory");
+        mvg_mbar_expect_tx_only(bar, bytes);
+        mvg_bulk_load(slot + k * 64, src + k * 64, bytes, bar);
+    }
+#ifdef MVG_CHECKED
+    else for (int i = 0; i < (k < 4 ? 8 : 16); i++) reinterpret_cast<uint4 *>(slot + k * 64)[i] = make_uint4(0x5A5A5A5Au, 0x5A5A5A5Au, 0x5A5A5A5Au, 0x5A5A5A5Au);
+#endif
+}
 
 #define KF_LUT_BYTES  ((sizeof(MvgLuts) + 127) / 128 * 128)
 #define KF_TAB_BYTES  ((sizeof(MvgXfTables) + 127) / 128 * 128)
@@ -211,7 +226,7 @@
             if (KF_MBS == 384) mvg_bulk_load(s.tile, lv_row, (unsigned)n0 * 768u, &s.mbar);
             else for (int j = 0; j < n0; j++) mvg_bulk_load(s.tile + j * KF_MBS, lv_row + j * 384, 768u, &s.mbar);
         }
-        unsigned nmeta = side.load(lane, (long long)mb0, min(KF_GROUP, W));
+        unsigned nmeta = side.load(lane, (long long)mb0, min(KF_GROUP, W), p.cbp);
 
         constexpr int sl = SL, per = 16 >> sl;
         const int opitch = W * per * 3;
@@ -250,13 +265,12 @@
             const unsigned meta = nmeta;
             const int nmb = min(KF_GROUP, W - g * KF_GROUP);
             const int n_next = min(KF_GROUP, W - (g + 1) * KF_GROUP);
-            if (n_next > 0) nmeta = side.load(lane, (long long)mb0 + (g + 1) * KF_GROUP, n_next);
+            if (n_next > 0) nmeta = side.load(lane, (long long)mb0 + (g + 1) * KF_GROUP, n_next, p.cbp);
             int16_t *tile = s.tile;
             mvg_mbar_wait(&s.mbar, parity);
             parity ^= 1u;
-            if (n_next > 0 && lane == 0) mvg_mbar_expect_tx(&s.mbar, (unsigned)n_next * 768u);
-
-            mvg_xf_group<KF_GROUP, KF_MBS>(tile, s.u.x, T, meta, nmb, lane);
+
+            uint3 pres = mvg_xf_group<KF_GROUP, KF_MBS, true>(tile, s.u.x, T, meta, nmb, lane);
             const uint4 rec = mvg_ctl_from_meta(meta);
 
 #if KF_HALO_GROUP
@@ -323,6 +337,8 @@
                 }
 #endif
                 c.resid = reinterpret_cast<const uint8_t *>(tile + j * KF_MBS);
+                c.rmask = pres.x & 0x00FFFFFFu;
+                pres.x = __funnelshift_r(pres.x, pres.y, 24); pres.y = __funnelshift_r(pres.y, pres.z, 24); pres.z >>= 24;
                 const unsigned cx = __shfl_sync(MVG_FULL, rec.x, 8 * j), cy = __shfl_sync(MVG_FULL, rec.y, 8 * j);
                 const unsigned cz = __shfl_sync(MVG_FULL, rec.z, 8 * j);
 
@@ -413,9 +429,13 @@
                 }
                 *cn_dst = *cn_src;
                 __syncwarp();
-                if (j < n_next && lane == 0) {
-                    asm volatile("fence.proxy.async.shared::cta;" ::: "memory");
-                    mvg_bulk_load(tile + j * KF_MBS, lv_row + (size_t)(mx + KF_GROUP) * 384, 768u, &s.mbar);
+                if (j < n_next) {
+                    const unsigned w = __shfl_sync(MVG_FULL, nmeta, 8 * j + 4);
+                    if (lane < 5) kf_copy_piece(tile + j * KF_MBS, lv_row + (size_t)(mx + KF_GROUP) * 384, lane, w, &s.mbar);
+                    if (j == n_next - 1) {
+                        __syncwarp();
+                        if (lane == 0) mvg_mbar_arrive(&s.mbar);
+                    }
                 }
                 if (OUT == KF_OUT_RGBS && j == nmb - 1) {
                     constexpr int unit = sl <= 2 ? 4 : 1, ppr = KF_GROUP * per * 3 / unit, total = per * ppr;
diff --git a/minivideo_b200/csrc/mvg_kernels.cuh b/minivideo_b200/csrc/mvg_kernels.cuh
--- a/minivideo_b200/csrc/mvg_kernels.cuh
+++ b/minivideo_b200/csrc/mvg_kernels.cuh
@@ -53,6 +53,7 @@
     const uint64_t *pic_base;
     const uint16_t *words;
     int16_t        *coeff;
+    uint8_t        *cbp;
     long long       n_mbs;
     int             mbs_per_pic;
 };
@@ -65,6 +66,9 @@
     const long long n_warps = ((long long)gridDim.x * blockDim.x) >> 5;
     for (long long mb = warp0; mb < p.n_mbs; mb += n_warps) {
         const unsigned nzb = __ldg(p.nz_blocks + mb) & 0x00FFFFFFu;
+        if (lane == 0)
+            p.cbp[mb] = (uint8_t)(((nzb & 0xFu) ? 1u : 0u) | ((nzb & 0xF0u) ? 2u : 0u) | ((nzb & 0xF00u) ? 4u : 0u) |
+                                  ((nzb & 0xF000u) ? 8u : 0u) | ((nzb >> 16) ? 0x20u : 0u));
         const long long pic = mb / p.mbs_per_pic;
         const uint16_t *w = p.words + __ldg(p.pic_base + pic) + __ldg(p.word_off + mb);
         const uint16_t *end = p.words + __ldg(p.pic_base + pic + 1);
@@ -155,6 +159,14 @@
 {
     asm volatile("mbarrier.arrive.expect_tx.shared::cta.b64 _, [%0], %1;" :: "r"(mvg_smem_u32(bar)), "r"(bytes) : "memory");
 }
+__device__ __forceinline__ void mvg_mbar_expect_tx_only(uint64_t *bar, unsigned bytes)
+{
+    asm volatile("mbarrier.expect_tx.relaxed.cta.shared::cta.b64 [%0], %1;" :: "r"(mvg_smem_u32(bar)), "r"(bytes) : "memory");
+}
+__device__ __forceinline__ void mvg_mbar_arrive(uint64_t *bar)
+{
+    asm volatile("mbarrier.arrive.shared::cta.b64 _, [%0];" :: "r"(mvg_smem_u32(bar)) : "memory");
+}
 __device__ __forceinline__ void mvg_mbar_wait(uint64_t *bar, unsigned parity)
 {
     unsigned ok;
@@ -183,6 +195,7 @@
     int32_t  f1[G][16];
     int32_t  tr[4][8][9];
     uint32_t meta[G];
+    uint32_t cm[G];
     int32_t  ls0[G];
     uint8_t  list4[G * 24 + 8];
     uint8_t  list8[G * 4 + 4];
@@ -230,28 +243,36 @@
                      : mt == 6 ? i16_mode : chroma_mode;
         stride = mt < 4 ? 16 : 1;
     }
-    __device__ __forceinline__ unsigned load(int lane, long long first, int n) const
+    __device__ __forceinline__ unsigned load(int lane, long long first, int n, const uint8_t *cbp = nullptr) const
     {
         unsigned v = 0u;
         if ((lane >> 3) < n) {
             const uint8_t *q = src + (first + (lane >> 3)) * stride;
             if ((lane & 7) < 4) v = __ldg(reinterpret_cast<const unsigned *>(q));
-            else v = (unsigned)__ldg(q);
+            else {
+                v = (unsigned)__ldg(q);
+                if (cbp && (lane & 7) == 4) v |= (unsigned)__ldg(cbp + first + (lane >> 3)) << 8;
+            }
         }
         return v;
     }
 };
 
-template <int G, int MBS = 384>
-__device__ __forceinline__ void mvg_xf_group(int16_t *tile, MvgXfScratch<G> &s, const MvgXfTables &T, unsigned meta, int nmb, int lane)
+template <int G, int MBS = 384, bool CBP = false>
+__device__ __forceinline__ uint3 mvg_xf_group(int16_t *tile, MvgXfScratch<G> &s, const MvgXfTables &T, unsigned meta, int nmb, int lane)
 {
     const int mj = lane >> 3, mt = lane & 7;
-    const int kind_j = (int)__shfl_sync(MVG_FULL, meta, (lane & ~7) + 4);
+    const unsigned kw = __shfl_sync(MVG_FULL, meta, (lane & ~7) + 4);
+    const int kind_j = CBP ? (int)(kw & 255) : (int)kw;
+    const unsigned cl_j = (kw >> 8) & 15, cc_j = min((kw >> 12) & 15, 2u);
     const int qp_j = min(max((int)(signed char)__shfl_sync(MVG_FULL, meta, (lane & ~7) + 5), 0), 51);
     if (mt == 0 && mj < G) {
         const unsigned sh = T.dcsh[qp_j];
         s.meta[mj] = (unsigned)kind_j | ((unsigned)(qp_j & 255) << 8) | (sh << 16) | (((1u << sh) >> 1) << 24);
         s.ls0[mj] = T.ls4q[qp_j * 16];
+        if (CBP)
+            s.cm[mj] = ((cl_j & 1u) | ((cl_j & 2u) << 3) | ((cl_j & 4u) << 6) | ((cl_j & 8u) << 9)) * 0xFu |
+                       (cc_j == 2 ? 0xFF0000u : 0u) | (cc_j == 1 ? 1u << 24 : 0u) | (kind_j == MVG_MB_I16x16 ? 1u << 25 : 0u);
     }
 
     if (mj < nmb) {
@@ -261,7 +282,7 @@
             const int c = cf[mvg_blk_of(2, mt) * 16], d = cf[mvg_blk_of(3, mt) * 16];
             int32_t *f1 = s.f1[mj] + mt * 4;
             f1[0] = a + b + c + d; f1[1] = a + b - c - d; f1[2] = a - b - c + d; f1[3] = a - b + c - d;
-        } else if (mt == 4 || mt == 5) {
+        } else if ((mt == 4 || mt == 5) && (!CBP || cc_j != 0)) {
             const int pl = mt - 4;
             const int16_t *cc = cf + 256 + pl * 64;
             const int c00 = cc[0], c01 = cc[16], c10 = cc[32], c11 = cc[48];
@@ -287,6 +308,7 @@
     __syncwarp();
 
     int n4 = 0, n8 = 0;
+    unsigned pres0 = 0u, pres1 = 0u, pres2 = 0u;
 #pragma unroll 1
     for (int r = 0; r < (G * 24 + 31) / 32; r++) {
         const int u = lane + 32 * r, j0 = G <= 4 ? r + (lane >= 24 - 8 * r) : u / 24, b = u - 24 * j0;
@@ -296,20 +318,29 @@
         const int kind = mw & 255;
         const bool is8 = kind == MVG_MB_I8x8 && b < 16;
         uint4 *blk = reinterpret_cast<uint4 *>(tile + j * MBS + b * 16);
+        bool ld = true, dcimp = false;
+        if (CBP) {
+            const unsigned cm = s.cm[j];
+            ld = live && ((cm >> b) & 1u);
+            dcimp = !ld && ((cm >> (b >= 16 ? 24 : 25)) & 1u);
+        }
         const int o = (lane >> 2) & 1;
-        const uint4 wa = blk[o], wb = blk[o ^ 1];
+        uint4 wa = make_uint4(0u, 0u, 0u, 0u), wb = wa;
+        if (ld) { wa = blk[o]; wb = blk[o ^ 1]; }
         const unsigned x0 = o ? wb.x : wa.x, x4 = o ? wa.x : wb.x;
         const unsigned rest = (x0 & 0xffff0000u) | x4 | wa.y | wa.z | wa.w | wb.y | wb.z | wb.w;
         const int dcraw = (short)(x0 & 0xffff);
         const bool nz8q = live && is8 && (rest | (x0 & 0xffffu)) != 0;
         const bool general = live && !is8 && rest != 0;
+        bool dconly;
         {
             const bool has_dc = b >= 16 || kind == MVG_MB_I16x16;
             const int sh = (mw >> 16) & 255;
             const int plain = (dcraw * s.ls0[j] + (int)(mw >> 24)) >> sh;
             const int d = has_dc ? s.dc[j][b] : plain;
             const int rv = min(max((d + 32) >> 6, -512), 511);
-            if (live && !is8 && rest == 0 && (rv != 0 || dcraw != 0)) {
+            dconly = live && !is8 && rest == 0 && (CBP ? rv != 0 && (ld || dcimp) : (rv != 0 || dcraw != 0));
+            if (dconly) {
                 const unsigned pk = (unsigned)(rv & 0xffff) * 0x10001u;
                 blk[o] = make_uint4(pk, pk, pk, pk); blk[o ^ 1] = make_uint4(pk, pk, pk, pk);
             }
@@ -323,6 +354,10 @@
         const unsigned lb = __ballot_sync(MVG_FULL, lead8);
         if (lead8) s.list8[n8 + __popc(lb & ((1u << lane) - 1))] = (uint8_t)(j * 4 + (b >> 2));
         n8 += __popc(lb);
+        if (CBP) {
+            const unsigned pb = __ballot_sync(MVG_FULL, dconly || general || any8);
+            if (r == 0) pres0 = pb; else if (r == 1) pres1 = pb; else pres2 = pb;
+        }
     }
     __syncwarp();
 
@@ -408,6 +443,7 @@
         __syncwarp();
     }
     __syncwarp();
+    return make_uint3(pres0, pres1, pres2);
 }
 
 __device__ __forceinline__ uint4 mvg_ctl_from_meta(unsigned meta)
@@ -570,6 +606,7 @@
     uint8_t *lt, *ct;
     uint8_t *n8;
     const uint8_t *resid;
+    unsigned rmask;
     const uint8_t *lut8;
     int lane;
     unsigned lut4;
@@ -622,15 +659,17 @@
         }
     }
     const uint8_t *r = c.resid + (lane >> 2) * 64 + (lane & 3) * 8;
-    const uint2 ra = *reinterpret_cast<const uint2 *>(r);
-    const uint2 rb = *reinterpret_cast<const uint2 *>(r + 32);
+    const unsigned rm = c.rmask >> (2 * (lane >> 2));
+    uint2 ra = make_uint2(0u, 0u), rb = ra;
+    if (rm & 1u) ra = *reinterpret_cast<const uint2 *>(r);
+    if (rm & 2u) rb = *reinterpret_cast<const uint2 *>(r + 32);
     const unsigned lo = mvg_pairs_to_bytes(mvg_add_clip8x2(pp[0], ra.x), mvg_add_clip8x2(pp[1], ra.y));
     const unsigned hi = mvg_pairs_to_bytes(mvg_add_clip8x2(pp[2], rb.x), mvg_add_clip8x2(pp[3], rb.y));
     *reinterpret_cast<uint2 *>(lt + K2_TO(0, 0) + y * MVG_LT_STRIDE + x0) = make_uint2(lo, hi);
 }
 
 template <int T>
-__device__ __forceinline__ void k2_luma4_step(const K2Ctx &c, unsigned seq, unsigned dcsteps)
+__device__ __forceinline__ void k2_luma4_step(const K2Ctx &c, unsigned seq, unsigned dcsteps, unsigned rsteps)
 {
     constexpr int bx0 = T & 1, by0 = T >> 1;
     constexpr bool v0 = T <= 7, v1 = T >= 2;
@@ -661,7 +700,8 @@
         const int other = __shfl_xor_sync(MVG_FULL, sum, 1);
         if (m == 0x100u) { sum += other; shift = 3; }
     }
-    const int r = *reinterpret_cast<const int16_t *>(c.resid + blk0 * 32 + ((by0 & 1) ? c.r4odd : c.r4even));
+    int r = 0;
+    if (rsteps & (1u << T)) r = *reinterpret_cast<const int16_t *>(c.resid + blk0 * 32 + ((by0 & 1) ? c.r4odd : c.r4even));
     const int v = mvg_add_clip8(sum >> shift, r);
     if ((v0 && v1) || (c.lane >= 16 ? v1 : v0)) c.lt[org1 + c.s4] = (uint8_t)v;
     __syncwarp();
@@ -698,20 +738,23 @@
         if (half) bits = (bits & 0xfcu) | ((bits & 3u) << 8);
         dcsteps = __reduce_or_sync(MVG_FULL, bits);
     }
-    k2_luma4_step<0>(c, seq, dcsteps);
-    k2_luma4_step<1>(c, seq, dcsteps);
-    k2_luma4_step<2>(c, seq, dcsteps);
-    k2_luma4_step<3>(c, seq, dcsteps);
-    k2_luma4_step<4>(c, seq, dcsteps);
-    k2_luma4_step<5>(c, seq, dcsteps);
-    k2_luma4_step<6>(c, seq, dcsteps);
-    k2_luma4_step<7>(c, seq, dcsteps);
-    k2_luma4_step<8>(c, seq, dcsteps);
-    k2_luma4_step<9>(c, seq, dcsteps);
+    const unsigned rm = c.rmask;
+    const unsigned rsteps = half ? ((rm >> 2) & 0x3Cu) | ((rm >> 6) & 0x3C0u) | (rm >> 30)
+                                 : (rm & 0xFu) | ((rm >> 4) & 0xF0u) | ((rm >> 22) & 0x300u);
+    k2_luma4_step<0>(c, seq, dcsteps, rsteps);
+    k2_luma4_step<1>(c, seq, dcsteps, rsteps);
+    k2_luma4_step<2>(c, seq, dcsteps, rsteps);
+    k2_luma4_step<3>(c, seq, dcsteps, rsteps);
+    k2_luma4_step<4>(c, seq, dcsteps, rsteps);
+    k2_luma4_step<5>(c, seq, dcsteps, rsteps);
+    k2_luma4_step<6>(c, seq, dcsteps, rsteps);
+    k2_luma4_step<7>(c, seq, dcsteps, rsteps);
+    k2_luma4_step<8>(c, seq, dcsteps, rsteps);
+    k2_luma4_step<9>(c, seq, dcsteps, rsteps);
 }
 
 template <int B8>
-__device__ __forceinline__ void k2_luma8_block(const K2Ctx &c, unsigned modes, unsigned fix, bool availA, bool availB, bool availC)
+__device__ __forceinline__ void k2_luma8_block(const K2Ctx &c, unsigned modes, unsigned fix, unsigned m8, bool availA, bool availB, bool availC)
 {
     uint8_t *lt = c.lt;
     const int lane = c.lane;
@@ -746,12 +789,13 @@
     const unsigned e = *reinterpret_cast<const unsigned *>(c.lut8 + mode * 128);
     MVG_ASSERT(mode < 16 && (e & 0xffffu) < MVG_N8_BYTES && (e >> 16) < MVG_N8_BYTES, 3);
     const unsigned pp = (unsigned)c.n8[e & 0xffffu] | ((unsigned)c.n8[e >> 16] << 16);
-    const unsigned r2 = *reinterpret_cast<const unsigned *>(c.resid + B8 * 128 + lane * 4);
+    unsigned r2 = 0u;
+    if ((m8 >> (4 * B8)) & 1u) r2 = *reinterpret_cast<const unsigned *>(c.resid + B8 * 128 + lane * 4);
     *reinterpret_cast<uint16_t *>(lt + org + c.s8) = (uint16_t)__byte_perm(mvg_add_clip8x2(pp, r2), 0, 0x4420);
     __syncwarp();
 }
 
-__device__ __forceinline__ void k2_luma8_block_rt(const K2Ctx &c, int b8, unsigned modes, unsigned fix, bool availA, bool availB, bool availC)
+__device__ __forceinline__ void k2_luma8_block_rt(const K2Ctx &c, int b8, unsigned modes, unsigned fix, unsigned m8, bool availA, bool availB, bool availC)
 {
     uint8_t *lt = c.lt;
     const int lane = c.lane;
@@ -785,7 +829,8 @@
     __syncwarp();
     const unsigned e = *reinterpret_cast<const unsigned *>(c.lut8 + mode * 128);
     const unsigned pp = (unsigned)c.n8[e & 0xffffu] | ((unsigned)c.n8[e >> 16] << 16);
-    const unsigned r2 = *reinterpret_cast<const unsigned *>(c.resid + b8 * 128 + lane * 4);
+    unsigned r2 = 0u;
+    if ((m8 >> (4 * b8)) & 1u) r2 = *reinterpret_cast<const unsigned *>(c.resid + b8 * 128 + lane * 4);
     *reinterpret_cast<uint16_t *>(lt + org + c.s8) = (uint16_t)__byte_perm(mvg_add_clip8x2(pp, r2), 0, 0x4420);
     __syncwarp();
 }
@@ -794,15 +839,16 @@
 __device__ __forceinline__ void k2_luma8(const K2Ctx &c, unsigned modes, bool availA, bool availB, bool availC, bool availD)
 {
     const unsigned fix = (availA ? 0u : c.fixA) | (availB ? 0u : c.fixB) | (availD ? 0u : c.fixD);
+    const unsigned m8 = (unsigned)((int)c.rmask >> (c.lane >> 3));
     if (COMPACT) {
 #pragma unroll 1
-        for (int b8 = 0; b8 < 4; b8++) k2_luma8_block_rt(c, b8, modes, fix, availA, availB, availC);
+        for (int b8 = 0; b8 < 4; b8++) k2_luma8_block_rt(c, b8, modes, fix, m8, availA, availB, availC);
         return;
     }
-    k2_luma8_block<0>(c, modes, fix, availA, availB, availC);
-    k2_luma8_block<1>(c, modes, fix, availA, availB, availC);
-    k2_luma8_block<2>(c, modes, fix, availA, availB, availC);
-    k2_luma8_block<3>(c, modes, fix, availA, availB, availC);
+    k2_luma8_block<0>(c, modes, fix, m8, availA, availB, availC);
+    k2_luma8_block<1>(c, modes, fix, m8, availA, availB, availC);
+    k2_luma8_block<2>(c, modes, fix, m8, availA, availB, availC);
+    k2_luma8_block<3>(c, modes, fix, m8, availA, availB, availC);
 }
 
 __device__ __forceinline__ void k2_chroma(const K2Ctx &c, int mode, bool left, bool up)
@@ -843,7 +889,8 @@
         p0 = (__vimin_s16x2_relu(pair, 0x1fff1fffu) >> 5) & 0x00ff00ffu;
         p1 = (__vimin_s16x2_relu(__vadd2(pair, (unsigned)((2 * b) & 0xffff) * 0x10001u), 0x1fff1fffu) >> 5) & 0x00ff00ffu;
     }
-    const uint2 r = *reinterpret_cast<const uint2 *>(c.resid + 512 + lane * 8);
+    uint2 r = make_uint2(0u, 0u);
+    if ((c.rmask >> (16 + (lane >> 2))) & 1u) r = *reinterpret_cast<const uint2 *>(c.resid + 512 + lane * 8);
     *reinterpret_cast<unsigned *>(ct + K2_CO(0, 0) + y * MVG_CT_STRIDE + x0) =
         mvg_pairs_to_bytes(mvg_add_clip8x2(p0, r.x), mvg_add_clip8x2(p1, r.y));
 }
@@ -879,6 +926,7 @@
     c.lane = lane;
     c.sel = p.sel;
     c.resid = reinterpret_cast<const uint8_t *>(s.resid[0]);
+    c.rmask = MVG_FULL;
     {
         const int half = lane >> 4, pix = lane & 15, px = pix & 3, py = pix >> 2;
         c.lut4 = lut_addr + (unsigned)lane * 4u;
```
